# tphakala/birdnet-go

Measured on AMD Instinct MI355X. Metric: 3s-48kHz clips/sec (whole node) + max-abs prob diff vs TFLite, BirdNET v2.4, higher is better.
Workload: dtype f32; 1 GPU; BASELINE configs[1]: BirdNET v2.4 fp32, batch 256 x 3 s @ 48 kHz per GPU, mel front-end + CNN + head on device, raw logits out; batch_per_gpu=256, n_samples=144000, n_classes=6522, pipeline_depth=2, input_sets=4

## Files before the change

### birdnet-go_amd/csrc/conv.hip

```cpp
#include "kernels.h"
#include "pw_common.h"

#include <algorithm>
#include <cstdlib>

namespace bnhip {

__global__ __launch_bounds__(256) void k_conv_direct(ConvParams p) {
    const int C4 = p.Cout >> 2;
    size_t total = (size_t)p.B * p.Ho * p.Wo * C4;
    size_t idx = (size_t)blockIdx.x * 256 + threadIdx.x;
    if (idx >= total) return;
    int c4 = (int)(idx % C4);
    size_t pix = idx / C4;
    int wo = (int)(pix % p.Wo);
    int ho = (int)((pix / p.Wo) % p.Ho);
    int b = (int)(pix / ((size_t)p.Wo * p.Ho));
    float4 acc = make_float4(0.f, 0.f, 0.f, 0.f);
    const float4* w4 = reinterpret_cast<const float4*>(p.w);
    for (int i = 0; i < p.kh; i++) {
        int hi = ho * p.sh - p.pt + i;
        if (hi < 0 || hi >= p.H) continue;
        for (int j = 0; j < p.kw; j++) {
            int wi = wo * p.sw - p.pl + j;
            if (wi < 0 || wi >= p.W) continue;
            const float* ip = p.in + (((size_t)b * p.H + hi) * p.W + wi) * p.Cin;
            const float4* wp = w4 + (size_t)((i * p.kw + j) * p.Cin) * C4 + c4;
            for (int ci = 0; ci < p.Cin; ci++) {
                float x = ip[ci];
                float4 w = wp[(size_t)ci * C4];
                acc.x = fmaf(x, w.x, acc.x); acc.y = fmaf(x, w.y, acc.y);
                acc.z = fmaf(x, w.z, acc.z); acc.w = fmaf(x, w.w, acc.w);
            }
        }
    }
    if (p.bias) {
        float4 bv = reinterpret_cast<const float4*>(p.bias)[c4];
        acc.x += bv.x; acc.y += bv.y; acc.z += bv.z; acc.w += bv.w;
    }
    acc.x = apply_act(acc.x, p.act); acc.y = apply_act(acc.y, p.act);
    acc.z = apply_act(acc.z, p.act); acc.w = apply_act(acc.w, p.act);
    reinterpret_cast<float4*>(p.out)[idx] = acc;
}
template <int KH, int KW, int CIN>
__global__ __launch_bounds__(256) void k_conv_direct_t(ConvParams p) {
    const int C4 = p.Cout >> 2;
    size_t total = (size_t)p.B * p.Ho * p.Wo * C4;
    size_t idx = (size_t)blockIdx.x * 256 + threadIdx.x;
    if (idx >= total) return;
    int c4 = (int)(idx % C4);
    size_t pix = idx / C4;
    int wo = (int)(pix % p.Wo);
    int ho = (int)((pix / p.Wo) % p.Ho);
    int b = (int)(pix / ((size_t)p.Wo * p.Ho));
    float x[KH][KW][CIN];
#pragma unroll
    for (int i = 0; i < KH; i++) {
        int hi = ho * p.sh - p.pt + i;
#pragma unroll
        for (int j = 0; j < KW; j++) {
            int wi = wo * p.sw - p.pl + j;
            bool ok = hi >= 0 && hi < p.H && wi >= 0 && wi < p.W;
            const float* ip = p.in + (((size_t)b * p.H + (ok ? hi : 0)) * p.W + (ok ? wi : 0)) * CIN;
#pragma unroll
            for (int ci = 0; ci < CIN; ci++) x[i][j][ci] = ok ? ip[ci] : 0.f;
        }
    }
    float4 acc = p.bias ? reinterpret_cast<const float4*>(p.bias)[c4] : make_float4(0.f, 0.f, 0.f, 0.f);
    float4 a2 = make_float4(0.f, 0.f, 0.f, 0.f);
    const float4* w4 = reinterpret_cast<const float4*>(p.w) + c4;
#pragma unroll
    for (int i = 0; i < KH; i++)
#pragma unroll
        for (int j = 0; j < KW; j++)
#pragma unroll
            for (int ci = 0; ci < CIN; ci++) {
                float4 w = w4[(size_t)((i * KW + j) * CIN + ci) * C4];
                float xv = x[i][j][ci];
                a2.x = fmaf(xv, w.x, a2.x); a2.y = fmaf(xv, w.y, a2.y); a2.z = fmaf(xv, w.z, a2.z); a2.w = fmaf(xv, w.w, a2.w);
            }
    with_act(p.act, [&](auto f) {
        acc.x = f(a2.x + acc.x); acc.y = f(a2.y + acc.y); acc.z = f(a2.z + acc.z); acc.w = f(a2.w + acc.w);
    });
    reinterpret_cast<float4*>(p.out)[idx] = acc;
}
template <int KH, int KW, int CIN, int S, int PX>
__global__ __launch_bounds__(256) void k_conv_direct_px(ConvParams p, int wgroups) {
    constexpr int NCOL = (PX - 1) * S + KW;
    const int C4 = p.Cout >> 2;
    size_t total = (size_t)p.B * p.Ho * wgroups * C4;
    size_t idx = (size_t)blockIdx.x * 256 + threadIdx.x;
    if (idx >= total) return;
    int c4 = (int)(idx % C4);
    size_t g = idx / C4;
    int wg = (int)(g % wgroups);
    int ho = (int)((g / wgroups) % p.Ho);
    int b = (int)(g / ((size_t)wgroups * p.Ho));
    const int wo0 = wg * PX, wi0 = wo0 * S - p.pl;
    float x[KH][NCOL][CIN];
#pragma unroll
    for (int i = 0; i < KH; i++) {
        int hi = ho * S - p.pt + i;
        bool rok = hi >= 0 && hi < p.H;
        const float* rp = p.in + ((size_t)b * p.H + (rok ? hi : 0)) * p.W * CIN;
#pragma unroll
        for (int c = 0; c < NCOL; c++) {
            int wi = wi0 + c;
            bool ok = rok && wi >= 0 && wi < p.W;
            const float* ip = rp + (size_t)(ok ? wi : 0) * CIN;
#pragma unroll
            for (int ci = 0; ci < CIN; ci++) x[i][c][ci] = ok ? ip[ci] : 0.f;
        }
    }
    const float4 bv = p.bias ? reinterpret_cast<const float4*>(p.bias)[c4] : make_float4(0.f, 0.f, 0.f, 0.f);
    float4 a2[PX];
#pragma unroll
    for (int q = 0; q < PX; q++) a2[q] = make_float4(0.f, 0.f, 0.f, 0.f);
    const float4* w4 = reinterpret_cast<const float4*>(p.w) + c4;
#pragma unroll
    for (int i = 0; i < KH; i++)
#pragma unroll
        for (int j = 0; j < KW; j++)
#pragma unroll
            for (int ci = 0; ci < CIN; ci++) {
                float4 w = w4[(size_t)((i * KW + j) * CIN + ci) * C4];
#pragma unroll
                for (int q = 0; q < PX; q++) {
                    float xv = x[i][q * S + j][ci];
                    a2[q].x = fmaf(xv, w.x, a2[q].x); a2[q].y = fmaf(xv, w.y, a2[q].y);
                    a2[q].z = fmaf(xv, w.z, a2[q].z); a2[q].w = fmaf(xv, w.w, a2[q].w);
                }
            }
    with_act(p.act, [&](auto f) {
#pragma unroll
        for (int q = 0; q < PX; q++) {
            a2[q].x = f(a2[q].x + bv.x); a2[q].y = f(a2[q].y + bv.y); a2[q].z = f(a2[q].z + bv.z); a2[q].w = f(a2[q].w + bv.w);
        }
    });
    const size_t o0 = (((size_t)b * p.Ho + ho) * p.Wo + wo0) * C4 + c4;
    float4* op = reinterpret_cast<float4*>(p.out) + o0;
#pragma unroll
    for (int q = 0; q < PX; q++)
        if (wo0 + q < p.Wo) {
            if (p.out_bf16) bf16x4_store(p.out, o0 + (size_t)q * C4, a2[q]);
            else op[(size_t)q * C4] = a2[q];
        }
}
bool conv_direct_bf16_ok(const ConvParams& p) {
    return p.kh == 3 && p.kw == 3 && (p.Cin == 1 || p.Cin == 2) && p.sh == 2 && p.sw == 2 && (p.Cout & 3) == 0;
}
void launch_conv_direct(const ConvParams& p, hipStream_t s) {
    if (p.kh == 3 && p.kw == 3 && p.Cin == 2 && p.sh == 2 && p.sw == 2 && (p.Cout & 3) == 0) {
        constexpr int PX = 4;
        int wgroups = (p.Wo + PX - 1) / PX;
        size_t tot = (size_t)p.B * p.Ho * wgroups * (p.Cout >> 2);
        hipLaunchKernelGGL((k_conv_direct_px<3, 3, 2, 2, PX>), dim3((unsigned)((tot + 255) / 256)), dim3(256), 0, s, p, wgroups);
        return;
    }
    if (p.kh == 3 && p.kw == 3 && p.Cin == 1 && p.sh == 2 && p.sw == 2 && (p.Cout & 3) == 0) {
        constexpr int PX = 4;
        int wgroups = (p.Wo + PX - 1) / PX;
        size_t tot = (size_t)p.B * p.Ho * wgroups * (p.Cout >> 2);
        hipLaunchKernelGGL((k_conv_direct_px<3, 3, 1, 2, PX>), dim3((unsigned)((tot + 255) / 256)), dim3(256), 0, s, p, wgroups);
        return;
    }
    size_t total = (size_t)p.B * p.Ho * p.Wo * (p.Cout >> 2);
    dim3 grid((unsigned)((total + 255) / 256));
    if (p.kh == 3 && p.kw == 3 && p.Cin == 2) hipLaunchKernelGGL((k_conv_direct_t<3, 3, 2>), grid, dim3(256), 0, s, p);
    else if (p.kh == 3 && p.kw == 3 && p.Cin == 1) hipLaunchKernelGGL((k_conv_direct_t<3, 3, 1>), grid, dim3(256), 0, s, p);
    else if (p.kh == 3 && p.kw == 3 && p.Cin == 3) hipLaunchKernelGGL((k_conv_direct_t<3, 3, 3>), grid, dim3(256), 0, s, p);
    else hipLaunchKernelGGL(k_conv_direct, grid, dim3(256), 0, s, p);
}

struct StemParams {
    const float* in; const float* wm ; const float* bias ; float* out;
    int B, H, W, Ho, Wo, Cout, pt, pl, act;
    unsigned total_px, tiles_per_wave;
};
template <int NTILES>
__global__ __launch_bounds__(256) void k_stem_mfma(StemParams p) {
    constexpr int CS = NTILES * 16 + 4;
    __shared__ __attribute__((aligned(16))) float stage[4 * 16 * CS];
    const int lane = threadIdx.x & 63, wave = threadIdx.x >> 6;
    const int li = lane & 15, kq = lane >> 4;
    f32x4 wf[2][NTILES];
    float4 bq[NTILES];
#pragma unroll
    for (int t = 0; t < NTILES; t++) {
#pragma unroll
        for (int sl = 0; sl < 2; sl++) {
            float4 w = *reinterpret_cast<const float4*>(p.wm + (size_t)(16 * t + li) * 32 + 16 * sl + 4 * kq);
            wf[sl][t] = (f32x4){w.x, w.y, w.z, w.w};
        }
        bq[t] = *reinterpret_cast<const float4*>(p.bias + 16 * t + 4 * kq);
    }
    const int i0 = kq >> 1, j0 = (kq & 1) * 2;
    const unsigned tile0 = (blockIdx.x * 4u + wave) * p.tiles_per_wave;
    const unsigned hw = (unsigned)p.Ho * p.Wo;
    unsigned px = tile0 * 16u + li;
    int b, oh, ow;
    {
        const unsigned pc = min(px, p.total_px - 1);
        b = pc / hw;
        const unsigned rem = pc - (unsigned)b * hw;
        oh = rem / p.Wo; ow = rem - oh * p.Wo;
    }
    for (unsigned tt = 0; tt < p.tiles_per_wave; tt++, px += 16u) {
        if ((tile0 + tt) * 16u >= p.total_px) break;
        if (tt) {
            ow += 16;
            while (ow >= p.Wo) { ow -= p.Wo; if (++oh == p.Ho) { oh = 0; b++; } }
            if (b >= p.B) { b = p.B - 1; oh = p.Ho - 1; ow = p.Wo - 1; }
        }
        const float* xb = p.in + (size_t)b * p.H * p.W * 2;
        f32x4 xf[2];
        const int r0 = oh * 2 - p.pt, c0 = ow * 2 - p.pl + j0;
        const bool inner = r0 >= 0 && r0 + 2 < p.H && c0 >= 0 && c0 + 1 < p.W;
        if (__builtin_amdgcn_ballot_w64(!inner) == 0) {
#pragma unroll
            for (int sl = 0; sl < 2; sl++) {
                const float* q = xb + ((size_t)(r0 + (sl == 0 ? i0 : 2)) * p.W + c0) * 2;
                const float2 a = *reinterpret_cast<const float2*>(q), c = *reinterpret_cast<const float2*>(q + 2);
                xf[sl] = (f32x4){a.x, a.y, c.x, c.y};
            }
        } else {
#pragma unroll
            for (int sl = 0; sl < 2; sl++) {
                const int row = r0 + (sl == 0 ? i0 : 2), col = c0;
                const bool rv = row >= 0 && row < p.H;
                const bool v0 = rv && col >= 0 && col < p.W, v1 = rv && col + 1 >= 0 && col + 1 < p.W;
                const int rc = min(max(row, 0), p.H - 1);
                const float2 a = *reinterpret_cast<const float2*>(xb + ((size_t)rc * p.W + min(max(col, 0), p.W - 1)) * 2);
                const float2 c = *reinterpret_cast<const float2*>(xb + ((size_t)rc * p.W + min(max(col + 1, 0), p.W - 1)) * 2);
                xf[sl] = (f32x4){v0 ? a.x : 0.f, v0 ? a.y : 0.f, v1 ? c.x : 0.f, v1 ? c.y : 0.f};
            }
        }
        f32x4 acc[NTILES];
#pragma unroll
        for (int t = 0; t < NTILES; t++) acc[t] = (f32x4){0.f, 0.f, 0.f, 0.f};
#pragma unroll
        for (int sl = 0; sl < 2; sl++)
#pragma unroll
            for (int sidx = 0; sidx < 4; sidx++)
#pragma unroll
                for (int t = 0; t < NTILES; t++)
                    acc[t] = __builtin_amdgcn_mfma_f32_16x16x4f32(wf[sl][t][sidx], xf[sl][sidx], acc[t], 0, 0, 0);
        with_act(p.act, [&](auto f) {
#pragma unroll
            for (int t = 0; t < NTILES; t++) {
                acc[t][0] = f(acc[t][0] + bq[t].x); acc[t][1] = f(acc[t][1] + bq[t].y);
                acc[t][2] = f(acc[t][2] + bq[t].z); acc[t][3] = f(acc[t][3] + bq[t].w);
            }
        });
        float* stg = stage + wave * (16 * CS);
#pragma unroll
        for (int t = 0; t < NTILES; t++) *reinterpret_cast<f32x4*>(&stg[li * CS + 16 * t + 4 * kq]) = acc[t];
        __builtin_amdgcn_s_waitcnt(0xc07f);
        __builtin_amdgcn_wave_barrier();
        const unsigned px0 = (tile0 + tt) * 16u;
#pragma unroll
        for (int q = 0; q < (16 * NTILES * 4) / 64; q++) {
            const int idx = lane + 64 * q;
            const int row = idx / (NTILES * 4), c4 = idx % (NTILES * 4);
            if (px0 + row < p.total_px)
                *reinterpret_cast<f32x4*>(p.out + (size_t)(px0 + row) * p.Cout + 4 * c4) = *reinterpret_cast<const f32x4*>(&stg[row * CS + 4 * c4]);
        }
        __builtin_amdgcn_wave_barrier();
    }
}
bool stem_mfma_supported(const ConvParams& p) {
    return p.kh == 3 && p.kw == 3 && p.sh == 2 && p.sw == 2 && p.Cin == 2 && (p.Cout == 32 || p.Cout == 64);
}
void launch_stem_mfma(const ConvParams& c, const float* wm, const float* bias_p, hipStream_t s) {
    static const int stem_tpw = getenv("BNHIP_STEM_TPW") ? std::max(atoi(getenv("BNHIP_STEM_TPW")), 1) : 8;
    StemParams p{c.in, wm, bias_p, c.out, c.B, c.H, c.W, c.Ho, c.Wo, c.Cout, c.pt, c.pl, c.act,
                 (unsigned)((size_t)c.B * c.Ho * c.Wo), (unsigned)stem_tpw};
    unsigned tiles = (p.total_px + 15) / 16;
    unsigned blocks = (tiles + 4 * p.tiles_per_wave - 1) / (4 * p.tiles_per_wave);
    if (c.Cout == 32) hipLaunchKernelGGL((k_stem_mfma<2>), dim3(blocks), dim3(256), 0, s, p);
    else hipLaunchKernelGGL((k_stem_mfma<4>), dim3(blocks), dim3(256), 0, s, p);
}

}
```

### birdnet-go_amd/csrc/dwconv.hip

```cpp
#include "kernels.h"
#include "pw_common.h"

#include <algorithm>
#include <cstdlib>

namespace bnhip {

template <int K, int S, int TH, int TW, bool IN16 = false>
__global__ __launch_bounds__(256) void k_dwconv_t(DwParams p, int CX, int PY, int tiles_w, int tiles, int tchunks,
                                                  int cchunks, unsigned nblk, float* __restrict__ partial) {
    __shared__ float red[256 * 4];
    const unsigned L = xcd_remap(blockIdx.x, nblk);
    const int bpc = tchunks * cchunks;
    const int b = L / bpc;
    const int rest = L % bpc;
    const int tc = rest / cchunks, cc = rest % cchunks;
    const int tx = threadIdx.x % CX, ty = threadIdx.x / CX;
    const int c4 = cc * CX + tx;
    const int C4 = p.C >> 2;
    const int tile = tc * PY + ty;
    const bool live = c4 < C4 && tile < tiles && ty < PY;
    float4 acc[TH][TW];
#pragma unroll
    for (int a = 0; a < TH; a++)
#pragma unroll
        for (int c = 0; c < TW; c++) acc[a][c] = make_float4(0.f, 0.f, 0.f, 0.f);
    const int th0 = live ? (tile / tiles_w) * TH : 0, tw0 = live ? (tile % tiles_w) * TW : 0;
    if (live) {
        constexpr int RW = (TW - 1) * S + K;
        constexpr int RH = (TH - 1) * S + K;
        const int hi0 = th0 * S - p.pt, wi0 = tw0 * S - p.pl;
        const float4* in4 = reinterpret_cast<const float4*>(p.in) + (size_t)b * p.H * p.W * C4 + c4;
        const float4* w4 = reinterpret_cast<const float4*>(p.w) + c4;
        uint2 raw[IN16 ? RH : 1][IN16 ? RW : 1];
        if constexpr (IN16) {
            const uint2* in2 = reinterpret_cast<const uint2*>(p.in) + (size_t)b * p.H * p.W * C4 + c4;
#pragma unroll
            for (int r = 0; r < RH; r++)
#pragma unroll
                for (int c = 0; c < RW; c++) {
                    const int hi = hi0 + r, wi = wi0 + c;
                    const bool in = hi >= 0 && hi < p.H && wi >= 0 && wi < p.W;
                    raw[r][c] = in ? in2[((size_t)hi * p.W + wi) * C4] : make_uint2(0u, 0u);
                }
        }
#pragma unroll
        for (int r = 0; r < RH; r++) {
            const int hi = hi0 + r;
            if (hi < 0 || hi >= p.H) continue;
            float4 x[RW];
#pragma unroll
            for (int c = 0; c < RW; c++) {
                int wi = wi0 + c;
                if constexpr (IN16) {
                    const uint2 rr = raw[r][c];
                    x[c] = make_float4(__uint_as_float(rr.x << 16), __uint_as_float(rr.x & 0xffff0000u), __uint_as_float(rr.y << 16), __uint_as_float(rr.y & 0xffff0000u));
                } else if (!(wi >= 0 && wi < p.W)) x[c] = make_float4(0.f, 0.f, 0.f, 0.f);
                else if (p.in_bf16) x[c] = bf16x4_load(p.in, ((size_t)b * p.H * p.W + (size_t)hi * p.W + wi) * C4 + c4);
                else x[c] = in4[((size_t)hi * p.W + wi) * C4];
            }
#pragma unroll
            for (int a = 0; a < TH; a++) {
                const int i = r - a * S;
                if (i < 0 || i >= K) continue;
#pragma unroll
// ... 16 lines not shown
        if (p.act == ACT_SWISH) {
#pragma unroll
            for (int a = 0; a < TH; a++)
#pragma unroll
                for (int c = 0; c < TW; c++) {
                    float4& v = acc[a][c];
                    const f32x4 r = swish4((f32x4){v.x + bv.x, v.y + bv.y, v.z + bv.z, v.w + bv.w});
                    v = make_float4(r[0], r[1], r[2], r[3]);
                }
        } else {
            with_act(p.act, [&](auto f) {
#pragma unroll
                for (int a = 0; a < TH; a++)
#pragma unroll
                    for (int c = 0; c < TW; c++) {
                        float4& v = acc[a][c];
                        v.x = f(v.x + bv.x); v.y = f(v.y + bv.y); v.z = f(v.z + bv.z); v.w = f(v.w + bv.w);
                    }
            });
        }
#pragma unroll
        for (int a = 0; a < TH; a++) {
            int ho = th0 + a;
            if (ho >= p.Ho) continue;
#pragma unroll
            for (int c = 0; c < TW; c++) {
                int wo = tw0 + c;
                if (wo >= p.Wo) continue;
                float4 v = acc[a][c];
                if (p.out_bf16) bf16x4_store(p.out, ((size_t)b * p.Ho * p.Wo + (size_t)ho * p.Wo + wo) * C4 + c4, v);
                else out4[((size_t)ho * p.Wo + wo) * C4] = v;
                sum.x += v.x; sum.y += v.y; sum.z += v.z; sum.w += v.w;
            }
        }
    }
    if (partial) {
        reinterpret_cast<float4*>(red)[threadIdx.x] = sum;
        __syncthreads();
        if (ty == 0 && c4 < C4) {
            float4 t = make_float4(0.f, 0.f, 0.f, 0.f);
            for (int y = 0; y < PY; y++) {
                float4 v = reinterpret_cast<float4*>(red)[y * CX + tx];
                t.x += v.x; t.y += v.y; t.z += v.z; t.w += v.w;
            }
            reinterpret_cast<float4*>(partial)[((size_t)b * tchunks + tc) * C4 + c4] = t;
        }
    }
}

template <int VEC>
__global__ __launch_bounds__(256) void k_dwconv(DwParams p) {
    const int CV = p.C / VEC;
    size_t total = (size_t)p.B * p.Ho * p.Wo * CV;
    size_t idx = (size_t)blockIdx.x * 256 + threadIdx.x;
    if (idx >= total) return;
    int cv = (int)(idx % CV);
    size_t pix = idx / CV;
    int wo = (int)(pix % p.Wo);
    int ho = (int)((pix / p.Wo) % p.Ho);
    int b = (int)(pix / ((size_t)p.Wo * p.Ho));
    float acc[VEC];
#pragma unroll
    for (int v = 0; v < VEC; v++) acc[v] = 0.f;
    for (int i = 0; i < p.kh; i++) {
        int hi = ho * p.sh - p.pt + i;
        if (hi < 0 || hi >= p.H) continue;
        for (int j = 0; j < p.kw; j++) {
            int wi = wo * p.sw - p.pl + j;
            if (wi < 0 || wi >= p.W) continue;
            const float* ip = p.in + (((size_t)b * p.H + hi) * p.W + wi) * p.C + (size_t)cv * VEC;
            const float* wp = p.w + (size_t)(i * p.kw + j) * p.C + (size_t)cv * VEC;
#pragma unroll
            for (int v = 0; v < VEC; v++) acc[v] = fmaf(ip[v], wp[v], acc[v]);
        }
    }
#pragma unroll
    for (int v = 0; v < VEC; v++) {
        float x = acc[v];
        if (p.bias) x += p.bias[cv * VEC + v];
        p.out[idx * VEC + v] = apply_act(x, p.act);
    }
}

static void dw_geometry(const DwParams& p, int TH, int TW, int* CX, int* PY, int* tiles_w, int* tiles, int* tchunks,
                        int* cchunks) {
    int C4 = p.C / 4;
    *CX = C4 < 64 ? C4 : 64;
    *PY = 256 / *CX;
    *tiles_w = (p.Wo + TW - 1) / TW;
    *tiles = *tiles_w * ((p.Ho + TH - 1) / TH);
    if (*PY > *tiles) *PY = *tiles;
    *tchunks = (*tiles + *PY - 1) / *PY;
    *cchunks = (C4 + *CX - 1) / *CX;
}
static bool dw_tiled_shape(const DwParams& p, int* TH, int* TW) {
    if ((p.C & 3) || p.kh != p.kw || p.sh != p.sw) return false;
    if (p.kh == 3 && p.sh == 1) { *TH = 2; *TW = 4; return true; }
    if (p.kh == 3 && p.sh == 2) { *TH = 2; *TW = 2; return true; }
    if (p.kh == 5 && p.sh == 1) { *TH = 2; *TW = 4; return true; }
    if (p.kh == 5 && p.sh == 2) { *TH = 1; *TW = 2; return true; }
    return false;
}
int dwconv_sum_slabs(const DwParams& p) {
    int TH, TW, CX, PY, tw, t, tch, cch;
    if (!dw_tiled_shape(p, &TH, &TW)) return 0;
    dw_geometry(p, TH, TW, &CX, &PY, &tw, &t, &tch, &cch);
    return tch;
}
bool dwconv_tile_geometry(const DwParams& p, int* PY, int* tiles_w, int* tiles, int* tchunks) {
    int TH, TW, CX, cch;
    if (!dw_tiled_shape(p, &TH, &TW) || TH != 2 || TW != 4) return false;
    dw_geometry(p, TH, TW, &CX, PY, tiles_w, tiles, tchunks, &cch);
    return true;
}
void launch_dwconv(const DwParams& p, float* partial, hipStream_t s) {
    int TH, TW;
    if (dw_tiled_shape(p, &TH, &TW)) {
        int CX, PY, tiles_w, tiles, tchunks, cchunks;
        dw_geometry(p, TH, TW, &CX, &PY, &tiles_w, &tiles, &tchunks, &cchunks);
        unsigned nblk = (unsigned)p.B * tchunks * cchunks;
        dim3 block(CX * PY < 64 ? 64 : CX * PY);
        static const bool pre16 = !(getenv("BNHIP_DW_PREFETCH") && atoi(getenv("BNHIP_DW_PREFETCH")) == 0);
#define DW_LAUNCH(K_, S_, TH_, TW_) do { if (p.in_bf16 && pre16) hipLaunchKernelGGL((k_dwconv_t<K_, S_, TH_, TW_, true>), dim3(nblk), block, 0, s, p, CX, PY, \
                                                       tiles_w, tiles, tchunks, cchunks, nblk, partial); \
                                         else hipLaunchKernelGGL((k_dwconv_t<K_, S_, TH_, TW_>), dim3(nblk), block, 0, s, p, CX, PY, \
                                                       tiles_w, tiles, tchunks, cchunks, nblk, partial); } while (0)
        if (p.kh == 3 && p.sh == 1) DW_LAUNCH(3, 1, 2, 4);
        else if (p.kh == 3) DW_LAUNCH(3, 2, 2, 2);
        else if (p.sh == 1) DW_LAUNCH(5, 1, 2, 4);
        else DW_LAUNCH(5, 2, 1, 2);
#undef DW_LAUNCH
        return;
    }
    if ((p.C & 3) == 0) {
        size_t total = (size_t)p.B * p.Ho * p.Wo * (p.C / 4);
        hipLaunchKernelGGL(k_dwconv<4>, dim3((unsigned)((total + 255) / 256)), dim3(256), 0, s, p);
    } else {
        size_t total = (size_t)p.B * p.Ho * p.Wo * p.C;
        hipLaunchKernelGGL(k_dwconv<1>, dim3((unsigned)((total + 255) / 256)), dim3(256), 0, s, p);
    }
}

#define MEAN_SLAB 512
int mean_splits(int HW) { return (HW + MEAN_SLAB - 1) / MEAN_SLAB; }

__global__ __launch_bounds__(256) void k_mean_partial(const float* __restrict__ in, float* __restrict__ partial,
                                                      int HW, int C, int S) {
    __shared__ float red[256];
    const int b = blockIdx.z, sp = blockIdx.y;
    const int CW = blockDim.x, PY = blockDim.y;
    const int c = blockIdx.x * CW + threadIdx.x;
    const int p0 = sp * MEAN_SLAB, p1 = min(HW, p0 + MEAN_SLAB);
    float acc = 0.f;
    if (c < C)
        for (int px = p0 + threadIdx.y; px < p1; px += PY) acc += in[((size_t)b * HW + px) * C + c];
    red[threadIdx.y * CW + threadIdx.x] = acc;
    __syncthreads();
    if (threadIdx.y == 0 && c < C) {
        float sum = 0.f;
        for (int y = 0; y < PY; y++) sum += red[y * CW + threadIdx.x];
        partial[((size_t)b * S + sp) * C + c] = sum;
    }
}
int mean_partial_py(int C) {
    int CW = C < 64 ? C : 64;
    int PY = 256 / CW; if (PY < 1) PY = 1;
    return PY;
}
void launch_mean_partial(const float* in, float* partial, int B, int HW, int C, int S, hipStream_t s) {
    int CW = C < 64 ? C : 64;
    int PY = mean_partial_py(C);
    dim3 grid((C + CW - 1) / CW, S, B);
    hipLaunchKernelGGL(k_mean_partial, grid, dim3(CW, PY), 0, s, in, partial, HW, C, S);
}
__global__ void k_mean_finish(const float* __restrict__ partial, float* __restrict__ out, int B, int HW, int C, int S) {
    size_t idx = (size_t)blockIdx.x * blockDim.x + threadIdx.x;
    if (idx >= (size_t)B * C) return;
    int c = (int)(idx % C); size_t b = idx / C;
    float sum = 0.f;
    for (int sidx = 0; sidx < S; sidx++) sum += partial[(b * S + sidx) * C + c];
    out[idx] = sum / (float)HW;
}
void launch_mean_finish(const float* partial, float* out, int B, int HW, int C, int S, hipStream_t s) {
    size_t total = (size_t)B * C;
    hipLaunchKernelGGL(k_mean_finish, dim3((unsigned)((total + 255) / 256)), dim3(256), 0, s, partial, out, B, HW, C, S);
}

__global__ __launch_bounds__(1024) void k_se(SeParams p) {
    extern __shared__ __attribute__((aligned(16))) float sm[];
    float* mean = sm;
    float* r = sm + p.C;
    const int b = blockIdx.x, tid = threadIdx.x, lane = tid & 63, wave = tid >> 6;
    const int NTHR = blockDim.x, NW = NTHR >> 6;
    const float inv = 1.0f / (float)p.HW;
    int P = 1;
    while (P * 2 * p.C <= NTHR && P * 2 <= p.S) P *= 2;
    float* part = sm + ((p.C + p.Cr + 3) & ~3);
    if (P > 1) {
        const int c = tid % p.C, q = tid / p.C;
        if (q < P) {
            float sum = 0.f;
#pragma unroll 4
            for (int sidx = q; sidx < p.S; sidx += P) sum += p.partial[((size_t)b * p.S + sidx) * p.C + c];
            part[q * p.C + c] = sum;
        }
        __syncthreads();
        for (int c2 = tid; c2 < p.C; c2 += NTHR) {
            float sum = 0.f;
            for (int q2 = 0; q2 < P; q2++) sum += part[q2 * p.C + c2];
            mean[c2] = sum * inv;
        }
    } else {
        for (int c = tid; c < p.C; c += NTHR) {
            float sum = 0.f;
#pragma unroll 4
            for (int sidx = 0; sidx < p.S; sidx++) sum += p.partial[((size_t)b * p.S + sidx) * p.C + c];
            mean[c] = sum * inv;
        }
    }
    __syncthreads();
    const bool v4 = (p.C & 3) == 0;
    for (int j0 = wave; j0 < p.Cr; j0 += 4 * NW) {
        float acc[4] = {0.f, 0.f, 0.f, 0.f};
        if (v4) {
            const float4* m4 = reinterpret_cast<const float4*>(mean);
            const float4* w4 = reinterpret_cast<const float4*>(p.w1);
            const int C4 = p.C / 4;
#pragma unroll 2
            for (int c = lane; c < C4; c += 64) {
                const float4 mv = m4[c];
                float4 w[4];
#pragma unroll
                for (int u = 0; u < 4; u++) w[u] = w4[(size_t)min(j0 + u * NW, p.Cr - 1) * C4 + c];
#pragma unroll
                for (int u = 0; u < 4; u++) {
                    acc[u] = fmaf(w[u].x, mv.x, acc[u]); acc[u] = fmaf(w[u].y, mv.y, acc[u]);
                    acc[u] = fmaf(w[u].z, mv.z, acc[u]); acc[u] = fmaf(w[u].w, mv.w, acc[u]);
                }
            }
        } else {
            for (int c = lane; c < p.C; c += 64) {
                const float mv = mean[c];
#pragma unroll
                for (int u = 0; u < 4; u++) acc[u] = fmaf(p.w1[(size_t)min(j0 + u * NW, p.Cr - 1) * p.C + c], mv, acc[u]);
            }
// ... 64 lines not shown
```

### birdnet-go_amd/csrc/engine.cpp

```cpp
#include "engine.h"

#include <algorithm>
#include <cmath>
#include <cstdio>
#include <cstdlib>
#include <cstring>
#include <mutex>
#include <sstream>

#include "../../include/bnhip.h"
#include "hostpipe.h"

namespace bnhip {

#define HIPCHK(call)                                                                           \
    do {                                                                                       \
        hipError_t e_ = (call);                                                                \
        if (e_ != hipSuccess) {                                                                \
            *err = std::string(#call) + ": " + hipGetErrorString(e_);                          \
            return false;                                                                      \
        }                                                                                      \
    } while (0)

Engine::~Engine() {
// ... 415 lines not shown
        const float* d_in = lanes[li].d_in; float* d_logits = lanes[li].d_logits; float* d_emb = lanes[li].d_emb;
        const int n = lanes[li].n, clip0 = nl > 1 ? li : -1;
        hipStream_t stream = lanes[li].st;
        float* in0 = vptr(s.in0, d_in, d_logits, d_emb, clip0);
        float* in1 = vptr(s.in1, d_in, d_logits, d_emb, clip0);
        float* in2 = vptr(s.in2, d_in, d_logits, d_emb, clip0);
        float* out = vptr(s.out, d_in, d_logits, d_emb, clip0);
        float* out2 = vptr(s.out2, d_in, d_logits, d_emb, clip0);
        if (s.kind == S_DW && si > 0 && steps[si - 1].tail == 2 && tail_taken(si - 1, n, nl > 1)) continue;
        if (s.kind == S_MEAN_PARTIAL && si > 0 && steps[si - 1].tail == 1 && tail_taken(si - 1, n, nl > 1)) continue;
        if (s.kind == S_MEAN_FINISH && si > 1 && steps[si - 2].tail == 1 && tail_taken(si - 2, n, nl > 1)) continue;
        if (s.kind == S_NORMALIZE && si == norm_pair + 1 && res_x[li]) continue;
        ProfEntry pe{};
        static const char* dbg_sync_before = getenv("BNHIP_DEBUG_SYNC_BEFORE");
        static const char* dbg_sync_after = getenv("BNHIP_DEBUG_SYNC_AFTER");
        static const char* dbg_ctx1_only = getenv("BNHIP_DEBUG_CTX1_ONLY");
        if (dbg_ctx1_only && cur_ctx == 1 && !strstr(dbg_ctx1_only, s.kclass)) continue;
        static const char* dbg_ctx1_skip = getenv("BNHIP_DEBUG_CTX1_SKIP");
        if (dbg_ctx1_skip && cur_ctx == 1 && strstr(dbg_ctx1_skip, s.kclass)) continue;
        if (dbg_sync_before && (!strcmp(dbg_sync_before, s.kclass) || s.name.rfind(dbg_sync_before, 0) == 0)) hipStreamSynchronize(stream);
        const bool prof_this = profiling && (profile_filter.empty() || profile_filter == s.kclass);
        if (prof_this) { pe.a = get_event(); pe.b = get_event(); pe.step = si; pe.n = n; hipEventRecord(pe.a, stream); }
        switch (s.kind) {
            case S_MINMAX:
                if (si == norm_pair && res_x[li]) {
                    const WinView lane_win = win_at(pcm.win, lanes[li].clip0);
                    if (!launch_clip_norm_resident(res_x[li], res_bits[li], n, n_samples, specs[0].eps, specs[0].norm_sub, specs[0].norm_mul,
                                                   reinterpret_cast<float2*>(out), vptr(steps[si + 1].out, d_in, d_logits, d_emb, clip0), stream,
                                                   res_framed[li] ? &lane_win : nullptr)) {
                        *err = "k_clip_norm_resident refused a call its predicate accepted"; mm_dirty = true; return false;
                    }
                    pe.more_bytes = steps[si + 1].bytes - s.bytes - (res_bits[li] ? (double)n_samples * (4 - res_bits[li] / 8) : 0.0);
                    break;
                }
                launch_clip_minmax(in0, n, n_samples, specs[0].eps, reinterpret_cast<float2*>(out),
                                   mm_scratch ? mm_scratch + ((size_t)std::max(cur_ctx, 0) * kMaxLanes + (size_t)li) * kMinMaxScratch : nullptr, stream);
                break;
            case S_FRONTEND: {
                const FrontSpec& fs = specs[s.spec];
                FrontendParams p;
                p.x = in0; p.mm = reinterpret_cast<const float2*>(in1); p.G = fs.G; p.window = fs.window; p.out = out;
                p.n_samples = n_samples; p.L = fs.L; p.Lfft = fs.Lfft; p.Kp = fs.Kp; p.hop = fs.hop; p.F = fs.F; p.n_mels = fs.n_mels;
                p.NTP = fs.NTP; p.C = C_spec; p.c = fs.c; p.norm_sub = fs.norm_sub; p.norm_mul = fs.norm_mul;
                p.p1 = fs.p1; p.p2 = fs.p2; p.n_clips = n;
                launch_frontend(p, stream);
                break;
            }
            case S_NORMALIZE:
                launch_normalize(in0, reinterpret_cast<const float2*>(in1), out, n, n_samples, specs[0].norm_sub, specs[0].norm_mul, stream);
                break;
            case S_STFT: {
                const FrontSpec& fs = specs[s.spec];
                StftParams p{in0, fs.window_full, fs.bins, out, n_samples, fs.Lfft, fs.L, fs.hop, fs.F, fs.nb, fs.nbp, fs.mode, n, fs.stft_tw, fs.pad_left};
                p.zmask = fs.stft_zmask;
                if (s.mode == 1) {
                    p.out = nullptr; p.img = out; p.mel = s.w3; p.mel_quads = s.S; p.n_mels = fs.n_mels; p.Ctot = C_spec; p.c0 = fs.c;
                    p.logc = fs.log_compress ? 1 : 0; p.time_major = fs.time_major ? 1 : 0; p.p1 = fs.p1; p.p2 = fs.p2;
                    p.lfloor = fs.log_floor; p.lscale = fs.log_scale;
                }
                {
                    static const bool f32_off = getenv("BNHIP_STFT_F32") && atoi(getenv("BNHIP_STFT_F32")) == 0;
                    if (precision == 1 && s.mode != 1 && fs.log_compress && !f32_off) p.f32 = 1;
                }
                launch_stft_bins(p, stream);
                break;
            }
            case S_MELBAND: {
                const FrontSpec& fa = specs[s.spec];
                const FrontSpec& fb = specs[s.S == 2 ? s.op : s.spec];
                MelBandParams p{{in0, s.S == 2 ? in1 : in0}, {s.w0, s.S == 2 ? s.w2 : s.w0},
                                {reinterpret_cast<const int*>(s.w1), reinterpret_cast<const int*>(s.S == 2 ? s.w3 : s.w1)},
                                {fa.nbp, fb.nbp}, {fa.p1, fb.p1}, {fa.p2, fb.p2}, out, fa.F, fa.n_mels, C_spec, fa.c,
                                fa.log_compress ? 1 : 0, fa.log_floor, fa.log_scale, fa.time_major ? 1 : 0};
                launch_mel_banded(p, s.S, n, stream);
                break;
            }
            case S_MELFIN: {
                const FrontSpec& fa = specs[s.spec];
                const FrontSpec& fb = specs[s.S == 2 ? s.op : s.spec];
                MelFinParams p{{in0, s.S == 2 ? in1 : in0}, {fa.p1, fb.p1}, {fa.p2, fb.p2}, out, fa.F, fa.n_mels, fa.n_mels, C_spec, fa.c,
                               fa.log_compress ? 1 : 0, fa.log_floor, fa.log_scale, fa.time_major ? 1 : 0};
                launch_mel_finish(p, s.S, n, stream);
                break;
            }
            case S_CONV_DIRECT: {
                ConvParams p{in0, s.w0, s.w1, out, n, s.H, s.W, s.C, s.Ho, s.Wo, s.Co, s.kh, s.kw, s.sh, s.sw, s.pt, s.pl, s.act};
                p.out_bf16 = vals[s.out].half ? 1 : 0;
                if (s.w2) launch_stem_mfma(p, s.w2, s.w3, stream);
                else launch_conv_direct(p, stream);
                break;
            }
            case S_CONV_IGEMM:
                launch_conv_igemm(in0, s.w0, s.w1, out, n, s.H, s.W, s.C, s.Ho, s.Wo, s.Co, s.kh, s.kw, s.sh, s.sw, s.g.dh, s.g.dw, s.pt, s.pl,
                                  s.act, 0, 0, stream);
                break;
            case S_PW: {
                PwParams p = pw_params(s, n, nl > 1);
                p.A = in0; p.ascale = in1; p.res = in2; p.out = out;
                if (tail_taken(si, n, nl > 1)) {
                    const Step& c = steps[si + 1];
                    PwTail t = tail_of(s, c);
                    if (s.tail == 2) { t.out = vptr(c.out, d_in, d_logits, d_emb, clip0); t.partial = vptr(c.out2, d_in, d_logits, d_emb, clip0); }
                    else p.out = vptr(steps[si + 2].out, d_in, d_logits, d_emb, clip0);
                    launch_pw_tail(p, t, s.wbx, p.nt, p.wm, stream);
                    break;
                }
                if (p.wm >= 13) p.wm = 10;
                if (p.wm >= 5 && s.wbx) launch_pw_bx3(p, s.wbx, stream);
                else launch_pw_gemm(p, stream);
                break;
            }
            case S_DW: {
                DwParams p = dw_params(s, in0, out, n);
                p.in_bf16 = vals[s.in0].half ? 1 : 0; p.out_bf16 = vals[s.out].half ? 1 : 0;
                if (s.dwl) launch_dwconv_lds(p, out2, s.shape, stream);
                else launch_dwconv(p, out2, stream);
                break;
            }
            case S_EXPAND_DW:
                {
                    StemGeom sg{s.H2, s.W2, s.pt2, s.pl2};
                    launch_expand_dw(in0, s.w0, s.w1, s.w2, s.w3, out, out2, n, s.H, s.W, s.C, s.Co,
                                     s.Ho, s.Wo, s.kh, s.sh, s.pt, s.pl, s.act, s.act2, s.shape, s.mode == 1 ? &sg : nullptr, stream,
                                     s.bx ? s.wbx : nullptr, precision, vals[s.out].half ? 1 : 0, vals[s.in0].half ? 1 : 0);
                }
                break;
            case S_MEAN_PARTIAL:
                launch_mean_partial(in0, out, n, s.H * s.W, s.C, s.S, stream);
                break;
            case S_MEAN_FINISH:
                launch_mean_finish(in0, out, n, s.H * s.W, s.C, s.S, stream);
                break;
            case S_SE: {
                SeParams p{in0, s.S, s.H * s.W, s.w0, s.w1, s.w2, s.w3, out, n, s.C, s.Cr, s.act, s.act2};
                if (cur_stream) p.threads = 256;
                launch_se(p, stream);
                break;
            }
            case S_UNARY:
                launch_unary(in0, out, vals[s.in0].elems * (size_t)n, s.act, stream);
                break;
            case S_BINARY:
                launch_binary(in0, s.mode == 2 ? s.w0 : in1, out, vals[s.in0].elems * (size_t)n, s.op, s.mode, s.H * s.W, s.C,
                              s.act, stream);
                break;
            case S_EW_UNARY:
                launch_unary_op(in0, out, vals[s.in0].elems * (size_t)n, s.op, s.g.alpha, stream);
                break;
            case S_EW_BINARY: {
                BcastParams p;
                p.a = s.g.a_const ? s.w0 : in0; p.b = s.g.b_const ? s.w1 : in1; p.out = out;
                for (int k = 0; k < 4; k++) { p.d[k] = s.g.d[k]; p.sa[k] = s.g.sa[k]; p.sb[k] = s.g.sb[k]; }
                p.bsa = s.g.a_const ? 0 : (long)vals[s.in0].elems; p.bsb = s.g.b_const ? 0 : (long)vals[s.in1].elems;
                p.op = s.op; p.act = s.act;
                launch_binary_bcast(p, n, stream);
                break;
            }
            case S_POOL: {
                PoolParams p{in0, out, n, s.H, s.W, s.C, s.Ho, s.Wo, s.kh, s.kw, s.sh, s.sw, s.pt, s.pl, s.mode, s.act};
                launch_pool2d(p, stream);
                break;
            }
            case S_COPY: {
                if (s.g.fill) launch_fill(out, vals[s.out].elems * (size_t)n, s.g.alpha, stream);
                CopyParams p;
                p.in = s.g.a_const ? s.w0 : in0; p.out = out;
                for (int k = 0; k < 4; k++) { p.d[k] = s.g.d[k]; p.si[k] = s.g.sa[k]; p.so[k] = s.g.so[k]; }
                p.offi = s.g.offa; p.offo = s.g.offo;
                p.bsi = s.g.a_const ? 0 : (long)vals[s.in0].elems; p.bso = (long)vals[s.out].elems;
                launch_copy_view(p, n, stream);
                break;
            }
            case S_SOFTMAX:
                launch_softmax_rows(in0, out, (size_t)s.H * (size_t)n, s.C, s.g.alpha, stream);
                break;
            case S_REDUCE: {
                ReduceParams p{in0, out, {s.g.d[0], s.g.d[1], s.g.d[2], s.g.d[3]}, s.g.mask, s.op};
                launch_reduce(p, n, stream);
                break;
            }
            case S_CONV_GENERIC: {
                GenConvParams p{in0, s.w0, s.w1, out, n, s.H, s.W, s.C, s.Ho, s.Wo, s.Co, s.kh, s.kw, s.sh, s.sw, s.g.dh, s.g.dw,
                                s.pt, s.pl, s.act, s.g.depthwise, s.g.mult};
                launch_conv_generic(p, stream);
                break;
            }
        }
// ... 29 lines not shown
        hipEventElapsedTime(&b, step_ev[0].first, step_ev[i].second);
        if (i < cap) { if (start_ms) start_ms[i] = a; if (end_ms) end_ms[i] = b; }
    }
    for (auto& p : step_ev) { hipEventDestroy(p.first); hipEventDestroy(p.second); }
    step_ev.clear();
    (void)hipGetLastError();
    return n;
}

static void jesc(std::ostringstream& os, const std::string& s) {
    for (char c : s) { if (c == '"' || c == '\\') os << '\\'; os << c; }
}

struct StepView { std::string name; double flops, bytes; bool absorbed; };
static StepView step_view(const Engine& e, size_t i) {
    const Step& s = e.steps[i];
    StepView v{s.name, s.flops, s.bytes, false};
    auto fused = [&](size_t k) { return e.steps[k].kind == S_PW && e.steps[k].tail && e.steps[k].wm_full >= 13; };
    if (fused(i)) {
        const double mine = 4.0 * s.H * s.W * s.Co;
        if (s.tail == 2) { v.name += "+dw"; v.flops += e.steps[i + 1].flops; }
        else { v.name += "+mean"; v.flops += e.steps[i + 1].flops + e.steps[i + 2].flops; v.bytes += 4.0 * s.Co - mine; }
    } else if ((s.kind == S_DW && i > 0 && e.steps[i - 1].tail == 2 && fused(i - 1)) ||
               (s.kind == S_MEAN_PARTIAL && i > 0 && e.steps[i - 1].tail == 1 && fused(i - 1)) ||
               (s.kind == S_MEAN_FINISH && i > 1 && e.steps[i - 2].tail == 1 && fused(i - 2))) {
        v.flops = 0; v.bytes = 0; v.absorbed = true;
    }
    return v;
}

std::string Engine::describe() const {
    std::ostringstream os;
    os << "{\"tune_source\":\"";
    jesc(os, tune_source);
    os << "\",\"tune_key\":\"" << (device >= 0 ? tune_key() : std::string()) << "\",\"split_step\":" << split_step << ",\"heatmap_tail\":\"" << (heatmap_pruned_step() >= 0 ? "pruned" : "gather") << "\",\"n_samples\":" << n_samples << ",\"n_classes\":" << n_classes << ",\"emb_dim\":" << emb_dim
       << ",\"max_batch\":" << max_batch << ",\"logits_output\":" << logits_output << ",\"embedding_output\":" << embedding_output << ",\"precision\":\"" << (precision ? "bf16" : "f32") << "\",\"lanes\":" << n_lanes << ",\"lane_min_batch\":" << dual_lane_min << ",\"act_arena_bytes\":" << act_bytes << ",\"weight_bytes\":" << w_bytes
       << ",\"specs\":[";
    for (size_t i = 0; i < specs.size(); i++) {
        const FrontSpec& f = specs[i];
        os << (i ? "," : "") << "{\"frame_length\":" << f.L << ",\"fft_length\":" << f.Lfft << ",\"hop\":" << f.hop
           << ",\"frames\":" << f.F << ",\"n_mels\":" << f.n_mels << ",\"channel\":" << f.c << ",\"p1\":" << f.p1
           << ",\"p2\":" << f.p2 << "}";
    }
    os << "],\"steps\":[";
    for (size_t i = 0; i < steps.size(); i++) {
        const Step& s = steps[i];
        const StepView sv = step_view(*this, i);
        const bool absorbed = sv.absorbed;
        os << (i ? "," : "") << "{\"i\":" << i << ",\"kernel\":\"" << s.kclass << "\",\"name\":\"";
        jesc(os, sv.name);
        os << "\",\"H\":" << s.H << ",\"W\":" << s.W << ",\"C\":" << s.C << ",\"Co\":" << s.Co << ",\"k\":" << s.kh
           << ",\"stride\":" << s.sh << ",\"act\":" << s.act << ",\"fused_scale\":" << (s.kind == S_PW && s.in1 >= 0 ? 1 : 0)
           << ",\"shape\":" << s.shape << ",\"dw_lds\":" << s.dwl << ",\"bx\":" << s.bx << ",\"nt\":" << s.nt << ",\"wm\":" << s.wm << ",\"nt_full\":" << s.nt_full << ",\"wm_full\":" << s.wm_full << ",\"fused_res\":" << (s.kind == S_PW && s.in2 >= 0 ? 1 : 0) << ",\"fused_sum\":" << (s.out2 >= 0 ? 1 : 0) << ",\"flops\":" << sv.flops << ",\"bytes\":" << sv.bytes << ",\"wbytes\":" << s.wbytes
           << ",\"tail\":" << s.tail << ",\"absorbed\":" << (absorbed ? 1 : 0) << ",\"out_v\":" << s.out << ",\"out2_v\":" << s.out2
           << ",\"in_bf16\":" << ((s.in0 >= 0 && vals[s.in0].half) ? 1 : 0) << ",\"out_bf16\":" << ((s.out >= 0 && vals[s.out].half) ? 1 : 0) << "}";
    }
    os << "]}";
    return os.str();
}

std::string Engine::profile_read() {
    hipStreamSynchronize(stream);
    struct Agg { double ms = 0, flops = 0, bytes = 0; long launches = 0; };
    std::map<std::string, Agg> agg;
    std::vector<std::string> order;
    std::vector<Agg> per_step(steps.size());
    for (auto& e : prof) {
        float ms = 0;
        hipEventElapsedTime(&ms, e.a, e.b);
        const Step& s = steps[e.step];
        const StepView sv = step_view(*this, e.step);
        if (!agg.count(s.kclass)) order.push_back(s.kclass);
        Agg& a = agg[s.kclass];
        a.ms += ms; a.launches++; a.flops += sv.flops * e.n; a.bytes += (sv.bytes + e.more_bytes) * e.n + s.wbytes;
        Agg& ps = per_step[e.step];
        ps.ms += ms; ps.launches++; ps.flops += sv.flops * e.n; ps.bytes += (sv.bytes + e.more_bytes) * e.n + s.wbytes;
        ev_pool.push_back(e.a); ev_pool.push_back(e.b);
    }
    prof.clear();
    std::ostringstream os;
    os << "[";
    for (size_t i = 0; i < order.size(); i++) {
        const Agg& a = agg[order[i]];
        os << (i ? "," : "") << "{\"kernel\":\"" << order[i] << "\",\"launches\":" << a.launches << ",\"ms\":" << a.ms
           << ",\"flops\":" << a.flops << ",\"bytes\":" << a.bytes << "}";
    }
    for (size_t i = 0; i < steps.size(); i++) {
        const Agg& a = per_step[i];
        if (!a.launches) continue;
        os << ",{\"step\":" << i << ",\"kernel\":\"" << steps[i].kclass << "\",\"name\":\"";
        jesc(os, step_view(*this, i).name);
        os << "\",\"launches\":" << a.launches << ",\"ms\":" << a.ms << ",\"flops\":" << a.flops << ",\"bytes\":" << a.bytes << "}";
    }
    os << "]";
    return os.str();
}

}
```

### birdnet-go_amd/csrc/engine.h

```cpp
#pragma once
#include <hip/hip_runtime.h>

#include <map>
#include <string>
#include <vector>

#include "kernels.h"
#include "tflite_model.h"

namespace bnhip {

enum StepKind { S_MINMAX, S_FRONTEND, S_NORMALIZE, S_STFT, S_MELFIN, S_MELBAND, S_CONV_DIRECT, S_PW, S_DW, S_EXPAND_DW, S_MEAN_PARTIAL, S_MEAN_FINISH, S_SE, S_UNARY, S_BINARY,
                S_EW_UNARY, S_EW_BINARY, S_POOL, S_COPY, S_SOFTMAX, S_REDUCE, S_CONV_GENERIC,
                S_CONV_IGEMM };

struct GenGeom {
    int d[4] = {1, 1, 1, 1};
    long sa[4] = {0, 0, 0, 0}, sb[4] = {0, 0, 0, 0}, so[4] = {0, 0, 0, 0};
    long offa = 0, offo = 0;
    bool a_const = false, b_const = false;
    int mask = 0;
    float alpha = 0.f;
    bool fill = false;
    int dh = 1, dw = 1, depthwise = 0, mult = 1;
};

struct Step {
    StepKind kind;
    std::string name;
    const char* kclass;
    int in0 = -1, in1 = -1, in2 = -1, out = -1, out2 = -1;
    const float *w0 = nullptr, *w1 = nullptr, *w2 = nullptr, *w3 = nullptr;
    const uint16_t* wbx = nullptr;
    int dwl = 0;
    int bx = 0;
    int H = 0, W = 0, C = 0, Ho = 0, Wo = 0, Co = 0, kh = 1, kw = 1, sh = 1, sw = 1, pt = 0, pl = 0;
    int act = 0, act2 = 0, op = 0, mode = 0, S = 1, Cr = 0;
    int nt = 0, wm = 0;
    int tail = 0;
    int H2 = 0, W2 = 0, pt2 = 0, pl2 = 0;
    int shape = -1;
    int nt_full = 0, wm_full = 0;
    int spec = -1;
    GenGeom g;
    double flops = 0, bytes = 0, wbytes = 0;
};

struct Value {
    int tfl = -1;
    size_t elems = 0;
    size_t offset = 0;
    size_t offset_lane = 0;
    int first = -1, last = -1;
    bool external = false;
    bool half = false;
};

struct FrontSpec {
    int L, Kp, Lfft, hop, F, n_mels, NTP, c;
    float p1, p2, eps, norm_sub, norm_mul;
    const double* G = nullptr;
    const float* window = nullptr;
    bool fft = false;
    int nb = 0, nbp = 0, mode = 0;
    const float* window_full = nullptr;
    const double* stft_tw = nullptr;
    unsigned stft_zmask = 0xffffffffu;
    const int* bins = nullptr;
    bool normalize = true, log_compress = false, time_major = false;
    int pad_left = 0;
    float log_floor = 0.f, log_scale = 1.f;
};

struct PcmSource { const void* samples = nullptr; int bits = 0;  WinView win = {}; };

struct ProfEntry { hipEvent_t a, b; int step; int n; double more_bytes = 0; };

struct WeightPlan {
    std::vector<float> img;
    std::vector<size_t> step_w[4];
    std::vector<size_t> step_bx;
};

inline DwParams dw_params(const Step& s, const float* in = nullptr, float* out = nullptr, int n = 1) {
    return DwParams{in, s.w0, s.w1, out, n, s.H, s.W, s.C, s.Ho, s.Wo, s.kh, s.kw, s.sh, s.sw, s.pt, s.pl, s.act};
}
PwTail tail_of(const Step& s, const Step& c);

class Engine {
  public:
    ~Engine();
    bool build(TflModel m, int device, int max_batch, bool plan_only, std::string* err, int* code);
    bool run(const float* d_in, int n, float* d_logits, float* d_emb, std::string* err, PcmSource pcm = {});

    int device = 0, max_batch = 256;
    bool no_reuse = false;
    bool autotune = true;
    bool defer_weights = false;
    void finish_deferred();
    char* weights_ptr() const { return w_arena; }
    size_t weights_bytes() const { return w_bytes; }
    int frontend_fft = -1;
    int logits_output = -1, embedding_output = -2;
    int precision = 0;
    int bf16x3 = 0;
    int pw_sw = 0;
    bool use_graphs = false;
    void drop_graphs();
    static constexpr int kMaxDepth = 3;
    int depth = 1;
    hipStream_t ctx_stream[kMaxDepth] = {nullptr, nullptr, nullptr};
    char* ctx_arena[kMaxDepth] = {nullptr, nullptr, nullptr};
    static constexpr int kMinMaxScratch = 16 * (2 * kMinMaxParts + 2);
    float* mm_scratch = nullptr;
    bool mm_dirty = false;
    bool norm_resident = true;
    int norm_pair = -1;
    bool pcm_direct = false;
    void find_norm_pair();
    bool norm_resident_taken(int n, const void* x, int bits, const float* xn) const;
    hipEvent_t ev_ctx_fork = nullptr, ev_ctx_done[kMaxDepth] = {nullptr, nullptr, nullptr};
    unsigned call_idx = 0;
    bool run_pipelined(const float* d_in, int n, float* d_logits, float* d_emb, std::string* err);
    void sync_contexts();
    int host_depth = 2;
    bool ensure_contexts(int d, std::string* err, bool with_streams = true);
    bool run_on_context(int c, hipStream_t st, const float* d_in, int n, float* d_logits, float* d_emb, std::string* err, PcmSource pcm = {});
    int split_step = -1, v_hand = -1;
    float* d_hand = nullptr;
    std::vector<int> split_candidates;
    void pick_split();
    size_t hand_clip_bytes() const { return v_hand < 0 ? 0 : vals[v_hand].elems * (vals[v_hand].half ? 2 : 4); }
    bool ensure_hand(std::string* err);
    bool run_part(int c, hipStream_t st, int s0, int s1, const float* d_in, int n, float* hand, float* d_logits, float* d_emb, std::string* err, PcmSource pcm = {});
    int heatmap_pruned_step() const;
    bool run_head(int s1, const float* d_in, int n, std::string* err);
    struct HostPipe* hostpipe = nullptr;
    static constexpr int kMaxLanes = 4;
    int n_lanes = 2;
    int dual_lane_min = 32;
    hipStream_t lane_stream[kMaxLanes - 1] = {nullptr, nullptr, nullptr};
    hipEvent_t ev_fork = nullptr, ev_join[kMaxLanes - 1] = {nullptr, nullptr, nullptr};
    void mark_tails();
    bool tail_taken(int si, int n, bool lane_tuning) const;
    PwParams pw_params(const Step& s, int n, bool lane_tuning) const;
    void mark_bf16_storage();
    void tune_or_load();
    void autotune_pw();
    void autotune_expdw();
    void autotune_dw();
    void autotune_tail();
    bool save_tuning(const char* path) const;
    bool load_tuning(const char* path);
    std::string tuning_text() const;
    bool apply_tuning_text(const std::string& text);
    std::string tune_key() const;
    std::string tune_dir;
    std::string tune_source;
    bool expdw_pipe16(const Step& s) const;
    ExpDwGeo expdw_geo(const Step& s) const;
    void set_sum_slabs(Step& s, int S);
    std::map<int, int> tensor_value;
    const float* value_ptr(int v) const { return reinterpret_cast<const float*>(act_arena + vals[v].offset); }
    int n_samples = 0, n_classes = 0, emb_dim = 0, C_spec = 0;
    hipStream_t stream = nullptr;
    bool own_stream = false;
    static constexpr int kMaxKStreams = 4;
    hipStream_t kstream[kMaxKStreams] = {nullptr, nullptr, nullptr, nullptr};
    hipStream_t kernel_stream(int i);
    hipStream_t copy_stream();
    hipStream_t xfer_stream = nullptr;
    bool ds_ref = false;
// ... 49 lines not shown
```

### birdnet-go_amd/csrc/expdw.hip

```cpp
#include "kernels.h"
#include "pw_common.h"

#include <algorithm>
#include <type_traits>
#include <cmath>
#include <cstdio>
#include <cstdlib>
#include <cstring>
#include <vector>

namespace bnhip {

struct ExpDwParams {
    const float* x; const float* we; const float* be; const float* wd; const float* bd;
    float* y; float* partial;
    int B, H, W, Cin, Cmid, Ho, Wo, pt, pl, act_e, act_d, tiles_h, tiles_w, cchunks, Kw, Cp;
    int Hin = 0, Win = 0, pts = 0, pls = 0;
    const uint16_t* wep = nullptr; int Kp = 0;
    int prec = 0;
    int xsh = 0, xsw = 1, ysh = 0, ysw = 1, tr = 0;
    int in_bf16 = 0, out_bf16 = 0;
    FDiv d_bpc{}, d_cch{}, d_tw{};
    int cpp = 0;
    FDiv d_part{};
};
#define ED_ES 36
#define ED_PERM2 0xfdce5764b98a1320ull
#define ED_PERM4 0xfdce9ba875461320ull
__device__ __forceinline__ int ed_perm(unsigned long long magic, int lane) {
    return (int)((magic >> ((lane >> 2) * 4)) & 15ull) * 4 + (lane & 3);
}
constexpr bool ed_perm_c4_rule(unsigned long long magic) {
    for (int g = 0; g < 16; g++)
        if (((magic >> (4 * g)) & 1ull) != (unsigned long long)((g >> 1) & 1)) return false;
    return true;
}
constexpr int expdw_min_waves(int K, int S, int TOW, int TRH) {
    const int tiw = (TOW - 1) * S + K, jt = (TRH * tiw + 15) / 16, jtw = (jt + 3) / 4;
    return jtw <= 4 ? 4 : (jtw == 5 ? 3 : 2);
}
#ifndef EXPDW_NW8_WAVES
#define EXPDW_NW8_WAVES (est <= 76 ? 6 : 4)
#endif
constexpr int expdw_sk_waves(int K, int S, int TOH, int TOW, int TRH, int KW, bool one_chunk, int NW = 4) {
    const int tiw = (TOW - 1) * S + K, jt = (TRH * tiw + 15) / 16, jtw = (jt + NW - 1) / NW;
    if (one_chunk) return jtw <= 3 ? 5 : expdw_min_waves(K, S, TOW, TRH);
    const int sh = TOH / NW, sw = TOW / 8, rw = (sw - 1) * S + K;
    const int p1 = jtw * 8 + 8, p2 = sh * sw * 4 + rw * 4 + K * 4;
    const int est = jtw * KW / 4 + (KW / 2 + 16) + 24 + (p1 > p2 ? p1 : p2);
    if (NW == 8) return EXPDW_NW8_WAVES;
    return est <= 120 ? 4 : (est <= 160 ? 3 : 2);
}
template <int K, int S, int TOH, int TOW, int TRH, int NW = 4, typename PreStore>
__device__ __forceinline__ float4 ed_phase2(const ExpDwParams& p, const float* E, const float4* wds, int b, int oh0, int ow0, int vr0,
                                            int vr1, int ty, int tx, int c4, int n_base, const float4& bv, PreStore&& pre_store) {
    constexpr int TIW = (TOW - 1) * S + K;
    static_assert(TOH % NW == 0, "a wave owns TOH / NW output rows");
    constexpr int SH = TOH / NW, SW = TOW / 8;
    constexpr int RW = (SW - 1) * S + K;
    const int n = n_base + 4 * c4;
    float4 sum = make_float4(0.f, 0.f, 0.f, 0.f);
    float4 acc2[SH][SW];
#pragma unroll
    for (int a = 0; a < SH; a++)
#pragma unroll
        for (int c = 0; c < SW; c++) acc2[a][c] = make_float4(0.f, 0.f, 0.f, 0.f);
    if (n < p.Cmid) {
        const float* e0 = E + (tx * SW * S) * ED_ES + 4 * c4;
#pragma unroll 1
        for (int i = 0; i < K; i++) {
            float4 w[K];
#pragma unroll
            for (int j = 0; j < K; j++) w[j] = wds[(i * K + j) * 8 + c4];
#pragma unroll
            for (int a = 0; a < SH; a++) {
                const int fr = (ty * SH + a) * S + i;
                if (fr < vr0 || fr >= vr1 || oh0 + ty * SH + a >= p.Ho) continue;
// ... 44 lines not shown
                const unsigned yo = ylane + (unsigned)((a * p.ysh + c * p.ysw) * p.Cmid);
                if (p.out_bf16) bf16x4_store(p.y, ((size_t)b * p.Ho * p.Wo * p.Cmid + yo) >> 2, v);
                else *reinterpret_cast<float4*>(yclip + yo) = v;
                sum.x += v.x; sum.y += v.y; sum.z += v.z; sum.w += v.w;
            }
        }
    }
    return sum;
}
__device__ __forceinline__ void ed_sums_lanes(float4 sum, float4* red, int wave, int lane, int c4) {
    static_assert(ed_perm_c4_rule(ED_PERM2) && ed_perm_c4_rule(ED_PERM4), "lane permutation: c4 bit 2 must be physical lane bit 3");
    auto xsum = [&](auto pat) {
        constexpr int P = decltype(pat)::value;
        sum.x += __builtin_bit_cast(float, __builtin_amdgcn_ds_swizzle(__builtin_bit_cast(int, sum.x), P));
        sum.y += __builtin_bit_cast(float, __builtin_amdgcn_ds_swizzle(__builtin_bit_cast(int, sum.y), P));
        sum.z += __builtin_bit_cast(float, __builtin_amdgcn_ds_swizzle(__builtin_bit_cast(int, sum.z), P));
        sum.w += __builtin_bit_cast(float, __builtin_amdgcn_ds_swizzle(__builtin_bit_cast(int, sum.w), P));
    };
    xsum(std::integral_constant<int, 0x101f>{});
    xsum(std::integral_constant<int, 0x401f>{});
    if ((lane & 0x14) == 0) red[(wave * 2 + (lane >> 5)) * 8 + c4] = sum;
}
template <int NW = 4>
__device__ __forceinline__ void ed_sums_out(const ExpDwParams& p, const float4* red, int tid, size_t tile_index, int n_base) {
    if (tid < 8 && n_base + 4 * tid < p.Cmid) {
        float4 t = red[tid];
#pragma unroll
        for (int w = 1; w < 2 * NW; w++) { float4 v = red[w * 8 + tid]; t.x += v.x; t.y += v.y; t.z += v.z; t.w += v.w; }
        unsigned l4 = 4u * (unsigned)tid;
        asm volatile("" : "+v"(l4));
        *reinterpret_cast<float4*>(p.partial + tile_index * p.Cmid + n_base + l4) = t;
    }
}

constexpr int expdw_fullw_vw(int K, int S, int TOW) { return TOW * S == 32 && (TOW - 1) * S + K >= 32 ? 32 : 0; }
template <int K, int S, int TOH, int TOW, int TRH, bool H8 = false, bool BX = false, bool COPY = false, int VW = 0>
__global__ __launch_bounds__(256, BX ? expdw_min_waves(K, S, TOW, TRH) : 1) void k_expand_dw(ExpDwParams p, unsigned nblk) {
    constexpr int TIH = (TOH - 1) * S + K, TIW = (TOW - 1) * S + K;
    static_assert(TRH <= TIH, "TRH is a cap on the footprint rows");
    constexpr bool FULLW = VW > 0;
    static_assert(!FULLW || (!COPY && VW % 16 == 0 && VW <= TIW && VW == expdw_fullw_vw(K, S, TOW)), "full-width form: see expdw_fullw_vw");
    static_assert(!FULLW || (TIW - VW) * TRH * 8 <= 256, "full-width form: the padding columns are one float4 store of some threads");
    constexpr int NPIX = TRH * TIW;
    constexpr int GW = FULLW ? VW : TIW;
    constexpr int JT = (TRH * GW + 15) / 16, JTW = (JT + 3) / 4;
    constexpr int SW = TOW / 8;
    __shared__ __attribute__((aligned(16))) float lds[NPIX * ED_ES + 256 + K * K * 32];
    float* E = lds;
    float4* red = reinterpret_cast<float4*>(lds + NPIX * ED_ES);
    float4* wds = reinterpret_cast<float4*>(lds + NPIX * ED_ES + 256);
    const int tid = threadIdx.x, lane = tid & 63, wave = __builtin_amdgcn_readfirstlane(tid >> 6);
    const int li = lane & 15, kq = lane >> 4;

    const unsigned L = xcd_remap(blockIdx.x, nblk);
    const int tiles = p.tiles_h * p.tiles_w;
    const int bpc = tiles * p.cchunks;
    const int b = (int)fdiv(L, p.d_bpc), rest = (int)L - b * bpc;
    const int tile = (int)fdiv((unsigned)rest, p.d_cch), cc = rest - tile * p.cchunks;
    const int trow = (int)fdiv((unsigned)tile, p.d_tw);
    const int oh0 = trow * TOH, ow0 = (tile - trow * p.tiles_w) * TOW;
    const int ih0 = oh0 * S - p.pt, iw0 = ow0 * S - p.pl;
    const int vr0 = max(ih0, 0) - ih0, vr1 = min(ih0 + TIH, p.H) - ih0;
    const int nvalid = (vr1 - vr0) * GW;
    const int jtv = (nvalid + 15) >> 4;
    const int Cin = p.Cin, Kw = p.Kw;
    const int n_base = cc * 32;

    static_assert(SW * S == 2 || SW * S == 4, "lane permutation tables cover SW*S in {2, 4}");
    constexpr unsigned long long PERM = SW * S == 2 ? ED_PERM2 : ED_PERM4;
    const int pl = ed_perm(PERM, lane);
    const int c4 = pl & 7, tx = pl >> 3;
    float4 wdreg = make_float4(0.f, 0.f, 0.f, 0.f);
    if (tid < K * K * 8 && (!COPY || n_base + 4 * (tid & 7) < p.Cmid)) {
        const int tap = tid >> 3, tsrc = p.tr ? (tap % K) * K + tap / K : tap;
        wdreg = *reinterpret_cast<const float4*>(p.wd + (size_t)tsrc * p.Cp + n_base + 4 * (tid & 7));
    }
    const float4 zero4 = make_float4(0.f, 0.f, 0.f, 0.f);
    const float4 bq0 = COPY ? zero4 : *reinterpret_cast<const float4*>(p.be + n_base + 4 * kq);
    const float4 bq1 = COPY ? zero4 : *reinterpret_cast<const float4*>(p.be + n_base + 16 + 4 * kq);
    const float4 bv = (COPY && (!p.bd || n_base + 4 * c4 >= p.Cmid)) ? zero4 : *reinterpret_cast<const float4*>(p.bd + n_base + 4 * c4);

    if constexpr (COPY) {
        const float4* x4 = reinterpret_cast<const float4*>(p.x);
        const int C4 = p.Cmid >> 2, q4 = (n_base >> 2) + (tid & 7);
        const bool cin = q4 < C4;
        const size_t img = (size_t)b * p.H * p.W;
#pragma unroll 4
        for (int j = tid >> 3; j < nvalid; j += 32) {
            const int r = j / TIW, c = j - r * TIW;
            const int iw = iw0 + c, ih = ih0 + vr0 + r;
            float4 v = zero4;
            if (cin && iw >= 0 && iw < p.W) {
                const size_t quad = (img + (size_t)ih * p.xsh + (size_t)iw * p.xsw) * C4 + q4;
                v = p.in_bf16 ? bf16x4_load(p.x, quad) : x4[quad];
            }
            *reinterpret_cast<float4*>(&E[j * ED_ES + 4 * (tid & 7)]) = v;
        }
        if (tid < K * K * 8) wds[tid] = wdreg;
        __syncthreads();
    } else {

    int xoff[JTW];
    bool xin[FULLW ? 1 : JTW];
#pragma unroll
    for (int a = 0; a < JTW; a++) {
        int j = 16 * (wave + 4 * a) + li;
        int r = j / GW, c = j - r * GW;
// ... 137 lines not shown
            if constexpr (FULLW) {
                int e = ((j / VW) * TIW + j % VW + p.pl) * ED_ES + 4 * kq;
                *reinterpret_cast<f32x4*>(&E[e]) = acc[a][0];
                *reinterpret_cast<f32x4*>(&E[e + 16]) = acc[a][1];
            } else if (j < nvalid) {
                int e = j * ED_ES + 4 * kq;
                if (border) {
                    const f32x4 z = (f32x4){0.f, 0.f, 0.f, 0.f};
                    *reinterpret_cast<f32x4*>(&E[e]) = xin[a] ? acc[a][0] : z;
                    *reinterpret_cast<f32x4*>(&E[e + 16]) = xin[a] ? acc[a][1] : z;
                } else {
                    *reinterpret_cast<f32x4*>(&E[e]) = acc[a][0];
                    *reinterpret_cast<f32x4*>(&E[e + 16]) = acc[a][1];
                }
            }
        }
    }
    if (tid < K * K * 8) wds[tid] = wdreg;
    __syncthreads();
    }

    const float4 sum = ed_phase2<K, S, TOH, TOW, TRH, 4>(p, E, wds, b, oh0, ow0, vr0, vr1, wave, tx, c4, n_base, bv, [] {});
    if (p.partial) {
        ed_sums_lanes(sum, red, wave, lane, c4);
        __syncthreads();
        ed_sums_out(p, red, tid, (size_t)b * tiles + tile, n_base);
    }
}

template <int K, int S, int TOH, int TOW, int TRH, bool STEM, int KW, bool LOOP = !STEM, int NW = 4, int PH = 0, int NS = 1>
__global__ __launch_bounds__(64 * NW, expdw_sk_waves(K, S, TOH, TOW, TRH, PH == 1 ? 16 * NS : KW, !LOOP, NW)) void k_expand_dw_sk(ExpDwParams p, unsigned nblk) {
    static_assert(PH == 0 || PH == 1, "phase 1 on the f32 or on the bf16 pipe");
    constexpr bool B16 = PH == 1;
    static_assert(!B16 || (LOOP && !STEM), "bf16 phase 1: chunk-loop form");
    static_assert(NS == 1 || B16, "several resident slabs: bf16 operands only");
    constexpr int KP = 32 * NS;
    static_assert(PH != 1 || KW == 24 || KW == 32, "one-product form: layers of the bf16 engines");
    static_assert(NW == 4 || (NW == 8 && LOOP && TOH % 8 == 0), "eight-wave blocks: chunk-loop form, tile height a multiple of 8");
    static_assert(KW == 16 || KW == 24 || KW == 32, "one or two K slabs, or a slab and a half");
    static_assert(!STEM || KW == 24, "the stem's window is 3 rows x 4 columns x 2 channels");
    constexpr int TIH = (TOH - 1) * S + K, TIW = (TOW - 1) * S + K;
    static_assert(TRH <= TIH, "TRH is a cap on the footprint rows");
    constexpr int NPIX = TRH * TIW, NPIXP = (NPIX + 15) / 16 * 16;
    constexpr int JT = NPIXP / 16, JTW = (JT + NW - 1) / NW;
    constexpr int SW = TOW / 8;
    constexpr int NMMA = B16 ? 2 * NS : KW / 2;
    __shared__ __attribute__((aligned(16))) float lds[NPIX * ED_ES + 64 * NW + K * K * 32];
    float* E = lds;
    float4* red = reinterpret_cast<float4*>(lds + NPIX * ED_ES);
    float4* wds = reinterpret_cast<float4*>(lds + NPIX * ED_ES + 64 * NW);
    const int tid = threadIdx.x, lane = tid & 63, wave = __builtin_amdgcn_readfirstlane(tid >> 6);
    const int li = lane & 15, kq = lane >> 4;

    const unsigned L = xcd_remap(blockIdx.x, nblk);
    const int tiles = p.tiles_h * p.tiles_w;
    int b, tile, cc0 = 0;
    int cpp = p.cchunks;
    if constexpr (LOOP) {
        if (p.cpp > 0) {
            cpp = p.cpp;
            const int nparts = (p.cchunks + cpp - 1) / cpp;
            b = (int)fdiv(L, p.d_bpc);
            const int rest = (int)L - b * tiles * nparts;
            tile = (int)fdiv((unsigned)rest, p.d_part);
            cc0 = (rest - tile * nparts) * cpp;
        } else {
            b = (int)fdiv(L, p.d_bpc); tile = (int)L - b * tiles;
        }
    } else {
        b = (int)fdiv(L, p.d_bpc);
        const int rest = (int)L - b * tiles * p.cchunks;
        tile = (int)fdiv((unsigned)rest, p.d_cch); cc0 = rest - tile * p.cchunks;
    }
    const int trow = (int)fdiv((unsigned)tile, p.d_tw);
    const int oh0 = trow * TOH, ow0 = (tile - trow * p.tiles_w) * TOW;
    const int ih0 = oh0 * S - p.pt, iw0 = ow0 * S - p.pl;
    const int vr0 = max(ih0, 0) - ih0, vr1 = min(ih0 + TIH, p.H) - ih0;
    const int nvalid = (vr1 - vr0) * TIW;
    const int jtv = (nvalid + 15) >> 4;
    const int Cin = p.Cin;
    const int ncc = LOOP ? min(cpp, p.cchunks - cc0) : 1;
    const size_t tile_index = (size_t)b * tiles + tile;

    static_assert(SW * S == 2 || SW * S == 4, "lane permutation tables cover SW*S in {2, 4}");
    constexpr unsigned long long PERM = SW * S == 2 ? ED_PERM2 : ED_PERM4;
    const int pl = ed_perm(PERM, lane);
    const int c4 = pl & 7, tx = pl >> 3;

    bool xin[JTW];
    f32x4 xA[B16 ? 1 : JTW];
    f32x4 xB[(KW == 32 && !B16) ? JTW : 1];
    f32x2 xH[(KW == 24 && !B16) ? JTW : 1];
    bf16x8 xb[B16 ? JTW : 1][NS];
    auto load_x = [&]() {
        const float* xbase = STEM ? p.x + (size_t)b * p.Hin * p.Win * 2 : p.x;
#pragma unroll
        for (int a = 0; a < JTW; a++) {
            const int j = 16 * (wave + NW * a) + li;
            const int r = j / TIW, c = j - r * TIW;
            const int iw = iw0 + c;
            xin[a] = j < nvalid && iw >= 0 && iw < p.W;
            const int ihc = min(ih0 + vr0 + r, p.H - 1), iwc = min(max(iw, 0), p.W - 1);
            if constexpr (STEM) {
                const int row0 = ihc * 2 - p.pts, col0 = iwc * 2 - p.pls;
                auto tap2 = [&](int row, int col) {
                    const bool v = row >= 0 && row < p.Hin && col >= 0 && col < p.Win;
                    const float2 u = *reinterpret_cast<const float2*>(xbase + ((size_t)min(max(row, 0), p.Hin - 1) * p.Win + min(max(col, 0), p.Win - 1)) * 2);
// ... 280 lines not shown
        if (best < 0 || c < best_cost) { best = i; best_cost = c; }
    }
    return best;
}
int expdw_sum_slabs(const ExpDwGeo& g) {
    int idx = expdw_default_shape(g);
    return idx < 0 ? 0 : expdw_shape_slabs(idx, g);
}
int expdw_max_slabs(const ExpDwGeo& g) {
    int mx = 0;
    for (int i = 0; i < 2 * kNumExpDwShapes; i++)
        if (expdw_shape_fits(i, g)) mx = std::max(mx, expdw_shape_slabs(i, g));
    return mx;
}
bool expdw_bx_ok(int Cin) { return (Cin & 7) == 0 && Cin >= 16; }
int expdw_kp(int Cin) { return (Cin + 31) / 32 * 32; }
std::vector<uint16_t> expdw_bx_image(const float* We , int Cmid, int Cin) {
    const int Cp = expdw_cp(Cmid), Kp = expdw_kp(Cin);
    std::vector<uint16_t> img((size_t)Cp * 3 * Kp, 0);
    for (int n = 0; n < Cmid; n++)
        for (int k = 0; k < Cin; k++) {
            uint16_t piece[3];
            bx3_split_host(We[(size_t)n * Cin + k], piece);
            for (int pl = 0; pl < 3; pl++) img[((size_t)n * 3 + pl) * Kp + k] = piece[pl];
        }
    return img;
}
bool expdw_sk_pipe16(int Cin, int act_e, bool stem, int prec, bool have_image) {
    static const bool off = getenv("BNHIP_EXPDW_B16") && atoi(getenv("BNHIP_EXPDW_B16")) == 0;
    static const int max_ns = getenv("BNHIP_EXPDW_B16_NS") ? atoi(getenv("BNHIP_EXPDW_B16_NS")) : 5;
    if (off || !have_image || stem || act_e != ACT_SWISH || !expdw_bx_ok(Cin)) return false;
    const int kw = expdw_skw(Cin, act_e, stem), ns = expdw_kp(Cin) / 32;
    return prec == 1 && ((kw == 24 || kw == 32) || (kw == 0 && (ns == 2 || ns == 3 || ns == 5) && ns <= max_ns));
}
bool expdw_supported(int k, int s, int Cin, int Cmid, int act_e, int prec) {
    if (!((k == 3 || k == 5) && (s == 1 || s == 2) && (Cin & 3) == 0 && (Cmid & 3) == 0)) return false;
    if (Cin <= 128) return true;
    return prec == 1 && expdw_sk_pipe16(Cin, act_e, false, prec, true);
}
template <int K, int S, int TH, int TW, int TR, bool H8, bool BX>
static void ed_launch(const ExpDwParams& p, unsigned nblk, hipStream_t st, bool fullw) {
    constexpr int VW = expdw_fullw_vw(K, S, TW);
    if constexpr (VW > 0) {
        if (fullw) {
            hipLaunchKernelGGL((k_expand_dw<K, S, TH, TW, TR, H8, BX, false, VW>), dim3(nblk), dim3(256), 0, st, p, nblk);
            return;
        }
    }
    hipLaunchKernelGGL((k_expand_dw<K, S, TH, TW, TR, H8, BX>), dim3(nblk), dim3(256), 0, st, p, nblk);
}
void launch_expand_dw(const float* x, const float* we, const float* be, const float* wd, const float* bd, float* y,
                      float* partial, int B, int H, int W, int Cin, int Cmid, int Ho, int Wo, int k, int s, int pt,
                      int pl, int act_e, int act_d, int shape, const StemGeom* stem, hipStream_t st, const uint16_t* wep, int prec, int out_bf16,
                      int in_bf16) {
    const bool pipe16 = expdw_sk_pipe16(Cin, act_e, stem != nullptr, prec, wep != nullptr);
    const ExpDwGeo g0{k, s, H, W, Ho, Wo, pt, pl, stem != nullptr, pipe16 ? 0 : expdw_skw(Cin, act_e, stem != nullptr)};
    if (!expdw_shape_fits(shape, g0, false)) shape = expdw_default_shape(g0);
    if (shape < 0) return;
    const ExpDwShape* sh = &kExpDwShapes[shape % kNumExpDwShapes];
    const bool tr = shape >= kNumExpDwShapes;
    const ExpDwGeo g = expdw_oriented(shape, g0);
    ExpDwParams p{x, we, be, wd, bd, y, partial, B, g.H, g.W, Cin, Cmid, g.Ho, g.Wo, g.pt, g.pl, act_e, act_d,
                  (g.Ho + sh->toh - 1) / sh->toh, (g.Wo + sh->tow - 1) / sh->tow, (Cmid + 31) / 32, expdw_kw(Cin), expdw_cp(Cmid)};
    p.xsh = tr ? 1 : W; p.xsw = tr ? W : 1; p.ysh = tr ? 1 : Wo; p.ysw = tr ? Wo : 1; p.tr = tr ? 1 : 0;
    p.out_bf16 = out_bf16;
    unsigned nblk = (unsigned)B * p.tiles_h * p.tiles_w * p.cchunks;
    p.d_bpc = make_fdiv((unsigned)(p.tiles_h * p.tiles_w * p.cchunks));
    p.d_cch = make_fdiv((unsigned)p.cchunks);
    p.d_tw = make_fdiv((unsigned)p.tiles_w);
    if (stem) p.Kw = 24;
    const bool sk = stem || pipe16 || (act_e == ACT_SWISH && (p.Kw == 16 || p.Kw == 24 || p.Kw == 32));
    const bool bx = wep != nullptr && !sk && expdw_bx_ok(Cin);
    if (bx) { p.wep = wep; p.Kp = expdw_kp(Cin); p.prec = prec; }
    const bool b16 = pipe16;
    const bool fullw = !sk && expdw_fullwidth(shape, g0);
    if (pipe16) { p.wep = wep; p.Kp = expdw_kp(Cin); p.prec = prec; p.in_bf16 = in_bf16; }
    if (sk && !stem) {
        const int tiles = p.tiles_h * p.tiles_w;
        nblk = (unsigned)B * tiles;
        p.d_bpc = make_fdiv((unsigned)tiles);
        const int cus = device_cus();
        if (p.cchunks > 1 && (long)B * tiles < cus / 2) {
            const int want = (int)std::min<long>(p.cchunks, (cus + (long)B * tiles - 1) / ((long)B * tiles));
            const int cpp = (p.cchunks + want - 1) / want, nparts = (p.cchunks + cpp - 1) / cpp;
            if (nparts > 1) {
                p.cpp = cpp;
                p.d_part = make_fdiv((unsigned)nparts);
                nblk = (unsigned)B * tiles * nparts;
                p.d_bpc = make_fdiv((unsigned)(tiles * nparts));
            }
        }
    }
    if (stem) {
        p.Hin = stem->Hin; p.Win = stem->Win; p.pts = stem->pt; p.pls = stem->pl;
#define ED_STEM(TH_, TW_, TR_)                                                                                \
    if (sh->k == 3 && sh->s == 1 && sh->toh == TH_ && sh->tow == TW_ && sh->trh == TR_) {                     \
        hipLaunchKernelGGL((k_expand_dw_sk<3, 1, TH_, TW_, TR_, true, 24>), dim3(nblk), dim3(256), 0, st, p, nblk);  \
        return;                                                                                               \
    }
        ED_STEM(8, 16, 10) ED_STEM(4, 16, 6) ED_STEM(8, 32, 6) ED_STEM(8, 32, 10)
#undef ED_STEM
        return;
    }
#define ED_CASE8(K_, S_, TH_, TW_, TR_)                                                                       \
    if (sh->nw == 8 && sh->k == K_ && sh->s == S_ && sh->toh == TH_ && sh->tow == TW_ && sh->trh == TR_) {    \
        if (p.Kw == 16) hipLaunchKernelGGL((k_expand_dw_sk<K_, S_, TH_, TW_, TR_, false, 16, true, 8>), dim3(nblk), dim3(512), 0, st, p, nblk); \
        else if (p.Kw == 24) hipLaunchKernelGGL((k_expand_dw_sk<K_, S_, TH_, TW_, TR_, false, 24, true, 8>), dim3(nblk), dim3(512), 0, st, p, nblk); \
        else hipLaunchKernelGGL((k_expand_dw_sk<K_, S_, TH_, TW_, TR_, false, 32, true, 8>), dim3(nblk), dim3(512), 0, st, p, nblk); \
        return;                                                                                               \
    }
    if (sh->nw == 8) {
        if (!sk || stem) return;
        ED_CASE8(3, 1, 8, 16, 10) ED_CASE8(3, 1, 8, 32, 6) ED_CASE8(3, 1, 8, 32, 10) ED_CASE8(5, 1, 8, 16, 12) ED_CASE8(5, 1, 8, 32, 6)
        ED_CASE8(3, 2, 8, 8, 12) ED_CASE8(3, 2, 8, 8, 17) ED_CASE8(5, 2, 8, 8, 19)
        return;
    }
#undef ED_CASE8
#define ED_CASE(K_, S_, TH_, TW_, TR_)                                                                        \
    if (sh->k == K_ && sh->s == S_ && sh->toh == TH_ && sh->tow == TW_ && sh->trh == TR_) {                   \
        if (bx) ed_launch<K_, S_, TH_, TW_, TR_, false, true>(p, nblk, st, fullw);                                \
        else if (b16 && p.Kp == 64) hipLaunchKernelGGL((k_expand_dw_sk<K_, S_, TH_, TW_, TR_, false, 32, true, 4, 1, 2>), dim3(nblk), dim3(256), 0, st, p, nblk); \
        else if (b16 && p.Kp == 96) hipLaunchKernelGGL((k_expand_dw_sk<K_, S_, TH_, TW_, TR_, false, 32, true, 4, 1, 3>), dim3(nblk), dim3(256), 0, st, p, nblk); \
        else if (b16 && p.Kp == 160) hipLaunchKernelGGL((k_expand_dw_sk<K_, S_, TH_, TW_, TR_, false, 32, true, 4, 1, 5>), dim3(nblk), dim3(256), 0, st, p, nblk); \
        else if (b16 && p.Kw == 24) hipLaunchKernelGGL((k_expand_dw_sk<K_, S_, TH_, TW_, TR_, false, 24, true, 4, 1>), dim3(nblk), dim3(256), 0, st, p, nblk); \
        else if (b16) hipLaunchKernelGGL((k_expand_dw_sk<K_, S_, TH_, TW_, TR_, false, 32, true, 4, 1>), dim3(nblk), dim3(256), 0, st, p, nblk); \
        else if (sk && p.Kw == 16) hipLaunchKernelGGL((k_expand_dw_sk<K_, S_, TH_, TW_, TR_, false, 16>), dim3(nblk), dim3(256), 0, st, p, nblk); \
        else if (sk && p.Kw == 24) hipLaunchKernelGGL((k_expand_dw_sk<K_, S_, TH_, TW_, TR_, false, 24>), dim3(nblk), dim3(256), 0, st, p, nblk); \
        else if (sk && p.Kw == 32) hipLaunchKernelGGL((k_expand_dw_sk<K_, S_, TH_, TW_, TR_, false, 32>), dim3(nblk), dim3(256), 0, st, p, nblk); \
        else if (p.Kw & 8) ed_launch<K_, S_, TH_, TW_, TR_, true, false>(p, nblk, st, fullw);                     \
        else ed_launch<K_, S_, TH_, TW_, TR_, false, false>(p, nblk, st, fullw);                                  \
        return;                                                                                               \
    }
    ED_CASE(3, 1, 8, 16, 10) ED_CASE(3, 1, 4, 16, 6) ED_CASE(3, 1, 8, 32, 6) ED_CASE(3, 1, 8, 32, 10)
    ED_CASE(5, 1, 8, 16, 12) ED_CASE(5, 1, 4, 16, 8) ED_CASE(5, 1, 8, 32, 6) ED_CASE(5, 1, 12, 16, 12)
    ED_CASE(3, 2, 4, 8, 9) ED_CASE(3, 2, 8, 8, 12) ED_CASE(3, 2, 8, 8, 17)
    ED_CASE(5, 2, 4, 8, 11) ED_CASE(5, 2, 4, 16, 6) ED_CASE(5, 2, 8, 8, 19)
#undef ED_CASE
}

bool dwconv_lds_supported(const DwParams& p) {
    return (p.C & 3) == 0 && p.kh == p.kw && p.sh == p.sw && (p.kh == 3 || p.kh == 5) && (p.sh == 1 || p.sh == 2);
}
void launch_dwconv_lds(const DwParams& q, float* partial, int shape, hipStream_t st) {
    const ExpDwGeo g0{q.kh, q.sh, q.H, q.W, q.Ho, q.Wo, q.pt, q.pl, false};
    if (!expdw_shape_fits(shape, g0, false)) shape = expdw_default_shape(g0);
    if (shape < 0) return;
    const ExpDwShape* sh = &kExpDwShapes[shape % kNumExpDwShapes];
    const bool tr = shape >= kNumExpDwShapes;
    const ExpDwGeo g = expdw_oriented(shape, g0);
    ExpDwParams p{q.in, nullptr, nullptr, q.w, q.bias, q.out, partial, q.B, g.H, g.W, q.C, q.C, g.Ho, g.Wo, g.pt, g.pl, ACT_NONE, q.act,
                  (g.Ho + sh->toh - 1) / sh->toh, (g.Wo + sh->tow - 1) / sh->tow, (q.C + 31) / 32, 0, q.C};
    p.xsh = tr ? 1 : q.W; p.xsw = tr ? q.W : 1; p.ysh = tr ? 1 : q.Wo; p.ysw = tr ? q.Wo : 1; p.tr = tr ? 1 : 0;
    p.in_bf16 = q.in_bf16; p.out_bf16 = q.out_bf16;
    unsigned nblk = (unsigned)q.B * p.tiles_h * p.tiles_w * p.cchunks;
    p.d_bpc = make_fdiv((unsigned)(p.tiles_h * p.tiles_w * p.cchunks));
    p.d_cch = make_fdiv((unsigned)p.cchunks);
    p.d_tw = make_fdiv((unsigned)p.tiles_w);
#define DL_CASE(K_, S_, TH_, TW_, TR_)                                                                        \
    if (sh->k == K_ && sh->s == S_ && sh->toh == TH_ && sh->tow == TW_ && sh->trh == TR_) {                   \
        hipLaunchKernelGGL((k_expand_dw<K_, S_, TH_, TW_, TR_, false, false, true>), dim3(nblk), dim3(256), 0, st, p, nblk); \
        return;                                                                                               \
    }
    DL_CASE(3, 1, 8, 16, 10) DL_CASE(3, 1, 4, 16, 6) DL_CASE(3, 1, 8, 32, 6) DL_CASE(3, 1, 8, 32, 10)
    DL_CASE(5, 1, 8, 16, 12) DL_CASE(5, 1, 4, 16, 8) DL_CASE(5, 1, 8, 32, 6) DL_CASE(5, 1, 12, 16, 12)
    DL_CASE(3, 2, 4, 8, 9) DL_CASE(3, 2, 8, 8, 12) DL_CASE(3, 2, 8, 8, 17)
    DL_CASE(5, 2, 4, 8, 11) DL_CASE(5, 2, 4, 16, 6) DL_CASE(5, 2, 8, 8, 19)
#undef DL_CASE
}


}
```

### birdnet-go_amd/csrc/kernels.h

```cpp
#pragma once
#include <atomic>
#include <hip/hip_runtime.h>

#include <vector>
#include <cstdint>

#include "analyze.h"

namespace bnhip {

inline int device_cus() {
    static std::atomic<int> cus[64];
    int dev = 0;
    if (hipGetDevice(&dev) != hipSuccess) { (void)hipGetLastError(); return 256; }
    if (dev < 0 || dev >= 64) return 256;
    int c = cus[dev].load(std::memory_order_relaxed);
    if (c > 0) return c;
    hipDeviceProp_t pr{};
    if (hipGetDeviceProperties(&pr, dev) != hipSuccess || pr.multiProcessorCount <= 0) { (void)hipGetLastError(); return 256; }
    cus[dev].store(pr.multiProcessorCount, std::memory_order_relaxed);
    return pr.multiProcessorCount;
}

struct PwGrid { int nblk_n; unsigned nblk; };
inline PwGrid pw_grid(int M, int N, int nt, int wm) {
    const int nblk_n = (N + nt * 16 - 1) / (nt * 16);
    return PwGrid{nblk_n, (unsigned)((M + 64 * wm - 1) / (64 * wm)) * (unsigned)nblk_n};
}
bool pw_fill_grid(int M, int N, int* nt, int* wm, PwGrid* g);

template <auto Kern>
inline void lds_limit_once(int bytes) {
    static std::atomic<unsigned long long> done{0};
    int dev = 0;
    if (hipGetDevice(&dev) != hipSuccess) { (void)hipGetLastError(); dev = 0; }
    if (dev < 0 || dev >= 64) { hipFuncSetAttribute(reinterpret_cast<const void*>(Kern), hipFuncAttributeMaxDynamicSharedMemorySize, bytes); return; }
    const unsigned long long bit = 1ull << dev;
    if (done.load(std::memory_order_acquire) & bit) return;
    if (hipFuncSetAttribute(reinterpret_cast<const void*>(Kern), hipFuncAttributeMaxDynamicSharedMemorySize, bytes) == hipSuccess)
        done.fetch_or(bit, std::memory_order_release);
    else (void)hipGetLastError();
}

enum Act : int { ACT_NONE = 0, ACT_RELU = 1, ACT_RELU_N1_TO_1 = 2, ACT_RELU6 = 3, ACT_TANH = 4, ACT_SWISH = 100, ACT_SIGMOID = 101, ACT_HARD_SWISH = 102 };

void launch_pcm_to_f32(const void* pcm, int bits , float* out, size_t n, hipStream_t s);

constexpr int kMinMaxParts = 16;
void launch_clip_minmax(const float* x, int n_clips, int n_samples, float eps, float2* mm, float* scratch , hipStream_t s);
bool clip_norm_resident_fits(int n_samples);
bool clip_norm_framed_ok(const void* block, const WinView& v);
bool launch_clip_norm_resident(const void* x, int bits, int n_clips, int n_samples, float eps, float norm_sub, float norm_mul, float2* mm, float* out,
                               hipStream_t s, const WinView* win = nullptr);

struct FrontendParams {
    const float* x;
    const float2* mm;
    const double* G;
    const float* window;
    float* out;
    int n_samples, L, Lfft, Kp, hop, F, n_mels, NTP, C, c;
    float norm_sub, norm_mul;
    float p1, p2;
    int n_clips;
};
void launch_frontend(const FrontendParams& p, hipStream_t s);
size_t frontend_lds_bytes(int Lfft, int Kp, int hop, int NTP);

struct StftParams {
    const float* xn;
    const float* window;
    const int* bins;
    float* out;
    int n_samples, Lfft, L, hop, F, nb, nbp, mode , n_clips;
    const double* tw = nullptr;
    int pad_left = 0;
    int nb_cap = 0, fpw = 0;
    int f32 = 0;
    unsigned zmask = 0xffffffffu;
    const float* mel = nullptr;
    int mel_quads = 0, n_mels = 0, Ctot = 1, c0 = 0, logc = 0, time_major = 0;
    float p1 = 1.f, p2 = 1.f, lfloor = 0.f, lscale = 1.f;
    float* img = nullptr;
};
std::vector<double> stft_build_tables(int Lfft, const int* bins, int nb);
unsigned stft_zmask(int Lfft, const int* bins, int nb);
std::vector<float> stft_mel_table(int Lfft, const float* melw, const int* span, int n_mels, int nb, int nbp, int* quads);
void launch_normalize(const float* x, const float2* mm, float* out, int n_clips, int n_samples, float norm_sub,
                      float norm_mul, hipStream_t s);
bool stft_supported(int Lfft, int nb);
void launch_stft_bins(const StftParams& p, hipStream_t s);
struct MelFinParams {
    const float* T[2];
    float p1[2], p2[2];
    float* out;
    int F, n_mels, ldt, Ctot, c0;
    int log = 0;
    float lfloor = 0.f, lscale = 1.f;
    int time_major = 0;
};
void launch_mel_finish(const MelFinParams& p, int nch, int n_clips, hipStream_t s);
struct MelBandParams {
    const float* bins[2];
    const float* w[2];
    const int* span[2];
    int nbp[2];
    float p1[2], p2[2];
    float* out;
    int F, n_mels, Ctot, c0;
    int log = 0;
    float lfloor = 0.f, lscale = 1.f;
    int time_major = 0;
};
bool mel_banded_supported(int n_mels, int nbp0, int nbp1);
void launch_mel_banded(const MelBandParams& p, int nch, int n_clips, hipStream_t s);
int frontend_kc(int Lfft, int hop, int NTP);

struct ConvParams {
    const float* in; const float* w ; const float* bias; float* out;
    int B, H, W, Cin, Ho, Wo, Cout, kh, kw, sh, sw, pt, pl, act;
    int out_bf16 = 0;
};
void launch_conv_direct(const ConvParams& p, hipStream_t s);
bool conv_direct_bf16_ok(const ConvParams& p);
bool conv_igemm_supported(int Cin, int Cout, int kh, int kw);
void launch_conv_igemm(const float* in, const float* w_ohwi, const float* bias, float* out, int B, int H, int W, int Cin, int Ho, int Wo,
                       int Cout, int kh, int kw, int sh, int sw, int dh, int dw, int pt, int pl, int act, int nt ,
                       int wm , hipStream_t s);
bool stem_mfma_supported(const ConvParams& p);
void launch_stem_mfma(const ConvParams& p, const float* wm, const float* bias_p, hipStream_t s);

struct PwParams {
    const float* A; const float* W; const float* bias; const float* ascale; const float* res; float* out;
    int M, N, K, HW, act;
    int nt = 0;
    int wm = 0;
    int prec = 0;
    int a_bf16 = 0;
    int out_bf16 = 0;
    int res_bf16 = 0;
    int sw = 0;
};
enum { PW_SW_B16_OFF = 1, PW_SW_B16_FORCE = 2, PW_SW_B16S_OFF = 4, PW_SW_B16S_FORCE = 8, PW_SW_WS_OFF = 16, PW_SW_WS_FORCE = 32, PW_SW_LAT_OFF = 64,
       PW_SW_TAIL_OFF = 128, PW_SW_TAIL_FORCE = 256 };
int pw_switches_from_env();
void launch_pw_gemm(const PwParams& p, hipStream_t s);
bool pw_pipe_ok(int nt, int wm, int K);
int pw_default_nt(int M, int N);
bool pw_bx3_ok(int K);
bool pw_bx3p_ok(int nt, int wm , int K);
int pw_bx3_npad(int N);
std::vector<uint16_t> pw_bx3_image(const float* W, int N, int K);
void launch_pw_bx3(const PwParams& p, const uint16_t* Wimg, hipStream_t s);
bool pw_b16_ok(int prec, int K, int sw);
struct PwTail {
    int kind = 0;
    int H = 0, W = 0;
    int k = 0, pt = 0, pl = 0, act = 0;
    const float* w = nullptr; const float* bias = nullptr;
    float* out = nullptr;
    float* partial = nullptr;
    int PY = 0, tiles_w = 0, tiles = 0, tchunks = 0;
};
int pw_tail_rows(int wm);
bool pw_tail_ok(const PwParams& p, const PwTail& t, int nt, int wm);
bool pw_tail_fills(const PwParams& p, int nt, int wm);
void launch_pw_tail(const PwParams& p, const PwTail& t, const uint16_t* Wimg, int nt, int wm, hipStream_t s);
bool pw_b16s_ok(const PwParams& p);
void launch_pw_b16s(const PwParams& p, const uint16_t* Wimg, int Npad, hipStream_t s);
void launch_pw_b16(const PwParams& p, const uint16_t* Wimg, int nt, int wm , int Npad, int nblk_n, unsigned nblk, hipStream_t s);
bool pw_lat_ok(const PwParams& p);
void launch_pw_lat(const PwParams& p, const uint16_t* Wimg, int Npad, hipStream_t s);
bool pw_ws_ok(const PwParams& p);
bool pw_ws_fills(const PwParams& p);
void launch_pw_ws(const PwParams& p, const uint16_t* Wimg, int Npad, hipStream_t s);

struct DwParams {
    const float* in; const float* w ; const float* bias; float* out;
    int B, H, W, C, Ho, Wo, kh, kw, sh, sw, pt, pl, act;
    int in_bf16 = 0, out_bf16 = 0;
};
int dwconv_sum_slabs(const DwParams& p);
bool dwconv_tile_geometry(const DwParams& p, int* PY, int* tiles_w, int* tiles, int* tchunks);
void launch_dwconv(const DwParams& p, float* partial, hipStream_t s);

bool expdw_supported(int k, int s, int Cin, int Cmid, int act_e = 0, int prec = 0);
struct ExpDwGeo { int k, s, H, W, Ho, Wo, pt, pl; bool stem = false; int skw = 0; };
int expdw_skw(int Cin, int act_e, bool stem);
bool expdw_sk_pipe16(int Cin, int act_e, bool stem, int prec, bool have_image);
int expdw_sum_slabs(const ExpDwGeo& g);
int expdw_num_shapes();
bool expdw_shape_fits(int idx, const ExpDwGeo& g, bool planning = true);
int expdw_shape_slabs(int idx, const ExpDwGeo& g);
bool expdw_fullwidth(int idx, const ExpDwGeo& g);
int expdw_default_shape(const ExpDwGeo& g);
int expdw_max_slabs(const ExpDwGeo& g);
struct StemGeom { int Hin, Win, pt, pl; };
int expdw_kw(int Cin);
int expdw_cp(int Cmid);
void launch_expand_dw(const float* x, const float* we, const float* be, const float* wd, const float* bd, float* y,
                      float* partial, int B, int H, int W, int Cin, int Cmid, int Ho, int Wo, int k, int s, int pt,
                      int pl, int act_e, int act_d, int shape ,
                      const StemGeom* stem ,
                      hipStream_t st, const uint16_t* wep = nullptr ,
                      int prec = 0 ,
                      int out_bf16 = 0 ,
                      int in_bf16 = 0 );
bool dwconv_lds_supported(const DwParams& p);
void launch_dwconv_lds(const DwParams& p, float* partial, int shape, hipStream_t st);
bool expdw_bx_ok(int Cin);
int expdw_kp(int Cin);
std::vector<uint16_t> expdw_bx_image(const float* We , int Cmid, int Cin);

int mean_splits(int HW);
int mean_partial_py(int C);
void launch_mean_partial(const float* in, float* partial, int B, int HW, int C, int S, hipStream_t s);
void launch_mean_finish(const float* partial, float* out, int B, int HW, int C, int S, hipStream_t s);

struct SeParams {
    const float* partial; int S; int HW;
    const float* w1; const float* b1;
    const float* w2; const float* b2;
    float* scale;
    int B, C, Cr, act1, act2;
    int threads = 0;
};
void launch_se(const SeParams& p, hipStream_t s);

void launch_unary(const float* in, float* out, size_t n, int act, hipStream_t s);
void launch_binary(const float* a, const float* b, float* out, size_t n, int op , int mode,
                   int HW, int C, int act, hipStream_t s);

enum UnaryOp : int { U_ABS = 200, U_SQRT, U_RSQRT, U_LOG, U_EXP, U_NEG, U_SQUARE, U_TANH, U_LEAKY_RELU, U_ELU, U_SIN, U_COS,
                     U_FLOOR, U_CEIL, U_ROUND, U_RELU_N1_TO_1, U_LOGISTIC, U_RELU, U_RELU6, U_HARD_SWISH, U_GELU, U_GELU_TANH };
enum BinaryOp : int { B_ADD = 0, B_MUL = 1, B_SUB = 2, B_DIV = 3, B_POW = 4, B_MAX = 5, B_MIN = 6, B_SQDIFF = 7 };
enum ReduceOp : int { R_SUM = 0, R_MEAN = 1, R_MAX = 2, R_MIN = 3, R_PROD = 4 };
void launch_unary_op(const float* in, float* out, size_t n, int op, float alpha, hipStream_t s);
struct BcastParams {
    const float* a; const float* b; float* out;
    int d[4]; long sa[4], sb[4]; long bsa, bsb;
    int op, act;
};
void launch_binary_bcast(const BcastParams& p, int n_clips, hipStream_t s);
struct CopyParams {
    const float* in; float* out;
    int d[4]; long si[4], so[4]; long offi, offo, bsi, bso;
};
void launch_copy_view(const CopyParams& p, int n_clips, hipStream_t s);
void launch_fill(float* out, size_t n, float v, hipStream_t s);
struct PoolParams { const float* in; float* out; int B, H, W, C, Ho, Wo, kh, kw, sh, sw, pt, pl, mode , act; };
void launch_pool2d(const PoolParams& p, hipStream_t s);
void launch_softmax_rows(const float* in, float* out, size_t rows, int n, float beta, hipStream_t s);
struct ReduceParams { const float* in; float* out; int d[4]; int mask ; int op; };
void launch_reduce(const ReduceParams& p, int n_clips, hipStream_t s);
struct GenConvParams {
    const float* in; const float* w; const float* bias; float* out;
    int B, H, W, Cin, Ho, Wo, Cout, kh, kw, sh, sw, dh, dw, pt, pl, act, depthwise, mult;
};
void launch_conv_generic(const GenConvParams& p, hipStream_t s);

void launch_activation(const float* logits, float* conf, int n_clips, int n_classes, int activation, double sens,
                       hipStream_t s);
void launch_topk(const float* conf, int n_clips, int n_classes, int k, float* out_conf, int32_t* out_idx,
                 hipStream_t s);

std::vector<double> us_twiddle_table(int fft_size);
void launch_us_frame_power(const void* samples , int pcm16, int n_clips, int n, int fft_size,
                           int hop, int frames, int split_bin, const double* d_tw, double* powers , hipStream_t s);
void launch_us_cv(const double* powers, int n_clips, int frames, double* cv, hipStream_t s);

}
```

### birdnet-go_amd/csrc/planner.cpp

```cpp
#include "engine.h"

#include <algorithm>
#include <cmath>
#include <cstdio>
#include <cstdlib>
#include <cstring>
#include <map>

#include "../../include/bnhip.h"

namespace bnhip {

namespace {

size_t align_up(size_t v, size_t a) { return (v + a - 1) / a * a; }

struct Planner {
    const TflModel& m;
    std::vector<int> producer;
    std::vector<std::vector<int>> consumers;
    std::vector<int> uses;
    std::vector<char> absorbed;
    std::string err;

// ... 1389 lines not shown
                } else {
                    off_of(v) = top; top += need;
                }
            }
        }
    }
    return top;
}

}

int pw_switches_from_env() {
    auto sw = [](const char* name, int off, int force) {
        const char* e = getenv(name);
        return !e ? 0 : e[0] == '0' ? off : e[0] == '2' ? force : 0;
    };
    return sw("BNHIP_PW_B16", PW_SW_B16_OFF, PW_SW_B16_FORCE) | sw("BNHIP_PW_B16S", PW_SW_B16S_OFF, PW_SW_B16S_FORCE) |
           sw("BNHIP_PW_WS", PW_SW_WS_OFF, PW_SW_WS_FORCE) | sw("BNHIP_PW_LAT", PW_SW_LAT_OFF, 0) |
           sw("BNHIP_PW_TAIL", PW_SW_TAIL_OFF, PW_SW_TAIL_FORCE);
}

void Engine::mark_tails() {
    for (auto& s : steps) s.tail = 0;
    if (precision != 0 || (pw_sw & PW_SW_TAIL_OFF)) return;
    const int ns = (int)steps.size();
    for (int si = 0; si + 1 < ns; si++) {
        Step& s = steps[si];
        if (s.kind != S_PW || !s.bx || s.in1 >= 0 || s.in2 >= 0 || s.out < 0 || s.out == v_logits || s.out == v_emb || vals[s.out].external) continue;
        int readers = 0;
        for (int k = 0; k < ns; k++)
            for (int v : {steps[k].in0, steps[k].in1, steps[k].in2}) readers += v == s.out;
        if (readers != 1 || steps[si + 1].in0 != s.out) continue;
        const Step& c = steps[si + 1];
        PwTail t;
        t.H = s.H; t.W = s.W;
        if (c.kind == S_DW && c.sh == 1 && c.sw == 1 && c.kh == c.kw && (c.kh == 3 || c.kh == 5) && c.Ho == c.H && c.Wo == c.W && c.H == s.H && c.W == s.W &&
            c.C == s.Co && c.Co == s.Co && c.pt == (c.kh - 1) / 2 && c.pl == (c.kw - 1) / 2) {
            t.kind = 2; t.k = c.kh; t.pt = c.pt; t.pl = c.pl; t.act = c.act;
        } else if (c.kind == S_MEAN_PARTIAL && si + 2 < ns && steps[si + 2].kind == S_MEAN_FINISH && steps[si + 2].in0 == c.out && c.C == s.Co) {
            t.kind = 1;
        } else continue;
        PwParams p{nullptr, nullptr, nullptr, nullptr, nullptr, nullptr, s.H * s.W, s.Co, s.C, s.H * s.W, s.act};
        p.prec = precision; p.sw = pw_sw;
        int want_wm = 0, want_nt = 6;
        if (const char* e = getenv("BNHIP_PW_TAIL_FORM")) { if (sscanf(e, "%d,%d", &want_wm, &want_nt) != 2) { want_wm = 0; want_nt = 6; } }
        int fit = 0, forced_fit = 0;
        for (int wm : {14, 13, 15}) if (pw_tail_ok(p, t, 6, wm)) { if (!fit) fit = wm; if (wm == want_wm && pw_tail_ok(p, t, want_nt, wm)) forced_fit = wm; }
        if (!fit) continue;
        s.tail = t.kind;
        if (pw_sw & PW_SW_TAIL_FORCE) { s.wm = s.wm_full = forced_fit ? forced_fit : fit; s.nt = s.nt_full = forced_fit ? want_nt : 6; }
    }
}

bool Engine::build(TflModel m, int dev, int maxb, bool plan_only, std::string* err, int* code) {
    device = dev;
    max_batch = maxb;
    pw_sw = pw_switches_from_env();
    if (const char* e = getenv("BNHIP_NORM_RESIDENT")) norm_resident = atoi(e) != 0;
    const PlanSwitches sw;
    *code = BNHIP_E_UNSUPPORTED;
    if (!run_graph_passes(&m, err)) return false;
    if (!select_outputs(m, &logits_output, &embedding_output)) {
        *code = BNHIP_E_INVALID;
        *err = "logits_output / embedding_output do not name two distinct graph outputs";
        return false;
    }
    Lowering L(*this, m, sw);
    if (!L.input_values() || !L.match_frontends() || !L.frontend() || !L.ops() || !L.bind_outputs()) {
        *err = L.err; *code = L.code;
        return false;
    }
    tensor_value = L.tv;
    mark_tails();
    find_norm_pair();

    mark_liveness(vals, steps);
    if (v_emb >= 0) vals[v_emb].last = (int)steps.size();
    for (const Value& v : vals)
        if (v.elems * (size_t)max_batch >= ((size_t)1 << 31)) {
            *err = "max_batch too large for this model: a " + std::to_string(v.elems) + "-element activation times " +
                   std::to_string(max_batch) + " clips exceeds 32-bit indexing";
            *code = BNHIP_E_INVALID;
            return false;
        }
    n_lanes = std::max(1, std::min(n_lanes, kMaxLanes));
    lane_cap = (max_batch + n_lanes - 1) / n_lanes;
    act_bytes = plan_arena(vals, steps, (size_t)max_batch, false, no_reuse);
    lane_bytes = n_lanes > 1 ? align_up(plan_arena(vals, steps, (size_t)lane_cap, true, no_reuse), 256) : 0;
    act_bytes = std::max(act_bytes, lane_bytes * (size_t)n_lanes);
    pick_split();

    w_bytes = L.w.img.size() * sizeof(float);
    if (plan_only) { device = -1; *code = BNHIP_OK; return true; }
    return bind_device(L.w, err, code);
}

}
```

### birdnet-go_amd/csrc/pw_b16.hip

```cpp
#include "pw_common.h"

#include <algorithm>
#include <atomic>

namespace bnhip {

#ifdef B16_TRACE
__device__ long long* g_b16_trace = nullptr;
#define B16_TRACE_SLOTS 160
#define B16_T(i) do { if (lane == 0 && L < 64u && (i) < B16_TRACE_SLOTS) g_b16_trace[((size_t)L * 4 + wave) * B16_TRACE_SLOTS + (i)] = clock64(); } while (0)
#else
#define B16_T(i) do { } while (0)
#endif

constexpr int pw_tail_group(int NT, int BM, int budget) {
    int g = 1;
    for (int c = 1; c <= NT; c++)
        if (NT % c == 0 && BM * (20 * c + 4) <= budget) g = c;
    return g;
}
template <int NT, int WM, int NW, int EPI, int LDSF>
__device__ __forceinline__ void pw_tail_epilogue(const PwParams& p, const PwTail& te, f32x4 (&acc)[NT][WM], float* lds, int m0, int n0) {
    constexpr int NTHR = 64 * NW, BM = 16 * WM * NW;
    constexpr int G = pw_tail_group(NT, BM, LDSF), NG = NT / G, GC = 16 * G, RS = GC + 4, Q = 4 * G;
// ... 110 lines not shown
                            if (wo >= W) continue;
                            const float4 v = a4[a][c];
                            out4[(size_t)(ho * W + wo) * C4] = v;
                            sum.x += v.x; sum.y += v.y; sum.z += v.z; sum.w += v.w;
                        }
                    }
                }
                reinterpret_cast<float4*>(red)[it] = sum;
            }
            __syncthreads();
            if (te.partial) {
                const int PY = te.PY, tchunks = te.tchunks;
                for (int it = tid; it < clips * tchunks * Q; it += NTHR) {
                    const int q = it % Q, rest = it / Q, tc = rest % tchunks, cl = rest / tchunks;
                    const int c4 = (ng0 >> 2) + q;
                    if (c4 >= C4) continue;
                    float4 t = make_float4(0.f, 0.f, 0.f, 0.f);
                    for (int y = 0; y < PY; y++) {
                        const int tile = tc * PY + y;
                        if (tile >= tiles) break;
                        const float4 v = reinterpret_cast<const float4*>(red)[(cl * tiles + tile) * Q + q];
                        t.x += v.x; t.y += v.y; t.z += v.z; t.w += v.w;
                    }
                    reinterpret_cast<float4*>(te.partial)[((size_t)(b0 + cl) * tchunks + tc) * C4 + c4] = t;
                }
            }
        }
    }
}

template <bool ABF, bool SCR, int WM = 2> struct ASet { ARaw<ABF> a[WM < 2 ? 2 : WM]; };
template <bool ABF, int WM> struct ASet<ABF, true, WM> { ARaw<ABF> a[WM < 2 ? 2 : WM]; float4 slo[WM < 2 ? 2 : WM], shi[WM < 2 ? 2 : WM]; };

template <int NT, bool SC, bool ABF, bool SCL = false, int WM = 2, bool SIX = false, int NW = 4, int EPI = 0>
__global__ __launch_bounds__(64 * NW) void k_pw_b16(PwParams p, const uint16_t* __restrict__ Wimg, int Npad, int nblk_n, unsigned nblk,
                                                     FDiv dn, FDiv dhw, PwTail tail) {
    static_assert(!SCL || SC, "SCL is a form of SC");
    static_assert(!SIX || !ABF, "fp32 engines keep fp32 activations");
    static_assert(EPI == 0 || (SIX && !SC), "the fused tails: six-product form without a scale");
    constexpr bool SCR = SC && !SCL;
    constexpr int NTHR = 64 * NW;
    constexpr int BM = 16 * WM * NW, BN = 16 * NT;
    constexpr int NP = SIX ? 3 : 1;
    constexpr int WSLOTS = NP * 4 * BN;
    constexpr int WQ = (WSLOTS + NTHR - 1) / NTHR;
    constexpr int SCLIPS = BM / 16 + 1;
    constexpr int SBUF = SCL ? SCLIPS * 32 : 0;
    constexpr int OBUF = WSLOTS * 4 + SBUF;
    constexpr int STG = 4 * 16 * (BN + 4);
    constexpr int LDSN = (EPI != 0 || 2 * OBUF > STG) ? 2 * OBUF : STG;
    __shared__ __attribute__((aligned(16))) float lds[LDSN];
    const int tid = threadIdx.x, lane = tid & 63, wave = tid >> 6;
    const int li = lane & 15, kq = lane >> 4;
    const unsigned L = xcd_remap(blockIdx.x, nblk);
    const int mblk = (int)fdiv(L, dn);
    const int m0 = mblk * BM;
    const int n0 = ((int)L - mblk * nblk_n) * BN;
    const int K = p.K;
    const int nslab = (K + 31) >> 5;

    unsigned aoff[WM], soff[SC ? WM : 1];
    const int b_first = SCL ? (int)fdiv((unsigned)m0, dhw) : 0;
#pragma unroll
    for (int mt = 0; mt < WM; mt++) {
        const int m = min(m0 + 16 * WM * wave + 16 * mt + li, p.M - 1);
        aoff[mt] = (unsigned)m * (unsigned)K + 4u * (unsigned)kq;
        if (SC) {
            const unsigned b = fdiv((unsigned)m, dhw);
            soff[SC ? mt : 0] = SCL ? (unsigned)(((int)b - b_first) * 32 + 4 * kq)
                                    : b * (unsigned)K + 4u * (unsigned)kq;
        }
    }
    unsigned woff[WQ];
#pragma unroll
    for (int q = 0; q < WQ; q++) {
        const int slot = min(tid + NTHR * q, WSLOTS - 1);
        const int kqs = slot / BN, r = slot - kqs * BN;
        woff[q] = (unsigned)kqs * (unsigned)Npad + (unsigned)min(n0 + r, Npad - 1);
    }
    const u32x4* W16 = reinterpret_cast<const u32x4*>(Wimg);
    const uint16_t* A16 = reinterpret_cast<const uint16_t*>(p.A);
    const int sclip = tid >> 3, sk4 = tid & 7;
    const int nclips_blk = SCL ? (int)fdiv((unsigned)(min(m0 + BM, p.M) - 1), dhw) - b_first + 1 : 0;

    ASet<ABF, SCR, WM> set0, set1;
    u32x4 wreg[WQ];
    float4 sreg;
    auto aload = [&](int sl, auto& st) {
        const int k0 = sl * 32;
        const bool inlo = k0 + 4 * kq < K, inhi = k0 + 16 + 4 * kq < K;
#pragma unroll
        for (int mt = 0; mt < WM; mt++) {
            if constexpr (ABF) {
                const uint16_t* ap = A16 + aoff[mt] + k0;
                st.a[mt].lo = inlo ? *reinterpret_cast<const u32x2*>(ap) : (u32x2){0u, 0u};
                st.a[mt].hi = inhi ? *reinterpret_cast<const u32x2*>(ap + 16) : (u32x2){0u, 0u};
            } else {
                const float* ap = p.A + aoff[mt] + k0;
                st.a[mt].lo = inlo ? *reinterpret_cast<const float4*>(ap) : make_float4(0.f, 0.f, 0.f, 0.f);
                st.a[mt].hi = inhi ? *reinterpret_cast<const float4*>(ap + 16) : make_float4(0.f, 0.f, 0.f, 0.f);
            }
            if constexpr (SCR) {
                const float* sp = p.ascale + soff[mt] + k0;
                st.slo[mt] = inlo ? *reinterpret_cast<const float4*>(sp) : make_float4(0.f, 0.f, 0.f, 0.f);
                st.shi[mt] = inhi ? *reinterpret_cast<const float4*>(sp + 16) : make_float4(0.f, 0.f, 0.f, 0.f);
            }
        }
// ... 63 lines not shown
        if constexpr (SIX) {
            u32x4 wfr[2][3];
#pragma unroll
            for (int pl3 = 0; pl3 < 3; pl3++) wfr[0][pl3] = Wl[(pl3 * 4 + kq) * BN + li];
#pragma unroll
            for (int t = 0; t < NT; t++) {
                if (t + 1 < NT) {
#pragma unroll
                    for (int pl3 = 0; pl3 < 3; pl3++) wfr[(t + 1) & 1][pl3] = Wl[(pl3 * 4 + kq) * BN + 16 * (t + 1) + li];
                }
                const bf16x8 wh = __builtin_bit_cast(bf16x8, wfr[t & 1][0]);
                const bf16x8 wm = __builtin_bit_cast(bf16x8, wfr[t & 1][1]);
                const bf16x8 wl = __builtin_bit_cast(bf16x8, wfr[t & 1][2]);
#pragma unroll
                for (int mt = 0; mt < WM; mt++) acc[t][mt] = bx3_mfma6(acc[t][mt], wh, wm, wl, ah[mt], am[SIX ? mt : 0], al[SIX ? mt : 0]);
            }
        } else {
            bf16x8 wf[NT];
#pragma unroll
            for (int t = 0; t < NT; t++) wf[t] = __builtin_bit_cast(bf16x8, Wl[kq * BN + 16 * t + li]);
#pragma unroll
            for (int t = 0; t < NT; t++)
#pragma unroll
                for (int mt = 0; mt < WM; mt++) acc[t][mt] = __builtin_amdgcn_mfma_f32_16x16x32_bf16(wf[t], ah[mt], acc[t][mt], 0, 0, 0);
        }
        B16_T(10 + 4 * sl);
        __syncthreads();
        B16_T(11 + 4 * sl);
    };
    B16_T(0);
    aload(0, set0);
    if (nslab > 1) aload(1, set1);
    wload(0);
    wstore(0);
    if (nslab > 1) wload(1);
    B16_T(1);
    __syncthreads();
    B16_T(2);
    for (int sl = 0; sl < nslab; sl += 2) {
        slab(sl, set0);
        if (sl + 1 < nslab) slab(sl + 1, set1);
    }
    B16_T(3);
    if constexpr (EPI == 0) pw_epilogue<NT, WM>(p, acc, lds, m0, n0);
    else pw_tail_epilogue<NT, WM, NW, EPI, 2 * OBUF>(p, tail, acc, lds, m0, n0);
    B16_T(4);
}

static std::atomic<long> g_pw_b16_launches{0};

template <int NT, int NS, bool SC, bool ABF>
__global__ __launch_bounds__(256) void k_pw_b16s(PwParams p, const uint16_t* __restrict__ Wimg, int Npad, int tiles_per_wave, FDiv dhw) {
    const int lane = threadIdx.x & 63, li = lane & 15, kq = lane >> 4;
    const int wave_g = blockIdx.x * 4 + (threadIdx.x >> 6);
    const int K = p.K, N = p.N;
    const int ntiles = (p.M + 15) >> 4;
    const int t0 = wave_g * tiles_per_wave, t1 = min(t0 + tiles_per_wave, ntiles);
    if (t0 >= t1) return;
    const u32x4* W16 = reinterpret_cast<const u32x4*>(Wimg);
    bf16x8 wf[NS][NT];
#pragma unroll
    for (int ns = 0; ns < NS; ns++)
#pragma unroll
        for (int t = 0; t < NT; t++) wf[ns][t] = __builtin_bit_cast(bf16x8, W16[((size_t)ns * 12 + kq) * Npad + min(16 * t + li, Npad - 1)]);
    f32x4 bias[NT];
#pragma unroll
    for (int t = 0; t < NT; t++) {
        bias[t] = (f32x4){0.f, 0.f, 0.f, 0.f};
        const int n = 16 * t + 4 * kq;
        if (p.bias && n + 3 < N) { const float4 b4 = *reinterpret_cast<const float4*>(p.bias + n); bias[t] = (f32x4){b4.x, b4.y, b4.z, b4.w}; }
    }
    const uint16_t* A16 = reinterpret_cast<const uint16_t*>(p.A);
    bool inlo[NS], inhi[NS];
#pragma unroll
    for (int ns = 0; ns < NS; ns++) { inlo[ns] = 32 * ns + 4 * kq < K; inhi[ns] = 32 * ns + 16 + 4 * kq < K; }
    ARaw<ABF> cur[NS], nxt[NS];
    auto aload = [&](int tile, ARaw<ABF> (&dst)[NS]) {
        const int m = min(16 * tile + li, p.M - 1);
        const size_t off = (size_t)m * K + 4 * kq;
#pragma unroll
        for (int ns = 0; ns < NS; ns++) {
            if constexpr (ABF) {
                dst[ns].lo = inlo[ns] ? *reinterpret_cast<const u32x2*>(A16 + off + 32 * ns) : (u32x2){0u, 0u};
                dst[ns].hi = inhi[ns] ? *reinterpret_cast<const u32x2*>(A16 + off + 32 * ns + 16) : (u32x2){0u, 0u};
            } else {
                dst[ns].lo = inlo[ns] ? *reinterpret_cast<const float4*>(p.A + off + 32 * ns) : make_float4(0.f, 0.f, 0.f, 0.f);
                dst[ns].hi = inhi[ns] ? *reinterpret_cast<const float4*>(p.A + off + 32 * ns + 16) : make_float4(0.f, 0.f, 0.f, 0.f);
            }
        }
    };
    float4 slo[SC ? NS : 1], shi[SC ? NS : 1];
    int sclip = -1;
    aload(t0, cur);
    for (int tile = t0; tile < t1; tile++) {
        if (tile + 1 < t1) aload(tile + 1, nxt);
        if constexpr (SC) {
            const int b = (int)fdiv((unsigned)min(16 * tile, p.M - 1), dhw);
            if (b != sclip) {
                sclip = b;
                const float* sp = p.ascale + (size_t)b * K + 4 * kq;
#pragma unroll
                for (int ns = 0; ns < NS; ns++) {
                    slo[ns] = inlo[ns] ? *reinterpret_cast<const float4*>(sp + 32 * ns) : make_float4(0.f, 0.f, 0.f, 0.f);
                    shi[ns] = inhi[ns] ? *reinterpret_cast<const float4*>(sp + 32 * ns + 16) : make_float4(0.f, 0.f, 0.f, 0.f);
                }
            }
        }
// ... 142 lines not shown
```

### birdnet-go_amd/csrc/pw_bx3.hip

```cpp
#include "kernels.h"
#include "pw_common.h"

#include <algorithm>
#include <type_traits>
#include <vector>

namespace bnhip {

template <int NT, bool SC, int WM>
__global__ __launch_bounds__(256) void k_pw_bx3(PwParams p, const uint16_t* __restrict__ Wimg, int Npad, int nblk_n, unsigned nblk,
                                                 FDiv dn, FDiv dhw) {
    constexpr int BM = 64 * WM;
    constexpr int XQ = BM * PW_C4 / 256;
    constexpr int WSLOTS = 12 * NT * 16;
    constexpr int WQ = (WSLOTS + 255) / 256;
    constexpr int TILE_F = BM * PW_LS + WSLOTS * 4;
    constexpr int STG = 4 * 16 * (NT * 16 + 4);
    constexpr int LDSN = TILE_F > STG ? TILE_F : STG;
    __shared__ __attribute__((aligned(16))) float lds[LDSN];
    const int tid = threadIdx.x, lane = tid & 63, wave = tid >> 6;
    const int li = lane & 15, kq = lane >> 4;
    const unsigned L = xcd_remap(blockIdx.x, nblk);
    const int mblk = (int)fdiv(L, dn);
    const int m0 = mblk * BM;
    const int n0 = ((int)L - mblk * nblk_n) * (NT * 16);
    const int K = p.K;

    unsigned xoff[XQ], soff[SC ? XQ : 1], woff[WQ];
    const bool one = p.prec == 1;
    const int wslots = one ? WSLOTS / 3 : WSLOTS;
    const int kc4 = 4 * (tid % PW_C4);
    const int lbase = (tid / PW_C4) * PW_LS + 4 * (tid % PW_C4);
    constexpr int LQ = (256 / PW_C4) * PW_LS;
#pragma unroll
    for (int q = 0; q < XQ; q++) {
        const int idx = tid + 256 * q, row = idx / PW_C4, c4 = idx % PW_C4;
        const int m = min(m0 + row, p.M - 1);
        xoff[q] = (unsigned)m * (unsigned)K + 4 * c4;
        if (SC) soff[SC ? q : 0] = fdiv((unsigned)m, dhw) * (unsigned)K + 4 * c4;
    }
#pragma unroll
    for (int q = 0; q < WQ; q++) {
        const int slot = min(tid + 256 * q, WSLOTS - 1);
        const int plkq = slot / (NT * 16), r = slot - plkq * (NT * 16);
        woff[q] = (unsigned)plkq * (unsigned)Npad + (unsigned)min(n0 + r, Npad - 1);
    }
    float4 xreg[XQ], sreg[SC ? XQ : 1];
    u32x4 wreg[WQ];
    const u32x4* W16 = reinterpret_cast<const u32x4*>(Wimg);
    constexpr int XH = XQ / 2;
    constexpr int LQH = 64 * PW_LS;
    if (p.a_bf16) {
#pragma unroll
        for (int q = 0; q < XH; q++) {
            const int row = (tid >> 2) + 64 * q;
            const int m = min(m0 + row, p.M - 1);
            xoff[q] = (unsigned)m * (unsigned)K + 8u * (unsigned)(tid & 3);
            if (SC) soff[SC ? q : 0] = fdiv((unsigned)m, dhw) * (unsigned)K + 8u * (unsigned)(tid & 3);
        }
    }
    auto gload = [&](int sl) {
        const float* Ak = p.A + sl * PW_BK;
        const bool kin = sl * PW_BK + kc4 < K;
        if (p.a_bf16) {
            const bool kinh = sl * PW_BK + 8 * (tid & 3) < K;
            const uint16_t* A16 = reinterpret_cast<const uint16_t*>(p.A) + sl * PW_BK;
#pragma unroll
            for (int q = 0; q < XH; q++) {
                xreg[q] = kinh ? *reinterpret_cast<const float4*>(A16 + xoff[q]) : make_float4(0.f, 0.f, 0.f, 0.f);
                if (SC) {
                    const float* sp = p.ascale + sl * PW_BK + soff[SC ? q : 0];
                    sreg[SC ? 2 * q : 0] = kinh ? *reinterpret_cast<const float4*>(sp) : make_float4(0.f, 0.f, 0.f, 0.f);
                    sreg[SC ? 2 * q + 1 : 0] = kinh ? *reinterpret_cast<const float4*>(sp + 4) : make_float4(0.f, 0.f, 0.f, 0.f);
                }
            }
// ... 57 lines not shown
                ah[mt] = bx1_cvt8(*reinterpret_cast<const f32x4*>(xr), *reinterpret_cast<const f32x4*>(xr + 16));
            }
#pragma unroll
            for (int t = 0; t < NT; t++) {
                const bf16x8 wh = __builtin_bit_cast(bf16x8, Wl[kq * (NT * 16) + 16 * t + li]);
#pragma unroll
                for (int mt = 0; mt < WM; mt++) acc[t][mt] = __builtin_amdgcn_mfma_f32_16x16x32_bf16(wh, ah[mt], acc[t][mt], 0, 0, 0);
            }
        } else {
#pragma unroll
        for (int mt = 0; mt < WM; mt++) {
            const float* xr = &lds[(16 * WM * wave + 16 * mt + li) * PW_LS + 4 * kq];
            const f32x4 x0 = *reinterpret_cast<const f32x4*>(xr), x1 = *reinterpret_cast<const f32x4*>(xr + 16);
            bx3_split8(x0, x1, &ah[mt], &am[mt], &al[mt]);
        }
        u32x4 wfr[2][3];
#pragma unroll
        for (int pl3 = 0; pl3 < 3; pl3++) wfr[0][pl3] = Wl[(pl3 * 4 + kq) * (NT * 16) + li];
#pragma unroll
        for (int t = 0; t < NT; t++) {
            if (t + 1 < NT) {
#pragma unroll
                for (int pl3 = 0; pl3 < 3; pl3++) wfr[(t + 1) & 1][pl3] = Wl[(pl3 * 4 + kq) * (NT * 16) + 16 * (t + 1) + li];
            }
            const bf16x8 wh = __builtin_bit_cast(bf16x8, wfr[t & 1][0]);
            const bf16x8 wm = __builtin_bit_cast(bf16x8, wfr[t & 1][1]);
            const bf16x8 wl = __builtin_bit_cast(bf16x8, wfr[t & 1][2]);
#pragma unroll
            for (int mt = 0; mt < WM; mt++) acc[t][mt] = bx3_mfma6(acc[t][mt], wh, wm, wl, ah[mt], am[mt], al[mt]);
        }
        }
        if (sl + 1 < nslab) {
            __syncthreads();
            lstore();
            if (sl + 2 < nslab) gload(sl + 2);
        }
        __syncthreads();
    }
    pw_epilogue<NT, WM>(p, acc, lds, m0, n0);
}

template <int NT, bool SC, int WM>
__global__ __launch_bounds__(256) void k_pw_bx3p(PwParams p, const uint16_t* __restrict__ Wimg, int Npad, int nblk_n, unsigned nblk,
                                                  FDiv dn, FDiv dhw) {
    constexpr int BM = 64 * WM;
    constexpr int XQ = BM * PW_C4 / 256;
    constexpr int WSLOTS = 12 * NT * 16;
    constexpr int WQ = (WSLOTS + 255) / 256;
    constexpr int TILE_F = BM * PW_LS + WSLOTS * 4;
    extern __shared__ __attribute__((aligned(16))) float bx3p_lds[];
    float* lds = bx3p_lds;
    const int tid = threadIdx.x, lane = tid & 63, wave = tid >> 6;
    const int li = lane & 15, kq = lane >> 4;
    const unsigned L = xcd_remap(blockIdx.x, nblk);
    const int mblk = (int)fdiv(L, dn);
    const int m0 = mblk * BM;
    const int n0 = ((int)L - mblk * nblk_n) * (NT * 16);
    const int K = p.K;

    unsigned xoff[XQ], soff[SC ? XQ : 1], woff[WQ];
    const bool one = p.prec == 1;
    const int wslots = one ? WSLOTS / 3 : WSLOTS;
    const int kc4 = 4 * (tid % PW_C4);
    const int lbase = (tid / PW_C4) * PW_LS + 4 * (tid % PW_C4);
    constexpr int LQ = (256 / PW_C4) * PW_LS;
#pragma unroll
    for (int q = 0; q < XQ; q++) {
        const int idx = tid + 256 * q, row = idx / PW_C4, c4 = idx % PW_C4;
        const int m = min(m0 + row, p.M - 1);
        xoff[q] = (unsigned)m * (unsigned)K + 4 * c4;
        if (SC) soff[SC ? q : 0] = fdiv((unsigned)m, dhw) * (unsigned)K + 4 * c4;
    }
#pragma unroll
    for (int q = 0; q < WQ; q++) {
        const int slot = min(tid + 256 * q, WSLOTS - 1);
        const int plkq = slot / (NT * 16), r = slot - plkq * (NT * 16);
        woff[q] = (unsigned)plkq * (unsigned)Npad + (unsigned)min(n0 + r, Npad - 1);
    }
    float4 xreg[XQ], sreg[SC ? XQ : 1];
    u32x4 wreg[WQ];
    const u32x4* W16 = reinterpret_cast<const u32x4*>(Wimg);
    constexpr int XH = XQ / 2;
    constexpr int LQH = 64 * PW_LS;
    if (p.a_bf16) {
#pragma unroll
        for (int q = 0; q < XH; q++) {
            const int row = (tid >> 2) + 64 * q;
            const int m = min(m0 + row, p.M - 1);
            xoff[q] = (unsigned)m * (unsigned)K + 8u * (unsigned)(tid & 3);
            if (SC) soff[SC ? q : 0] = fdiv((unsigned)m, dhw) * (unsigned)K + 8u * (unsigned)(tid & 3);
        }
    }
    auto gload = [&](int sl) {
        const float* Ak = p.A + sl * PW_BK;
        const bool kin = sl * PW_BK + kc4 < K;
        if (p.a_bf16) {
            const bool kinh = sl * PW_BK + 8 * (tid & 3) < K;
            const uint16_t* A16 = reinterpret_cast<const uint16_t*>(p.A) + sl * PW_BK;
#pragma unroll
            for (int q = 0; q < XH; q++) {
                xreg[q] = kinh ? *reinterpret_cast<const float4*>(A16 + xoff[q]) : make_float4(0.f, 0.f, 0.f, 0.f);
                if (SC) {
                    const float* sp = p.ascale + sl * PW_BK + soff[SC ? q : 0];
                    sreg[SC ? 2 * q : 0] = kinh ? *reinterpret_cast<const float4*>(sp) : make_float4(0.f, 0.f, 0.f, 0.f);
                    sreg[SC ? 2 * q + 1 : 0] = kinh ? *reinterpret_cast<const float4*>(sp + 4) : make_float4(0.f, 0.f, 0.f, 0.f);
                }
            }
// ... 155 lines not shown
```

### birdnet-go_amd/csrc/pw_gemm.hip

```cpp
#include "kernels.h"
#include "pw_common.h"

#include <algorithm>
#include <type_traits>
#include <cstdlib>

namespace bnhip {

#ifdef PW_TRACE
__device__ long long* g_pw_trace = nullptr;
#define PW_TRACE_SLOTS 128
#define PW_T(i) do { if (lane == 0 && L < 64u && (i) < PW_TRACE_SLOTS && !((i) >= 60 && (i) < 64)) g_pw_trace[((size_t)L * 4 + wave) * PW_TRACE_SLOTS + (i)] = clock64(); } while (0)
#else
#define PW_T(i) do { } while (0)
#endif
struct ImGeo {
    int H, W, Cin, kw, sh, sw, dh, dw, pt, pl, Wo;
    FDiv d_cin, d_kw, d_wo, d_howo;
};
template <int NT, bool SC, int WM, bool IM = false>
__global__ __launch_bounds__(256) void k_pw_gemm(PwParams p, int nblk_n, unsigned nblk, FDiv dn, FDiv dhw, ImGeo g) {
    constexpr int BM = 64 * WM;
    constexpr int XQ = BM * PW_C4 / 256;
    constexpr int TILE = (BM + NT * 16) * PW_LS;
    constexpr int STG = 4 * 16 * (NT * 16 + 4);
    constexpr int LDSN = TILE > STG ? TILE : STG;
    __shared__ __attribute__((aligned(16))) float lds[LDSN];
    constexpr int WQ = (NT * 16 * PW_C4 + 255) / 256;
    const int tid = threadIdx.x, lane = tid & 63, wave = tid >> 6;
    const int li = lane & 15, kq = lane >> 4;
    const unsigned L = xcd_remap(blockIdx.x, nblk);
    const int mblk = (int)fdiv(L, dn);
    const int m0 = mblk * BM;
    const int n0 = ((int)L - mblk * nblk_n) * (NT * 16);
    const int K = p.K;

    float4 xreg[XQ], wreg[WQ], sreg[SC ? XQ : 1];
    int srow[SC ? XQ : 1];
    if (SC) {
#pragma unroll
        for (int q = 0; q < XQ; q++) {
            int m = m0 + ((tid + 256 * q) / PW_C4);
            srow[SC ? q : 0] = (int)fdiv((unsigned)(m < p.M ? m : 0), dhw);
        }
    }
    int ih0[IM ? XQ : 1], iw0[IM ? XQ : 1]; unsigned ibase[IM ? XQ : 1];
    if (IM) {
#pragma unroll
        for (int q = 0; q < XQ; q++) {
            const unsigned m = (unsigned)min(m0 + (tid + 256 * q) / PW_C4, p.M - 1);
            const unsigned b = fdiv(m, g.d_howo), pix = m - b * g.d_howo.d;
            const unsigned oh = fdiv(pix, g.d_wo), ow = pix - oh * (unsigned)g.Wo;
            ih0[IM ? q : 0] = (int)oh * g.sh - g.pt; iw0[IM ? q : 0] = (int)ow * g.sw - g.pl;
            ibase[IM ? q : 0] = b * (unsigned)(g.H * g.W);
        }
    }
    auto gload = [&](int k0) {
#pragma unroll
        for (int q = 0; q < XQ; q++) {
            int idx = tid + 256 * q;
            int row = idx / PW_C4, c4 = idx % PW_C4;
            int m = m0 + row, k = k0 + 4 * c4;
            float4 v = make_float4(0.f, 0.f, 0.f, 0.f), sc = make_float4(0.f, 0.f, 0.f, 0.f);
            if (IM) {
                if (m < p.M && k < K) {
                    const unsigned tap = fdiv((unsigned)k, g.d_cin), ci = (unsigned)k - tap * (unsigned)g.Cin;
                    const unsigned ti = fdiv(tap, g.d_kw), tj = tap - ti * (unsigned)g.kw;
                    const int ih = ih0[IM ? q : 0] + (int)ti * g.dh, iw = iw0[IM ? q : 0] + (int)tj * g.dw;
                    if (ih >= 0 && ih < g.H && iw >= 0 && iw < g.W)
                        v = *reinterpret_cast<const float4*>(p.A + ((size_t)ibase[IM ? q : 0] + (size_t)ih * g.W + iw) * g.Cin + ci);
                }
            } else if (m < p.M && k < K) {
                v = *reinterpret_cast<const float4*>(p.A + (size_t)m * K + k);
                if (SC) sc = *reinterpret_cast<const float4*>(p.ascale + (size_t)srow[SC ? q : 0] * K + k);
            }
            xreg[q] = v;
            if (SC) sreg[SC ? q : 0] = sc;
        }
#pragma unroll
        for (int q = 0; q < WQ; q++) {
            int idx = tid + 256 * q;
            int row = idx / PW_C4, c4 = idx % PW_C4;
            int n = n0 + row, k = k0 + 4 * c4;
            float4 v = make_float4(0.f, 0.f, 0.f, 0.f);
// ... 35 lines not shown
        PW_T(4 + 4 * sl);
        const float* Xs = lds;
        const float* Ws = Xs + BM * PW_LS;
#pragma unroll
        for (int t16 = 0; t16 < PW_BK / 16; t16++) {
            f32x4 xf[WM], wf[NT];
#pragma unroll
            for (int mt = 0; mt < WM; mt++)
                xf[mt] = *reinterpret_cast<const f32x4*>(&Xs[(16 * WM * wave + 16 * mt + li) * PW_LS + 16 * t16 + 4 * kq]);
#pragma unroll
            for (int t = 0; t < NT; t++)
                wf[t] = *reinterpret_cast<const f32x4*>(&Ws[(16 * t + li) * PW_LS + 16 * t16 + 4 * kq]);
#pragma unroll
            for (int sidx = 0; sidx < 4; sidx++) {
#pragma unroll
                for (int t = 0; t < NT; t++)
#pragma unroll
                    for (int mt = 0; mt < WM; mt++)
                        acc[t][mt] = __builtin_amdgcn_mfma_f32_16x16x4f32(wf[t][sidx], xf[mt][sidx], acc[t][mt], 0, 0, 0);
            }
        }
        PW_T(5 + 4 * sl);
        if (sl + 1 < nslab) {
            __syncthreads();
            PW_T(6 + 4 * sl);
#ifdef PW_TRACE
            __builtin_amdgcn_s_waitcnt(0x0f70);
            PW_T(64 + 2 * sl);
#endif
            lstore();
#ifdef PW_TRACE
            __builtin_amdgcn_s_waitcnt(0xc07f);
            PW_T(65 + 2 * sl);
#endif
            if (sl + 2 < nslab) gload((sl + 2) * PW_BK);
            PW_T(7 + 4 * sl);
        }
        __syncthreads();
    }
    PW_T(2);

    pw_epilogue<NT, WM>(p, acc, lds, m0, n0);
    PW_T(3);
}

template <int NT, bool SC, int WM>
__global__ __launch_bounds__(256) void k_pw_pipe(PwParams p, int nblk_n, unsigned nblk, FDiv dn, FDiv dhw) {
    constexpr int BM = 64 * WM;
    constexpr int XQ = BM * PW_C4 / 256, WQ = (NT * 16 * PW_C4 + 255) / 256;
    constexpr int TILE = (BM + NT * 16) * PW_LS;
    __shared__ __attribute__((aligned(16))) float lds[2 * TILE];
    const int tid = threadIdx.x, lane = tid & 63, wave = tid >> 6;
    const int li = lane & 15, kq = lane >> 4;
    const unsigned L = xcd_remap(blockIdx.x, nblk);
    const int mblk = (int)fdiv(L, dn);
    const int m0 = mblk * BM;
    const int n0 = ((int)L - mblk * nblk_n) * (NT * 16);
    const int K = p.K;

    unsigned xoff[XQ], soff[SC ? XQ : 1], woff[WQ];
    const int lbase = (tid / PW_C4) * PW_LS + 4 * (tid % PW_C4);
    constexpr int LQ = (256 / PW_C4) * PW_LS;
#pragma unroll
    for (int q = 0; q < XQ; q++) {
        const int idx = tid + 256 * q, row = idx / PW_C4, c4 = idx % PW_C4;
        const int m = min(m0 + row, p.M - 1);
        xoff[q] = (unsigned)m * (unsigned)K + 4 * c4;
        if (SC) soff[SC ? q : 0] = fdiv((unsigned)m, dhw) * (unsigned)K + 4 * c4;
    }
#pragma unroll
    for (int q = 0; q < WQ; q++) {
        const int idx = tid + 256 * q, row = min(idx / PW_C4, NT * 16 - 1), c4 = idx % PW_C4;
        woff[q] = (unsigned)min(n0 + row, p.N - 1) * (unsigned)K + 4 * c4;
    }
    float4 xreg[XQ], wreg[WQ], sreg[SC ? XQ : 1];
    auto gload = [&](int k0) {
        const float* Ak = p.A + k0;
        const float* Wk = p.W + k0;
#pragma unroll
        for (int q = 0; q < XQ; q++) {
            xreg[q] = *reinterpret_cast<const float4*>(Ak + xoff[q]);
            if (SC) sreg[SC ? q : 0] = *reinterpret_cast<const float4*>(p.ascale + k0 + soff[SC ? q : 0]);
        }
#pragma unroll
        for (int q = 0; q < WQ; q++) wreg[q] = *reinterpret_cast<const float4*>(Wk + woff[q]);
    };
    auto lstore = [&](float* buf) {
#pragma unroll
        for (int q = 0; q < XQ; q++) {
            float4 v = xreg[q];
            if (SC) { const float4 sc = sreg[SC ? q : 0]; v.x *= sc.x; v.y *= sc.y; v.z *= sc.z; v.w *= sc.w; }
            *reinterpret_cast<float4*>(&buf[lbase + q * LQ]) = v;
        }
#pragma unroll
        for (int q = 0; q < WQ; q++)
            if ((NT * 16 * PW_C4) % 256 == 0 || (tid + 256 * q) / PW_C4 < NT * 16)
                *reinterpret_cast<float4*>(&buf[BM * PW_LS + lbase + q * LQ]) = wreg[q];
    };

    f32x4 acc[NT][WM];
#pragma unroll
    for (int t = 0; t < NT; t++)
#pragma unroll
        for (int mt = 0; mt < WM; mt++) acc[t][mt] = (f32x4){0.f, 0.f, 0.f, 0.f};

    const int nslab = K / PW_BK;
    gload(0);
// ... 2 lines not shown
    __syncthreads();
    auto slab = [&](int sl, auto DS, auto DL) {
        const float* Xs = lds + (sl & 1) * TILE;
        const float* Ws = Xs + BM * PW_LS;
        float* nxt = lds + ((sl + 1) & 1) * TILE;
#pragma unroll
        for (int t16 = 0; t16 < PW_BK / 16; t16++) {
            f32x4 xf[WM], wf[NT];
#pragma unroll
            for (int mt = 0; mt < WM; mt++)
                xf[mt] = *reinterpret_cast<const f32x4*>(&Xs[(16 * WM * wave + 16 * mt + li) * PW_LS + 16 * t16 + 4 * kq]);
#pragma unroll
            for (int t = 0; t < NT; t++)
                wf[t] = *reinterpret_cast<const f32x4*>(&Ws[(16 * t + li) * PW_LS + 16 * t16 + 4 * kq]);
            if (t16 == 0 && decltype(DS)::value) lstore(nxt);
            if (t16 == PW_BK / 16 - 1 && decltype(DL)::value) gload((sl + 2) * PW_BK);
#pragma unroll
            for (int sidx = 0; sidx < 4; sidx++) {
#pragma unroll
                for (int t = 0; t < NT; t++)
#pragma unroll
                    for (int mt = 0; mt < WM; mt++)
                        acc[t][mt] = __builtin_amdgcn_mfma_f32_16x16x4f32(wf[t][sidx], xf[mt][sidx], acc[t][mt], 0, 0, 0);
            }
            constexpr int NMF = 4 * NT * WM, NREF = XQ + WQ, STEP = NMF / (NREF + 1) > 0 ? NMF / (NREF + 1) : 1;
            __builtin_amdgcn_sched_group_barrier(0x100, WM + NT, 0);
            if (t16 == 0 && decltype(DS)::value) {
#pragma unroll
                for (int r = 0; r < NREF; r++) {
                    __builtin_amdgcn_sched_group_barrier(0x008, STEP, 0);
                    if (SC) __builtin_amdgcn_sched_group_barrier(0x002, 4, 0);
                    __builtin_amdgcn_sched_group_barrier(0x200, 1, 0);
                }
            }
            if (t16 == PW_BK / 16 - 1 && decltype(DL)::value) {
#pragma unroll
                for (int r = 0; r < NREF + (SC ? XQ : 0); r++) {
                    __builtin_amdgcn_sched_group_barrier(0x008, SC ? 1 : STEP, 0);
                    __builtin_amdgcn_sched_group_barrier(0x020, 1, 0);
                }
            }
        }
        __syncthreads();
    };
    int sl = 0;
    for (; sl + 2 < nslab; sl++) slab(sl, std::true_type{}, std::true_type{});
    if (nslab >= 2) { slab(sl, std::true_type{}, std::false_type{}); sl++; }
    slab(sl, std::false_type{}, std::false_type{});

    pw_epilogue<NT, WM>(p, acc, lds, m0, n0);
}

__global__ void k_pw_naive(PwParams p) {
    size_t idx = (size_t)blockIdx.x * blockDim.x + threadIdx.x;
    if (idx >= (size_t)p.M * p.N) return;
    int n = (int)(idx % p.N);
    size_t m = idx / p.N;
    float acc = 0.f;
    for (int k = 0; k < p.K; k++) {
        float a = p.A[m * p.K + k];
        if (p.ascale) a *= p.ascale[(m / p.HW) * p.K + k];
        acc = fmaf(a, p.W[(size_t)n * p.K + k], acc);
    }
    if (p.bias) acc += p.bias[n];
    acc = apply_act(acc, p.act);
    if (p.res) acc += p.res[idx];
    p.out[idx] = acc;
}

bool pw_pipe_ok(int nt, int wm, int K) { return K % PW_BK == 0 && nt >= 1 && nt <= 4 && 2 * (64 * wm + 16 * nt) * PW_LS * 4 <= 64 * 1024; }
static int pick_nt(int M, int N) {
    (void)M;
    long best_cols = -1;
    for (int nt = 1; nt <= 4; nt++) {
        long cols = (long)((N + nt * 16 - 1) / (nt * 16)) * nt * 16;
        if (best_cols < 0 || cols < best_cols) best_cols = cols;
    }
    int best = 1;
    for (int nt = 1; nt <= 4; nt++) {
        long cols = (long)((N + nt * 16 - 1) / (nt * 16)) * nt * 16;
        if (cols * 100 <= best_cols * 115) best = nt;
    }
    static const int ov = getenv("BNHIP_PW_NT") ? atoi(getenv("BNHIP_PW_NT")) : 0;
    if (ov >= 1 && ov <= 8) best = ov;
    return best;
}

int pw_default_nt(int M, int N) { return pick_nt(M, N); }

bool pw_fill_grid(int M, int N, int* nt, int* wm, PwGrid* g) {
    static const int target_env = getenv("BNHIP_PW_FILL") ? atoi(getenv("BNHIP_PW_FILL")) : -1;
    const int target = target_env >= 0 ? target_env : device_cus();
    bool changed = false;
    while ((int)g->nblk < target && (*wm > 1 || *nt > 1)) {
        if (*wm > 1) *wm = 1;
        else *nt = (*nt + 1) / 2;
        changed = true;
        *g = pw_grid(M, N, *nt, *wm);
    }
    return changed;
}

void launch_pw_gemm(const PwParams& p, hipStream_t s) {
    if ((p.K & 3) != 0) {
        size_t total = (size_t)p.M * p.N;
        hipLaunchKernelGGL(k_pw_naive, dim3((unsigned)((total + 255) / 256)), dim3(256), 0, s, p);
        return;
// ... 47 lines not shown
```

### birdnet-go_amd/csrc/pw_ws.hip

```cpp
#include "pw_common.h"

#include <algorithm>
#include <atomic>

namespace bnhip {

__device__ __forceinline__ void ws_pair(const float4& lo, const float4& hi, int q, float& x0, float& x1) {
    x0 = q == 0 ? lo.x : q == 1 ? lo.z : q == 2 ? hi.x : hi.z;
    x1 = q == 0 ? lo.y : q == 1 ? lo.w : q == 2 ? hi.y : hi.w;
}

struct WsFrag { u32x4 h, m, l; };

template <int WM, bool SIX>
__device__ __forceinline__ void ws_mfma(f32x4 (&c)[WM], const u32x4 (&w)[SIX ? 3 : 1], const WsFrag (&f)[2]) {
    const bf16x8 wh = __builtin_bit_cast(bf16x8, w[0]);
    if constexpr (SIX) {
        const bf16x8 wm = __builtin_bit_cast(bf16x8, w[1]), wl = __builtin_bit_cast(bf16x8, w[2]);
#pragma unroll
        for (int mt = 0; mt < WM; mt++) c[mt] = __builtin_amdgcn_mfma_f32_16x16x32_bf16(wl, __builtin_bit_cast(bf16x8, f[mt].h), c[mt], 0, 0, 0);
#pragma unroll
        for (int mt = 0; mt < WM; mt++) c[mt] = __builtin_amdgcn_mfma_f32_16x16x32_bf16(wh, __builtin_bit_cast(bf16x8, f[mt].l), c[mt], 0, 0, 0);
#pragma unroll
        for (int mt = 0; mt < WM; mt++) c[mt] = __builtin_amdgcn_mfma_f32_16x16x32_bf16(wm, __builtin_bit_cast(bf16x8, f[mt].m), c[mt], 0, 0, 0);
#pragma unroll
        for (int mt = 0; mt < WM; mt++) c[mt] = __builtin_amdgcn_mfma_f32_16x16x32_bf16(wm, __builtin_bit_cast(bf16x8, f[mt].h), c[mt], 0, 0, 0);
#pragma unroll
        for (int mt = 0; mt < WM; mt++) c[mt] = __builtin_amdgcn_mfma_f32_16x16x32_bf16(wh, __builtin_bit_cast(bf16x8, f[mt].m), c[mt], 0, 0, 0);
    }
#pragma unroll
    for (int mt = 0; mt < WM; mt++) c[mt] = __builtin_amdgcn_mfma_f32_16x16x32_bf16(wh, __builtin_bit_cast(bf16x8, f[mt].h), c[mt], 0, 0, 0);
}

__device__ __forceinline__ void ws_store(const PwParams& p, f32x4 v, const float* bias, int m, int n) {
    const bool vec = (p.N & 3) == 0;
    if (n >= p.N) return;
    if (bias) {
        if (vec) { const float4 b4 = *reinterpret_cast<const float4*>(bias + n); v += (f32x4){b4.x, b4.y, b4.z, b4.w}; }
        else {
#pragma unroll
            for (int r = 0; r < 4; r++) if (n + r < p.N) v[r] += bias[n + r];
        }
    }
    if (p.act == ACT_SWISH) v = swish4(v);
    else if (p.act != ACT_NONE) { v[0] = apply_act(v[0], p.act); v[1] = apply_act(v[1], p.act); v[2] = apply_act(v[2], p.act); v[3] = apply_act(v[3], p.act); }
    const size_t o = (size_t)m * p.N + n;
    if (vec) {
        if (p.res) {
            const float4 rv = p.res_bf16 ? bf16x4_load(p.res, o >> 2) : *reinterpret_cast<const float4*>(p.res + o);
            v[0] += rv.x; v[1] += rv.y; v[2] += rv.z; v[3] += rv.w;
        }
        if (p.out_bf16) bf16x4_store(p.out, o >> 2, make_float4(v[0], v[1], v[2], v[3]));
        else *reinterpret_cast<float4*>(p.out + o) = make_float4(v[0], v[1], v[2], v[3]);
    } else {
#pragma unroll
        for (int r = 0; r < 4; r++)
            if (n + r < p.N) p.out[o + r] = v[r] + (p.res ? p.res[o + r] : 0.f);
    }
}

static std::atomic<long> g_pw_ws_launches{0};

template <int NT, int NS, int R, bool SIX, bool ABF, int NW>
__global__ __launch_bounds__(64 * NW) void k_pw_ws(PwParams p, const uint16_t* __restrict__ Wimg, int Npad, int nblk_n, unsigned nblk,
                                                    unsigned GW , FDiv dn) {
    static_assert(NS % R == 0 && R < NS, "the register ring must divide the slab count (slab s of every tile lives in set s % R)");
    static_assert(!SIX || !ABF, "fp32 engines keep fp32 activations");
    constexpr int BN = 16 * NT, NP = SIX ? 3 : 1;
    constexpr int WSLOTS = NS * NP * 4 * BN;
    extern __shared__ __attribute__((aligned(16))) unsigned char ws_lds[];
    u32x4* Wl = reinterpret_cast<u32x4*>(ws_lds);
    float* Bl = reinterpret_cast<float*>(ws_lds + (size_t)WSLOTS * 16);
    const int tid = threadIdx.x, lane = tid & 63, li = lane & 15, kq = lane >> 4;
    const int wave = __builtin_amdgcn_readfirstlane(tid >> 6);
    const unsigned L = xcd_remap(blockIdx.x, nblk);
    const int g = (int)fdiv(L, dn);
    const int n0 = ((int)L - g * nblk_n) * BN;
    const int K = p.K, N = p.N;
#ifdef WS_TRACE
    long long* trc = reinterpret_cast<long long*>(const_cast<float*>(p.res)) + ((size_t)blockIdx.x * NW + wave) * 32;
    int tslot = 0;
    p.res = nullptr;
    if (lane == 0) trc[30] = wall_clock64();
#define WS_T() do { if (lane == 0 && tslot < 29) trc[tslot] = clock64(); tslot++; } while (0)
#else
#define WS_T() do { } while (0)
#endif
    WS_T();
    const u32x4* W16 = reinterpret_cast<const u32x4*>(Wimg);
    {
        constexpr int WQ = (WSLOTS + 64 * NW - 1) / (64 * NW);
        u32x4 wv[WQ];
#pragma unroll
        for (int i = 0; i < WQ; i++) {
            const int slot = min(tid + 64 * NW * i, WSLOTS - 1);
            const int r = slot % BN, q = slot / BN;
            const int kqs = q & 3, pl = (q >> 2) % NP, sl = (q >> 2) / NP;
            wv[i] = W16[((size_t)sl * 12 + pl * 4 + kqs) * Npad + min(n0 + r, Npad - 1)];
        }
#pragma unroll
        for (int i = 0; i < WQ; i++)
            if (tid + 64 * NW * i < WSLOTS) Wl[tid + 64 * NW * i] = wv[i];
    }
    for (int c = tid; c < BN; c += 64 * NW) Bl[c] = (p.bias && n0 + c < N) ? p.bias[n0 + c] : 0.f;
    __syncthreads();
    WS_T();

    const unsigned mt16 = (unsigned)(p.M + 15) >> 4;
    const unsigned gw = (unsigned)g * NW + (unsigned)wave;
    const int t0 = (int)(gw * mt16 / GW), t1 = (int)((gw + 1) * mt16 / GW);
    if (t0 >= t1) return;

    const uint16_t* A16 = reinterpret_cast<const uint16_t*>(p.A);
    auto rows = [&](int tile, unsigned (&off)[2]) {
#pragma unroll
        for (int mt = 0; mt < 2; mt++) off[mt] = (unsigned)min(16 * (tile + mt) + li, p.M - 1) * (unsigned)K + 4u * (unsigned)kq;
    };
    auto aload = [&](const unsigned (&off)[2], int ns, ARaw<ABF> (&dst)[2]) {
        const bool last = ns == NS - 1;
        const bool inlo = !last || 32 * ns + 4 * kq < K, inhi = !last || 32 * ns + 16 + 4 * kq < K;
        const int klo = inlo ? 32 * ns : 32 * ns - 4 * kq, khi = inhi ? 32 * ns + 16 : 32 * ns - 4 * kq;
#pragma unroll
        for (int mt = 0; mt < 2; mt++) {
            if constexpr (ABF) {
                const uint16_t* ap = A16 + off[mt];
                const u32x2 lo = *reinterpret_cast<const u32x2*>(ap + klo), hi = *reinterpret_cast<const u32x2*>(ap + khi);
                dst[mt].lo = inlo ? lo : (u32x2){0u, 0u};
                dst[mt].hi = inhi ? hi : (u32x2){0u, 0u};
// ... 282 lines not shown
```

### birdnet-go_amd/csrc/stft.hip

```cpp
#include "kernels.h"
#include "fft_r8.h"

#include <hip/hip_runtime.h>

#include <algorithm>
#include <vector>
#include <cmath>
#include <cstdio>
#include <cstdlib>

namespace bnhip {

__global__ void k_normalize(const float* __restrict__ x, const float2* __restrict__ mm, float* __restrict__ out,
                            int n_samples, float norm_sub, float norm_mul) {
    const int b = blockIdx.y;
    const float2 m = mm[b];
    const float* xc = x + (size_t)b * n_samples;
    float* oc = out + (size_t)b * n_samples;
    for (int i = blockIdx.x * blockDim.x + threadIdx.x; i < n_samples; i += gridDim.x * blockDim.x) {
        float t = xc[i] - m.x;
        t = t / m.y;
        t = t - norm_sub;
        oc[i] = t * norm_mul;
    }
}
void launch_normalize(const float* x, const float2* mm, float* out, int n_clips, int n_samples, float norm_sub,
                      float norm_mul, hipStream_t s) {
    dim3 grid((n_samples + 256 * 8 - 1) / (256 * 8), n_clips);
    hipLaunchKernelGGL(k_normalize, grid, dim3(256), 0, s, x, mm, out, n_samples, norm_sub, norm_mul);
}

__device__ __forceinline__ float mel_pow(float v, float p1, float p2);
__device__ __forceinline__ float mel_log(float v, float lfloor, float lscale);

template <int P, int W, bool MEL = false, typename R = double>
__global__ __launch_bounds__(64 * W) void k_stft_bins(StftParams p) {
    constexpr int N2 = 64 * P;
    constexpr int N = 2 * N2;
    constexpr int Q = 64 / P;
    constexpr int RS = P == 8 ? 66 : 65;
    constexpr int WSZ = P * RS;
    constexpr int NPAIR = (P * P + 63) / 64;
    extern __shared__ __attribute__((aligned(16))) unsigned char stft_sm[];
    R* sm = reinterpret_cast<R*>(stft_sm);
    R* twr = sm;
    R* twi = twr + P * 64;
    R* t2r = twi + P * 64;
    R* t2i = t2r + Q * P;
    R* work = t2i + Q * P;
    float4* melw4 = reinterpret_cast<float4*>(work + (size_t)W * 2 * WSZ);
    const int* binq = reinterpret_cast<const int*>(melw4 + p.mel_quads);
    const int tid = threadIdx.x, lane = tid & 63, wave = tid >> 6;
    const int b = blockIdx.y;

    constexpr int NTAB = 2 * P * 64 + 2 * Q * P;
    for (int i = tid; i < NTAB; i += blockDim.x) sm[i] = (R)p.tw[i];
    int mA = 0, loA = 0, nA = 0, wA = 0, mB = 0, loB = 0, nB = 0, wB = 0;
    if (MEL) {
        const float4* src = reinterpret_cast<const float4*>(p.mel + 64 * 8);
        for (int i = tid; i < p.mel_quads + (p.mel_quads + 3) / 4; i += blockDim.x) melw4[i] = src[i];
        const int4* lt = reinterpret_cast<const int4*>(p.mel) + 2 * lane;
        const int4 ta = lt[0], tb = lt[1];
        mA = ta.x; loA = ta.y; nA = ta.z; wA = ta.w; mB = tb.x; loB = tb.y; nB = tb.z; wB = tb.w;
    }
    __syncthreads();

    R* wre = work + (size_t)wave * 2 * WSZ;
    R* wim = wre + WSZ;
    const float* xc = p.xn + (size_t)b * p.n_samples;
    float w0[P], w1[P];
#pragma unroll
    for (int n1 = 0; n1 < P; n1++) {
        int n = 128 * n1 + 2 * lane;
        w0[n1] = n < p.L ? p.window[n] : 0.f;
        w1[n1] = n + 1 < p.L ? p.window[n + 1] : 0.f;
    }
    const int k1b = lane % P, qb = lane / P;
    constexpr int NBL = 8;
    int ka_[NBL], kb_[NBL];
    R trr[NBL], tri[NBL];
#pragma unroll
    for (int t = 0; t < NBL; t++) {
        int idx = lane + 64 * t;
        int k = idx < p.nb ? p.bins[idx] : 0;
        ka_[t] = k % N2; kb_[t] = (N2 - k % N2) % N2;
        const bool in = idx < p.nb_cap;
        trr[t] = in ? (R)p.tw[NTAB + idx] : (R)1.0;
        tri[t] = in ? (R)p.tw[NTAB + p.nb_cap + idx] : (R)0.0;
    }

    const int f_begin = (blockIdx.x * W + wave) * p.fpw;
    const int f_end = min(f_begin + p.fpw, p.F);
    float2 nx[P];
    auto fetch = [&](int f) {
        const int first = f * p.hop - p.pad_left;
        const int s0 = first + 2 * lane;
        if (first >= 0 && first + N <= p.n_samples && (first & 1) == 0) {
#pragma unroll
            for (int n1 = 0; n1 < P; n1++)
                nx[n1] = 128 * n1 < p.L ? *reinterpret_cast<const float2*>(xc + s0 + 128 * n1) : make_float2(0.f, 0.f);
        } else {
#pragma unroll
            for (int n1 = 0; n1 < P; n1++) {
                int s = s0 + 128 * n1;
                float2 v = make_float2(0.f, 0.f);
                if (128 * n1 < p.L) {
                    if (s >= 0 && s < p.n_samples) v.x = xc[s];
                    if (s + 1 >= 0 && s + 1 < p.n_samples) v.y = xc[s + 1];
                }
                nx[n1] = v;
            }
        }
    };
    if (f_begin < f_end) fetch(f_begin);
    for (int f = f_begin; f < f_end; f++) {
        R re[P], im[P];
#pragma unroll
        for (int n1 = 0; n1 < P; n1++) {
            re[n1] = (R)(nx[n1].x * w0[n1]);
            im[n1] = (R)(nx[n1].y * w1[n1]);
        }
        if (f + 1 < f_end) fetch(f + 1);
        fft_regs<P, R>(re, im);
#pragma unroll
        for (int k1 = 0; k1 < P; k1++) {
            const R c = twr[k1 * 64 + lane], s = twi[k1 * 64 + lane];
            const R r = fma(re[k1], c, -(im[k1] * s)), i2 = fma(re[k1], s, im[k1] * c);
            wre[k1 * RS + lane] = r; wim[k1 * RS + lane] = i2;
        }
        __builtin_amdgcn_s_waitcnt(0xc07f);
        __builtin_amdgcn_wave_barrier();
#pragma unroll
        for (int j = 0; j < P; j++) { re[j] = wre[k1b * RS + Q * j + qb]; im[j] = wim[k1b * RS + Q * j + qb]; }
        __builtin_amdgcn_s_waitcnt(0xc07f);
        __builtin_amdgcn_wave_barrier();
        fft_regs<P, R>(re, im);
#pragma unroll
        for (int j = 0; j < P; j++) {
            const R c = t2r[qb * P + j], s = t2i[qb * P + j];
            const R r = fma(re[j], c, -(im[j] * s)), i2 = fma(re[j], s, im[j] * c);
            const int slot = j * P + k1b;
            wre[qb * (P * P) + slot] = r; wim[qb * (P * P) + slot] = i2;
        }
        __builtin_amdgcn_s_waitcnt(0xc07f);
// ... 245 lines not shown
    if (p2 == 1.0f) return y;
    if (y >= 0.0f) return y == 0.0f ? 0.0f : __builtin_amdgcn_exp2f(p2 * __builtin_amdgcn_logf(y));
    return powf(y, p2);
}
__device__ __forceinline__ float mel_log(float v, float lfloor, float lscale) {
    return lscale * (0.6931471805599453f * __builtin_amdgcn_logf(fmaxf(v, lfloor)));
}
template <int C>
__global__ __launch_bounds__(256) void k_mel_finish(MelFinParams p) {
    __shared__ float tile[C][32][33];
    const int b = blockIdx.z, f0 = blockIdx.x * 32, m0 = blockIdx.y * 32;
    const int tx = threadIdx.x & 31, ty = threadIdx.x >> 5;
#pragma unroll
    for (int c = 0; c < C; c++)
        for (int r = ty; r < 32; r += 8) {
            int f = f0 + r, m = m0 + tx;
            float v = 0.f;
            if (f < p.F && m < p.n_mels) {
                const float t = p.T[c][((size_t)b * p.F + f) * p.ldt + m];
                v = p.log ? mel_log(t, p.lfloor, p.lscale) : mel_pow(t, p.p1[c], p.p2[c]);
            }
            tile[c][r][tx] = v;
        }
    __syncthreads();
    if (p.time_major) {
        for (int r = ty; r < 32; r += 8) {
            int f = f0 + r, m = m0 + tx;
            if (f < p.F && m < p.n_mels) {
                float* o = p.out + (((size_t)b * p.F + f) * p.n_mels + m) * p.Ctot + p.c0;
                if (C == 2) *reinterpret_cast<float2*>(o) = make_float2(tile[0][r][tx], tile[1][r][tx]);
                else o[0] = tile[0][r][tx];
            }
        }
        return;
    }
    for (int r = ty; r < 32; r += 8) {
        int m = m0 + r, f = f0 + tx;
        if (f < p.F && m < p.n_mels) {
            float* o = p.out + (((size_t)b * p.n_mels + m) * p.F + f) * p.Ctot + p.c0;
            if (C == 2) *reinterpret_cast<float2*>(o) = make_float2(tile[0][tx][r], tile[1][tx][r]);
            else o[0] = tile[0][tx][r];
        }
    }
}
#define MSP_F 8
template <int C, int VAR = 0>
__global__ __launch_bounds__(256) void k_mel_banded(MelBandParams p) {
    extern __shared__ __attribute__((aligned(16))) float msm[];
    float* rows[2];
    rows[0] = msm;
    rows[1] = msm + (size_t)MSP_F * p.nbp[0];
    float* tile = rows[C - 1] + (size_t)MSP_F * p.nbp[C - 1];
    const int TS = p.n_mels + 1;
    const int b = blockIdx.y, f0 = blockIdx.x * MSP_F, nf = min(MSP_F, p.F - f0), tid = threadIdx.x, nthr = blockDim.x;
#pragma unroll
    for (int c = 0; c < C; c++) {
        const float4* src = reinterpret_cast<const float4*>(p.bins[c] + ((size_t)b * p.F + f0) * p.nbp[c]);
        float4* dst = reinterpret_cast<float4*>(rows[c]);
        const int n4 = nf * p.nbp[c] / 4, n4all = MSP_F * p.nbp[c] / 4;
        for (int base = 0; base < n4all; base += 4 * nthr) {
            float4 v[4];
#pragma unroll
            for (int j = 0; j < 4; j++) {
                const int i = base + tid + nthr * j;
                v[j] = i < n4 ? src[i] : make_float4(0.f, 0.f, 0.f, 0.f);
            }
#pragma unroll
            for (int j = 0; j < 4; j++) {
                const int i = base + tid + nthr * j;
                if (i < n4all) dst[i] = v[j];
            }
        }
    }
    __syncthreads();
    const int m = tid >> 1, g = tid & 1;
    if (m < p.n_mels) {
#pragma unroll
        for (int c = 0; c < C; c++) {
            const int lo = p.span[c][2 * m], hi = p.span[c][2 * m + 1], ld = p.nbp[c];
            const float4* wr = reinterpret_cast<const float4*>(p.w[c] + (size_t)m * ld);
            const float* L = rows[c] + (size_t)(g * (MSP_F / 2)) * ld;
            float acc[MSP_F / 2];
#pragma unroll
            for (int i = 0; i < MSP_F / 2; i++) acc[i] = 0.f;
            const int k4e = (hi + 3) >> 2, k4max = ld / 4 - 1;
            for (int k4 = lo >> 2; k4 < k4e; k4 += 4) {
                float4 w4[4];
#pragma unroll
                for (int j = 0; j < 4; j++) w4[j] = wr[min(k4 + j, k4max)];
#pragma unroll
                for (int j = 0; j < 4; j++) {
                    if (k4 + j < k4e) {
#pragma unroll
                        for (int i = 0; i < MSP_F / 2; i++) {
                            const float4 x4 = *reinterpret_cast<const float4*>(L + (size_t)i * ld + 4 * (k4 + j));
                            if (VAR == 2) asm volatile("s_waitcnt lgkmcnt(0)" ::: "memory");
                            if (VAR == 1) {
                                asm volatile("v_fmac_f32 %0, %1, %2" : "+v"(acc[i]) : "v"(x4.x), "v"(w4[j].x));
                                asm volatile("v_fmac_f32 %0, %1, %2" : "+v"(acc[i]) : "v"(x4.y), "v"(w4[j].y));
                                asm volatile("v_fmac_f32 %0, %1, %2" : "+v"(acc[i]) : "v"(x4.z), "v"(w4[j].z));
                                asm volatile("v_fmac_f32 %0, %1, %2" : "+v"(acc[i]) : "v"(x4.w), "v"(w4[j].w));
                            } else
                            acc[i] = fmaf(x4.w, w4[j].w, fmaf(x4.z, w4[j].z, fmaf(x4.y, w4[j].y, fmaf(x4.x, w4[j].x, acc[i]))));
                        }
                    }
                }
            }
// ... 49 lines not shown
```

Baseline: 78600 clips/s.

## Alternate block traversal direction between producer and consumer kernels for cache reuse

```diff
diff --git a/birdnet-go_amd/csrc/conv.hip b/birdnet-go_amd/csrc/conv.hip
--- a/birdnet-go_amd/csrc/conv.hip
+++ b/birdnet-go_amd/csrc/conv.hip
@@ -9,7 +9,7 @@
 __global__ __launch_bounds__(256) void k_conv_direct(ConvParams p) {
     const int C4 = p.Cout >> 2;
     size_t total = (size_t)p.B * p.Ho * p.Wo * C4;
-    size_t idx = (size_t)blockIdx.x * 256 + threadIdx.x;
+    size_t idx = (size_t)traverse_index(blockIdx.x, gridDim.x, p.back) * 256 + threadIdx.x;
     if (idx >= total) return;
     int c4 = (int)(idx % C4);
     size_t pix = idx / C4;
@@ -46,7 +46,7 @@
 __global__ __launch_bounds__(256) void k_conv_direct_t(ConvParams p) {
     const int C4 = p.Cout >> 2;
     size_t total = (size_t)p.B * p.Ho * p.Wo * C4;
-    size_t idx = (size_t)blockIdx.x * 256 + threadIdx.x;
+    size_t idx = (size_t)traverse_index(blockIdx.x, gridDim.x, p.back) * 256 + threadIdx.x;
     if (idx >= total) return;
     int c4 = (int)(idx % C4);
     size_t pix = idx / C4;
@@ -89,7 +89,7 @@
     constexpr int NCOL = (PX - 1) * S + KW;
     const int C4 = p.Cout >> 2;
     size_t total = (size_t)p.B * p.Ho * wgroups * C4;
-    size_t idx = (size_t)blockIdx.x * 256 + threadIdx.x;
+    size_t idx = (size_t)traverse_index(blockIdx.x, gridDim.x, p.back) * 256 + threadIdx.x;
     if (idx >= total) return;
     int c4 = (int)(idx % C4);
     size_t g = idx / C4;
@@ -176,6 +176,7 @@
     const float* in; const float* wm ; const float* bias ; float* out;
     int B, H, W, Ho, Wo, Cout, pt, pl, act;
     unsigned total_px, tiles_per_wave;
+    int back = 0;
 };
 template <int NTILES>
 __global__ __launch_bounds__(256) void k_stem_mfma(StemParams p) {
@@ -195,7 +196,7 @@
         bq[t] = *reinterpret_cast<const float4*>(p.bias + 16 * t + 4 * kq);
     }
     const int i0 = kq >> 1, j0 = (kq & 1) * 2;
-    const unsigned tile0 = (blockIdx.x * 4u + wave) * p.tiles_per_wave;
+    const unsigned tile0 = (traverse_index(blockIdx.x, gridDim.x, p.back) * 4u + wave) * p.tiles_per_wave;
     const unsigned hw = (unsigned)p.Ho * p.Wo;
     unsigned px = tile0 * 16u + li;
     int b, oh, ow;
@@ -275,6 +276,7 @@
     static const int stem_tpw = getenv("BNHIP_STEM_TPW") ? std::max(atoi(getenv("BNHIP_STEM_TPW")), 1) : 8;
     StemParams p{c.in, wm, bias_p, c.out, c.B, c.H, c.W, c.Ho, c.Wo, c.Cout, c.pt, c.pl, c.act,
                  (unsigned)((size_t)c.B * c.Ho * c.Wo), (unsigned)stem_tpw};
+    p.back = c.back;
     unsigned tiles = (p.total_px + 15) / 16;
     unsigned blocks = (tiles + 4 * p.tiles_per_wave - 1) / (4 * p.tiles_per_wave);
     if (c.Cout == 32) hipLaunchKernelGGL((k_stem_mfma<2>), dim3(blocks), dim3(256), 0, s, p);
diff --git a/birdnet-go_amd/csrc/dwconv.hip b/birdnet-go_amd/csrc/dwconv.hip
--- a/birdnet-go_amd/csrc/dwconv.hip
+++ b/birdnet-go_amd/csrc/dwconv.hip
@@ -10,7 +10,8 @@
 __global__ __launch_bounds__(256) void k_dwconv_t(DwParams p, int CX, int PY, int tiles_w, int tiles, int tchunks,
                                                   int cchunks, unsigned nblk, float* __restrict__ partial) {
     __shared__ float red[256 * 4];
-    const unsigned L = xcd_remap(blockIdx.x, nblk);
+    const int back = traverse_flag(p.back);
+    const unsigned L = traverse_index(xcd_remap(blockIdx.x, nblk), nblk, back);
     const int bpc = tchunks * cchunks;
     const int b = L / bpc;
     const int rest = L % bpc;
@@ -133,7 +134,7 @@
 __global__ __launch_bounds__(256) void k_dwconv(DwParams p) {
     const int CV = p.C / VEC;
     size_t total = (size_t)p.B * p.Ho * p.Wo * CV;
-    size_t idx = (size_t)blockIdx.x * 256 + threadIdx.x;
+    size_t idx = (size_t)traverse_index(blockIdx.x, gridDim.x, p.back) * 256 + threadIdx.x;
     if (idx >= total) return;
     int cv = (int)(idx % CV);
     size_t pix = idx / CV;
@@ -226,11 +227,11 @@
 int mean_splits(int HW) { return (HW + MEAN_SLAB - 1) / MEAN_SLAB; }
 
 __global__ __launch_bounds__(256) void k_mean_partial(const float* __restrict__ in, float* __restrict__ partial,
-                                                      int HW, int C, int S) {
+                                                      int HW, int C, int S, int back) {
     __shared__ float red[256];
-    const int b = blockIdx.z, sp = blockIdx.y;
+    const int b = (int)traverse_index(blockIdx.z, gridDim.z, back), sp = (int)traverse_index(blockIdx.y, gridDim.y, back);
     const int CW = blockDim.x, PY = blockDim.y;
-    const int c = blockIdx.x * CW + threadIdx.x;
+    const int c = (int)traverse_index(blockIdx.x, gridDim.x, back) * CW + threadIdx.x;
     const int p0 = sp * MEAN_SLAB, p1 = min(HW, p0 + MEAN_SLAB);
     float acc = 0.f;
     if (c < C)
@@ -248,30 +249,30 @@
     int PY = 256 / CW; if (PY < 1) PY = 1;
     return PY;
 }
-void launch_mean_partial(const float* in, float* partial, int B, int HW, int C, int S, hipStream_t s) {
+void launch_mean_partial(const float* in, float* partial, int B, int HW, int C, int S, hipStream_t s, int back) {
     int CW = C < 64 ? C : 64;
     int PY = mean_partial_py(C);
     dim3 grid((C + CW - 1) / CW, S, B);
-    hipLaunchKernelGGL(k_mean_partial, grid, dim3(CW, PY), 0, s, in, partial, HW, C, S);
-}
-__global__ void k_mean_finish(const float* __restrict__ partial, float* __restrict__ out, int B, int HW, int C, int S) {
-    size_t idx = (size_t)blockIdx.x * blockDim.x + threadIdx.x;
+    hipLaunchKernelGGL(k_mean_partial, grid, dim3(CW, PY), 0, s, in, partial, HW, C, S, back);
+}
+__global__ void k_mean_finish(const float* __restrict__ partial, float* __restrict__ out, int B, int HW, int C, int S, int back) {
+    size_t idx = (size_t)traverse_index(blockIdx.x, gridDim.x, back) * blockDim.x + threadIdx.x;
     if (idx >= (size_t)B * C) return;
     int c = (int)(idx % C); size_t b = idx / C;
     float sum = 0.f;
     for (int sidx = 0; sidx < S; sidx++) sum += partial[(b * S + sidx) * C + c];
     out[idx] = sum / (float)HW;
 }
-void launch_mean_finish(const float* partial, float* out, int B, int HW, int C, int S, hipStream_t s) {
+void launch_mean_finish(const float* partial, float* out, int B, int HW, int C, int S, hipStream_t s, int back) {
     size_t total = (size_t)B * C;
-    hipLaunchKernelGGL(k_mean_finish, dim3((unsigned)((total + 255) / 256)), dim3(256), 0, s, partial, out, B, HW, C, S);
+    hipLaunchKernelGGL(k_mean_finish, dim3((unsigned)((total + 255) / 256)), dim3(256), 0, s, partial, out, B, HW, C, S, back);
 }
 
 __global__ __launch_bounds__(1024) void k_se(SeParams p) {
     extern __shared__ __attribute__((aligned(16))) float sm[];
     float* mean = sm;
     float* r = sm + p.C;
-    const int b = blockIdx.x, tid = threadIdx.x, lane = tid & 63, wave = tid >> 6;
+    const int b = (int)traverse_index(blockIdx.x, gridDim.x, p.back), tid = threadIdx.x, lane = tid & 63, wave = tid >> 6;
     const int NTHR = blockDim.x, NW = NTHR >> 6;
     const float inv = 1.0f / (float)p.HW;
     int P = 1;
diff --git a/birdnet-go_amd/csrc/engine.cpp b/birdnet-go_amd/csrc/engine.cpp
--- a/birdnet-go_amd/csrc/engine.cpp
+++ b/birdnet-go_amd/csrc/engine.cpp
@@ -491,7 +491,7 @@
             case S_STFT: {
                 const FrontSpec& fs = specs[s.spec];
                 StftParams p{in0, fs.window_full, fs.bins, out, n_samples, fs.Lfft, fs.L, fs.hop, fs.F, fs.nb, fs.nbp, fs.mode, n, fs.stft_tw, fs.pad_left};
-                p.zmask = fs.stft_zmask;
+                p.zmask = fs.stft_zmask; p.back = s.back;
                 if (s.mode == 1) {
                     p.out = nullptr; p.img = out; p.mel = s.w3; p.mel_quads = s.S; p.n_mels = fs.n_mels; p.Ctot = C_spec; p.c0 = fs.c;
                     p.logc = fs.log_compress ? 1 : 0; p.time_major = fs.time_major ? 1 : 0; p.p1 = fs.p1; p.p2 = fs.p2;
@@ -511,6 +511,7 @@
                                 {reinterpret_cast<const int*>(s.w1), reinterpret_cast<const int*>(s.S == 2 ? s.w3 : s.w1)},
                                 {fa.nbp, fb.nbp}, {fa.p1, fb.p1}, {fa.p2, fb.p2}, out, fa.F, fa.n_mels, C_spec, fa.c,
                                 fa.log_compress ? 1 : 0, fa.log_floor, fa.log_scale, fa.time_major ? 1 : 0};
+                p.back = s.back;
                 launch_mel_banded(p, s.S, n, stream);
                 break;
             }
@@ -524,7 +525,7 @@
             }
             case S_CONV_DIRECT: {
                 ConvParams p{in0, s.w0, s.w1, out, n, s.H, s.W, s.C, s.Ho, s.Wo, s.Co, s.kh, s.kw, s.sh, s.sw, s.pt, s.pl, s.act};
-                p.out_bf16 = vals[s.out].half ? 1 : 0;
+                p.out_bf16 = vals[s.out].half ? 1 : 0; p.back = s.back;
                 if (s.w2) launch_stem_mfma(p, s.w2, s.w3, stream);
                 else launch_conv_direct(p, stream);
                 break;
@@ -535,7 +536,7 @@
                 break;
             case S_PW: {
                 PwParams p = pw_params(s, n, nl > 1);
-                p.A = in0; p.ascale = in1; p.res = in2; p.out = out;
+                p.A = in0; p.ascale = in1; p.res = in2; p.out = out; p.back = s.back;
                 if (tail_taken(si, n, nl > 1)) {
                     const Step& c = steps[si + 1];
                     PwTail t = tail_of(s, c);
@@ -551,7 +552,7 @@
             }
             case S_DW: {
                 DwParams p = dw_params(s, in0, out, n);
-                p.in_bf16 = vals[s.in0].half ? 1 : 0; p.out_bf16 = vals[s.out].half ? 1 : 0;
+                p.in_bf16 = vals[s.in0].half ? 1 : 0; p.out_bf16 = vals[s.out].half ? 1 : 0; p.back = s.back;
                 if (s.dwl) launch_dwconv_lds(p, out2, s.shape, stream);
                 else launch_dwconv(p, out2, stream);
                 break;
@@ -561,17 +562,18 @@
                     StemGeom sg{s.H2, s.W2, s.pt2, s.pl2};
                     launch_expand_dw(in0, s.w0, s.w1, s.w2, s.w3, out, out2, n, s.H, s.W, s.C, s.Co,
                                      s.Ho, s.Wo, s.kh, s.sh, s.pt, s.pl, s.act, s.act2, s.shape, s.mode == 1 ? &sg : nullptr, stream,
-                                     s.bx ? s.wbx : nullptr, precision, vals[s.out].half ? 1 : 0, vals[s.in0].half ? 1 : 0);
+                                     s.bx ? s.wbx : nullptr, precision, vals[s.out].half ? 1 : 0, vals[s.in0].half ? 1 : 0, s.back);
                 }
                 break;
             case S_MEAN_PARTIAL:
-                launch_mean_partial(in0, out, n, s.H * s.W, s.C, s.S, stream);
+                launch_mean_partial(in0, out, n, s.H * s.W, s.C, s.S, stream, s.back);
                 break;
             case S_MEAN_FINISH:
-                launch_mean_finish(in0, out, n, s.H * s.W, s.C, s.S, stream);
+                launch_mean_finish(in0, out, n, s.H * s.W, s.C, s.S, stream, s.back);
                 break;
             case S_SE: {
                 SeParams p{in0, s.S, s.H * s.W, s.w0, s.w1, s.w2, s.w3, out, n, s.C, s.Cr, s.act, s.act2};
+                p.back = s.back;
                 if (cur_stream) p.threads = 256;
                 launch_se(p, stream);
                 break;
@@ -707,7 +709,7 @@
         os << "\",\"H\":" << s.H << ",\"W\":" << s.W << ",\"C\":" << s.C << ",\"Co\":" << s.Co << ",\"k\":" << s.kh
            << ",\"stride\":" << s.sh << ",\"act\":" << s.act << ",\"fused_scale\":" << (s.kind == S_PW && s.in1 >= 0 ? 1 : 0)
            << ",\"shape\":" << s.shape << ",\"dw_lds\":" << s.dwl << ",\"bx\":" << s.bx << ",\"nt\":" << s.nt << ",\"wm\":" << s.wm << ",\"nt_full\":" << s.nt_full << ",\"wm_full\":" << s.wm_full << ",\"fused_res\":" << (s.kind == S_PW && s.in2 >= 0 ? 1 : 0) << ",\"fused_sum\":" << (s.out2 >= 0 ? 1 : 0) << ",\"flops\":" << sv.flops << ",\"bytes\":" << sv.bytes << ",\"wbytes\":" << s.wbytes
-           << ",\"tail\":" << s.tail << ",\"absorbed\":" << (absorbed ? 1 : 0) << ",\"out_v\":" << s.out << ",\"out2_v\":" << s.out2
+           << ",\"tail\":" << s.tail << ",\"back\":" << s.back << ",\"absorbed\":" << (absorbed ? 1 : 0) << ",\"out_v\":" << s.out << ",\"out2_v\":" << s.out2
            << ",\"in_bf16\":" << ((s.in0 >= 0 && vals[s.in0].half) ? 1 : 0) << ",\"out_bf16\":" << ((s.out >= 0 && vals[s.out].half) ? 1 : 0) << "}";
     }
     os << "]}";
diff --git a/birdnet-go_amd/csrc/engine.h b/birdnet-go_amd/csrc/engine.h
--- a/birdnet-go_amd/csrc/engine.h
+++ b/birdnet-go_amd/csrc/engine.h
@@ -39,6 +39,7 @@
     int nt = 0, wm = 0;
     int tail = 0;
     int H2 = 0, W2 = 0, pt2 = 0, pl2 = 0;
+    int back = 0;
     int shape = -1;
     int nt_full = 0, wm_full = 0;
     int spec = -1;
@@ -118,6 +119,8 @@
     int norm_pair = -1;
     bool pcm_direct = false;
     void find_norm_pair();
+    bool traverse = true;
+    void mark_traverse();
     bool norm_resident_taken(int n, const void* x, int bits, const float* xn) const;
     hipEvent_t ev_ctx_fork = nullptr, ev_ctx_done[kMaxDepth] = {nullptr, nullptr, nullptr};
     unsigned call_idx = 0;
diff --git a/birdnet-go_amd/csrc/expdw.hip b/birdnet-go_amd/csrc/expdw.hip
--- a/birdnet-go_amd/csrc/expdw.hip
+++ b/birdnet-go_amd/csrc/expdw.hip
@@ -23,6 +23,7 @@
     FDiv d_bpc{}, d_cch{}, d_tw{};
     int cpp = 0;
     FDiv d_part{};
+    int back = 0;
 };
 #define ED_ES 36
 #define ED_PERM2 0xfdce5764b98a1320ull
@@ -173,7 +174,8 @@
     const int tid = threadIdx.x, lane = tid & 63, wave = __builtin_amdgcn_readfirstlane(tid >> 6);
     const int li = lane & 15, kq = lane >> 4;
 
-    const unsigned L = xcd_remap(blockIdx.x, nblk);
+    const int back = traverse_flag(p.back);
+    const unsigned L = traverse_index(xcd_remap(blockIdx.x, nblk), nblk, back);
     const int tiles = p.tiles_h * p.tiles_w;
     const int bpc = tiles * p.cchunks;
     const int b = (int)fdiv(L, p.d_bpc), rest = (int)L - b * bpc;
@@ -417,7 +419,8 @@
     const int tid = threadIdx.x, lane = tid & 63, wave = __builtin_amdgcn_readfirstlane(tid >> 6);
     const int li = lane & 15, kq = lane >> 4;
 
-    const unsigned L = xcd_remap(blockIdx.x, nblk);
+    const int back = traverse_flag(p.back);
+    const unsigned L = traverse_index(xcd_remap(blockIdx.x, nblk), nblk, back);
     const int tiles = p.tiles_h * p.tiles_w;
     int b, tile, cc0 = 0;
     int cpp = p.cchunks;
@@ -804,7 +807,7 @@
 void launch_expand_dw(const float* x, const float* we, const float* be, const float* wd, const float* bd, float* y,
                       float* partial, int B, int H, int W, int Cin, int Cmid, int Ho, int Wo, int k, int s, int pt,
                       int pl, int act_e, int act_d, int shape, const StemGeom* stem, hipStream_t st, const uint16_t* wep, int prec, int out_bf16,
-                      int in_bf16) {
+                      int in_bf16, int back) {
     const bool pipe16 = expdw_sk_pipe16(Cin, act_e, stem != nullptr, prec, wep != nullptr);
     const ExpDwGeo g0{k, s, H, W, Ho, Wo, pt, pl, stem != nullptr, pipe16 ? 0 : expdw_skw(Cin, act_e, stem != nullptr)};
     if (!expdw_shape_fits(shape, g0, false)) shape = expdw_default_shape(g0);
@@ -815,7 +818,7 @@
     ExpDwParams p{x, we, be, wd, bd, y, partial, B, g.H, g.W, Cin, Cmid, g.Ho, g.Wo, g.pt, g.pl, act_e, act_d,
                   (g.Ho + sh->toh - 1) / sh->toh, (g.Wo + sh->tow - 1) / sh->tow, (Cmid + 31) / 32, expdw_kw(Cin), expdw_cp(Cmid)};
     p.xsh = tr ? 1 : W; p.xsw = tr ? W : 1; p.ysh = tr ? 1 : Wo; p.ysw = tr ? Wo : 1; p.tr = tr ? 1 : 0;
-    p.out_bf16 = out_bf16;
+    p.out_bf16 = out_bf16; p.back = back;
     unsigned nblk = (unsigned)B * p.tiles_h * p.tiles_w * p.cchunks;
     p.d_bpc = make_fdiv((unsigned)(p.tiles_h * p.tiles_w * p.cchunks));
     p.d_cch = make_fdiv((unsigned)p.cchunks);
@@ -903,7 +906,7 @@
     ExpDwParams p{q.in, nullptr, nullptr, q.w, q.bias, q.out, partial, q.B, g.H, g.W, q.C, q.C, g.Ho, g.Wo, g.pt, g.pl, ACT_NONE, q.act,
                   (g.Ho + sh->toh - 1) / sh->toh, (g.Wo + sh->tow - 1) / sh->tow, (q.C + 31) / 32, 0, q.C};
     p.xsh = tr ? 1 : q.W; p.xsw = tr ? q.W : 1; p.ysh = tr ? 1 : q.Wo; p.ysw = tr ? q.Wo : 1; p.tr = tr ? 1 : 0;
-    p.in_bf16 = q.in_bf16; p.out_bf16 = q.out_bf16;
+    p.in_bf16 = q.in_bf16; p.out_bf16 = q.out_bf16; p.back = q.back;
     unsigned nblk = (unsigned)q.B * p.tiles_h * p.tiles_w * p.cchunks;
     p.d_bpc = make_fdiv((unsigned)(p.tiles_h * p.tiles_w * p.cchunks));
     p.d_cch = make_fdiv((unsigned)p.cchunks);
diff --git a/birdnet-go_amd/csrc/kernels.h b/birdnet-go_amd/csrc/kernels.h
--- a/birdnet-go_amd/csrc/kernels.h
+++ b/birdnet-go_amd/csrc/kernels.h
@@ -42,6 +42,9 @@
     else (void)hipGetLastError();
 }
 
+__device__ __forceinline__ unsigned traverse_index(unsigned L, unsigned nblk, int back) { return back ? nblk - 1u - L : L; }
+__device__ __forceinline__ int traverse_flag(int back) { asm volatile("" : "+s"(back)); return back; }
+
 enum Act : int { ACT_NONE = 0, ACT_RELU = 1, ACT_RELU_N1_TO_1 = 2, ACT_RELU6 = 3, ACT_TANH = 4, ACT_SWISH = 100, ACT_SIGMOID = 101, ACT_HARD_SWISH = 102 };
 
 void launch_pcm_to_f32(const void* pcm, int bits , float* out, size_t n, hipStream_t s);
@@ -82,6 +85,7 @@
     int mel_quads = 0, n_mels = 0, Ctot = 1, c0 = 0, logc = 0, time_major = 0;
     float p1 = 1.f, p2 = 1.f, lfloor = 0.f, lscale = 1.f;
     float* img = nullptr;
+    int back = 0;
 };
 std::vector<double> stft_build_tables(int Lfft, const int* bins, int nb);
 unsigned stft_zmask(int Lfft, const int* bins, int nb);
@@ -111,6 +115,7 @@
     int log = 0;
     float lfloor = 0.f, lscale = 1.f;
     int time_major = 0;
+    int back = 0;
 };
 bool mel_banded_supported(int n_mels, int nbp0, int nbp1);
 void launch_mel_banded(const MelBandParams& p, int nch, int n_clips, hipStream_t s);
@@ -120,6 +125,7 @@
     const float* in; const float* w ; const float* bias; float* out;
     int B, H, W, Cin, Ho, Wo, Cout, kh, kw, sh, sw, pt, pl, act;
     int out_bf16 = 0;
+    int back = 0;
 };
 void launch_conv_direct(const ConvParams& p, hipStream_t s);
 bool conv_direct_bf16_ok(const ConvParams& p);
@@ -140,6 +146,7 @@
     int out_bf16 = 0;
     int res_bf16 = 0;
     int sw = 0;
+    int back = 0;
 };
 enum { PW_SW_B16_OFF = 1, PW_SW_B16_FORCE = 2, PW_SW_B16S_OFF = 4, PW_SW_B16S_FORCE = 8, PW_SW_WS_OFF = 16, PW_SW_WS_FORCE = 32, PW_SW_LAT_OFF = 64,
        PW_SW_TAIL_OFF = 128, PW_SW_TAIL_FORCE = 256 };
@@ -179,6 +186,7 @@
     const float* in; const float* w ; const float* bias; float* out;
     int B, H, W, C, Ho, Wo, kh, kw, sh, sw, pt, pl, act;
     int in_bf16 = 0, out_bf16 = 0;
+    int back = 0;
 };
 int dwconv_sum_slabs(const DwParams& p);
 bool dwconv_tile_geometry(const DwParams& p, int* PY, int* tiles_w, int* tiles, int* tchunks);
@@ -205,7 +213,8 @@
                       hipStream_t st, const uint16_t* wep = nullptr ,
                       int prec = 0 ,
                       int out_bf16 = 0 ,
-                      int in_bf16 = 0 );
+                      int in_bf16 = 0 ,
+                      int back = 0 );
 bool dwconv_lds_supported(const DwParams& p);
 void launch_dwconv_lds(const DwParams& p, float* partial, int shape, hipStream_t st);
 bool expdw_bx_ok(int Cin);
@@ -214,8 +223,8 @@
 
 int mean_splits(int HW);
 int mean_partial_py(int C);
-void launch_mean_partial(const float* in, float* partial, int B, int HW, int C, int S, hipStream_t s);
-void launch_mean_finish(const float* partial, float* out, int B, int HW, int C, int S, hipStream_t s);
+void launch_mean_partial(const float* in, float* partial, int B, int HW, int C, int S, hipStream_t s, int back = 0 );
+void launch_mean_finish(const float* partial, float* out, int B, int HW, int C, int S, hipStream_t s, int back = 0 );
 
 struct SeParams {
     const float* partial; int S; int HW;
@@ -224,6 +233,7 @@
     float* scale;
     int B, C, Cr, act1, act2;
     int threads = 0;
+    int back = 0;
 };
 void launch_se(const SeParams& p, hipStream_t s);
 
diff --git a/birdnet-go_amd/csrc/planner.cpp b/birdnet-go_amd/csrc/planner.cpp
--- a/birdnet-go_amd/csrc/planner.cpp
+++ b/birdnet-go_amd/csrc/planner.cpp
@@ -1465,11 +1465,28 @@
     }
 }
 
+void Engine::mark_traverse() {
+    for (auto& s : steps) s.back = 0;
+    if (!traverse) return;
+    std::vector<int> dir(vals.size(), 0);
+    for (auto& s : steps) {
+        const int pd = s.in0 >= 0 ? dir[s.in0] : 0;
+        const bool light = s.kind == S_SE || s.kind == S_MEAN_PARTIAL || s.kind == S_MEAN_FINISH;
+        const bool takes = light || s.kind == S_STFT || s.kind == S_MELBAND || s.kind == S_CONV_DIRECT || s.kind == S_PW || s.kind == S_DW ||
+                           s.kind == S_EXPAND_DW;
+        const bool has_producer = s.in0 >= 0 && s.in0 != v_input && !vals[s.in0].external;
+        s.back = !takes ? 0 : light ? pd : (has_producer ? !pd : 0);
+        if (s.out >= 0) dir[s.out] = s.back;
+        if (s.out2 >= 0) dir[s.out2] = s.back;
+    }
+}
+
 bool Engine::build(TflModel m, int dev, int maxb, bool plan_only, std::string* err, int* code) {
     device = dev;
     max_batch = maxb;
     pw_sw = pw_switches_from_env();
     if (const char* e = getenv("BNHIP_NORM_RESIDENT")) norm_resident = atoi(e) != 0;
+    if (const char* e = getenv("BNHIP_TRAVERSE")) traverse = atoi(e) != 0;
     const PlanSwitches sw;
     *code = BNHIP_E_UNSUPPORTED;
     if (!run_graph_passes(&m, err)) return false;
@@ -1486,6 +1503,7 @@
     tensor_value = L.tv;
     mark_tails();
     find_norm_pair();
+    mark_traverse();
 
     mark_liveness(vals, steps);
     if (v_emb >= 0) vals[v_emb].last = (int)steps.size();
diff --git a/birdnet-go_amd/csrc/pw_b16.hip b/birdnet-go_amd/csrc/pw_b16.hip
--- a/birdnet-go_amd/csrc/pw_b16.hip
+++ b/birdnet-go_amd/csrc/pw_b16.hip
@@ -186,7 +186,8 @@
     __shared__ __attribute__((aligned(16))) float lds[LDSN];
     const int tid = threadIdx.x, lane = tid & 63, wave = tid >> 6;
     const int li = lane & 15, kq = lane >> 4;
-    const unsigned L = xcd_remap(blockIdx.x, nblk);
+    const int back = traverse_flag(p.back);
+    const unsigned L = traverse_index(xcd_remap(blockIdx.x, nblk), nblk, back);
     const int mblk = (int)fdiv(L, dn);
     const int m0 = mblk * BM;
     const int n0 = ((int)L - mblk * nblk_n) * BN;
@@ -356,7 +357,7 @@
 template <int NT, int NS, bool SC, bool ABF>
 __global__ __launch_bounds__(256) void k_pw_b16s(PwParams p, const uint16_t* __restrict__ Wimg, int Npad, int tiles_per_wave, FDiv dhw) {
     const int lane = threadIdx.x & 63, li = lane & 15, kq = lane >> 4;
-    const int wave_g = blockIdx.x * 4 + (threadIdx.x >> 6);
+    const int wave_g = (int)traverse_index(blockIdx.x, gridDim.x, p.back) * 4 + (threadIdx.x >> 6);
     const int K = p.K, N = p.N;
     const int ntiles = (p.M + 15) >> 4;
     const int t0 = wave_g * tiles_per_wave, t1 = min(t0 + tiles_per_wave, ntiles);
diff --git a/birdnet-go_amd/csrc/pw_bx3.hip b/birdnet-go_amd/csrc/pw_bx3.hip
--- a/birdnet-go_amd/csrc/pw_bx3.hip
+++ b/birdnet-go_amd/csrc/pw_bx3.hip
@@ -20,7 +20,8 @@
     __shared__ __attribute__((aligned(16))) float lds[LDSN];
     const int tid = threadIdx.x, lane = tid & 63, wave = tid >> 6;
     const int li = lane & 15, kq = lane >> 4;
-    const unsigned L = xcd_remap(blockIdx.x, nblk);
+    const int back = traverse_flag(p.back);
+    const unsigned L = traverse_index(xcd_remap(blockIdx.x, nblk), nblk, back);
     const int mblk = (int)fdiv(L, dn);
     const int m0 = mblk * BM;
     const int n0 = ((int)L - mblk * nblk_n) * (NT * 16);
@@ -184,7 +185,8 @@
     float* lds = bx3p_lds;
     const int tid = threadIdx.x, lane = tid & 63, wave = tid >> 6;
     const int li = lane & 15, kq = lane >> 4;
-    const unsigned L = xcd_remap(blockIdx.x, nblk);
+    const int back = traverse_flag(p.back);
+    const unsigned L = traverse_index(xcd_remap(blockIdx.x, nblk), nblk, back);
     const int mblk = (int)fdiv(L, dn);
     const int m0 = mblk * BM;
     const int n0 = ((int)L - mblk * nblk_n) * (NT * 16);
diff --git a/birdnet-go_amd/csrc/pw_gemm.hip b/birdnet-go_amd/csrc/pw_gemm.hip
--- a/birdnet-go_amd/csrc/pw_gemm.hip
+++ b/birdnet-go_amd/csrc/pw_gemm.hip
@@ -29,7 +29,8 @@
     constexpr int WQ = (NT * 16 * PW_C4 + 255) / 256;
     const int tid = threadIdx.x, lane = tid & 63, wave = tid >> 6;
     const int li = lane & 15, kq = lane >> 4;
-    const unsigned L = xcd_remap(blockIdx.x, nblk);
+    const int back = traverse_flag(p.back);
+    const unsigned L = traverse_index(xcd_remap(blockIdx.x, nblk), nblk, back);
     const int mblk = (int)fdiv(L, dn);
     const int m0 = mblk * BM;
     const int n0 = ((int)L - mblk * nblk_n) * (NT * 16);
@@ -171,7 +172,8 @@
     __shared__ __attribute__((aligned(16))) float lds[2 * TILE];
     const int tid = threadIdx.x, lane = tid & 63, wave = tid >> 6;
     const int li = lane & 15, kq = lane >> 4;
-    const unsigned L = xcd_remap(blockIdx.x, nblk);
+    const int back = traverse_flag(p.back);
+    const unsigned L = traverse_index(xcd_remap(blockIdx.x, nblk), nblk, back);
     const int mblk = (int)fdiv(L, dn);
     const int m0 = mblk * BM;
     const int n0 = ((int)L - mblk * nblk_n) * (NT * 16);
@@ -280,7 +282,7 @@
 }
 
 __global__ void k_pw_naive(PwParams p) {
-    size_t idx = (size_t)blockIdx.x * blockDim.x + threadIdx.x;
+    size_t idx = (size_t)traverse_index(blockIdx.x, gridDim.x, p.back) * blockDim.x + threadIdx.x;
     if (idx >= (size_t)p.M * p.N) return;
     int n = (int)(idx % p.N);
     size_t m = idx / p.N;
diff --git a/birdnet-go_amd/csrc/pw_ws.hip b/birdnet-go_amd/csrc/pw_ws.hip
--- a/birdnet-go_amd/csrc/pw_ws.hip
+++ b/birdnet-go_amd/csrc/pw_ws.hip
@@ -73,7 +73,8 @@
     float* Bl = reinterpret_cast<float*>(ws_lds + (size_t)WSLOTS * 16);
     const int tid = threadIdx.x, lane = tid & 63, li = lane & 15, kq = lane >> 4;
     const int wave = __builtin_amdgcn_readfirstlane(tid >> 6);
-    const unsigned L = xcd_remap(blockIdx.x, nblk);
+    const int back = traverse_flag(p.back);
+    const unsigned L = traverse_index(xcd_remap(blockIdx.x, nblk), nblk, back);
     const int g = (int)fdiv(L, dn);
     const int n0 = ((int)L - g * nblk_n) * BN;
     const int K = p.K, N = p.N;
diff --git a/birdnet-go_amd/csrc/stft.hip b/birdnet-go_amd/csrc/stft.hip
--- a/birdnet-go_amd/csrc/stft.hip
+++ b/birdnet-go_amd/csrc/stft.hip
@@ -51,7 +51,7 @@
     float4* melw4 = reinterpret_cast<float4*>(work + (size_t)W * 2 * WSZ);
     const int* binq = reinterpret_cast<const int*>(melw4 + p.mel_quads);
     const int tid = threadIdx.x, lane = tid & 63, wave = tid >> 6;
-    const int b = blockIdx.y;
+    const int b = (int)traverse_index(blockIdx.y, gridDim.y, p.back), bx = (int)traverse_index(blockIdx.x, gridDim.x, p.back);
 
     constexpr int NTAB = 2 * P * 64 + 2 * Q * P;
     for (int i = tid; i < NTAB; i += blockDim.x) sm[i] = (R)p.tw[i];
@@ -89,7 +89,7 @@
         tri[t] = in ? (R)p.tw[NTAB + p.nb_cap + idx] : (R)0.0;
     }
 
-    const int f_begin = (blockIdx.x * W + wave) * p.fpw;
+    const int f_begin = (bx * W + wave) * p.fpw;
     const int f_end = min(f_begin + p.fpw, p.F);
     float2 nx[P];
     auto fetch = [&](int f) {
@@ -441,7 +441,8 @@
     rows[1] = msm + (size_t)MSP_F * p.nbp[0];
     float* tile = rows[C - 1] + (size_t)MSP_F * p.nbp[C - 1];
     const int TS = p.n_mels + 1;
-    const int b = blockIdx.y, f0 = blockIdx.x * MSP_F, nf = min(MSP_F, p.F - f0), tid = threadIdx.x, nthr = blockDim.x;
+    const int b = (int)traverse_index(blockIdx.y, gridDim.y, p.back), f0 = (int)traverse_index(blockIdx.x, gridDim.x, p.back) * MSP_F;
+    const int nf = min(MSP_F, p.F - f0), tid = threadIdx.x, nthr = blockDim.x;
 #pragma unroll
     for (int c = 0; c < C; c++) {
         const float4* src = reinterpret_cast<const float4*>(p.bins[c] + ((size_t)b * p.F + f0) * p.nbp[c]);
```

New measurement: 78880 clips/s (median of 6 runs). Within noise of the previous version (+0.4%).
